# sxyu/volrend

Hardware: AMD Instinct MI355X
Metric: Mrays/s at 800x800, NeRF-synthetic-like SH16 (synthetic C1) (higher is better)
Workload: dtype f32; 1 GPU; C1: synthetic lego-like PlenOctree, depth 9, SH16, 2025715 nodes, 2.23 GB in HBM, 800x800, fx=fy=1111.111, 200-pose orbit, default RenderOptions; fp_mode=strict, launches=38, pcie_inclusive=False, launch_streams=1, parallelism=single GPU

## Files before the change

include/volrend_hip.h:

```cpp
#ifndef VOLREND_HIP_H_
#define VOLREND_HIP_H_

#include <stddef.h>
#include <stdint.h>

#ifdef __cplusplus
extern "C" {
#endif

#define VR_ABI_VERSION 3

enum {
    VR_OK = 0,
    VR_ERR_INVALID_ARGUMENT = 1,
    VR_ERR_HIP = 2,
    VR_ERR_NO_DEVICE = 3,
    VR_ERR_BAD_TREE = 4,
    VR_ERR_UNSUPPORTED = 5,
    VR_ERR_OUT_OF_MEMORY = 6
};

enum { VR_FORMAT_RGBA = 0, VR_FORMAT_SH = 1, VR_FORMAT_SG = 2, VR_FORMAT_ASG = 3 };

enum { VR_FP_STRICT = 0, VR_FP_FMA = 1 };

#define VR_MAX_BASIS 25

typedef struct VrTreeOpaque* vr_tree_t;

typedef struct VrTreeDesc {
    const int32_t* child;
    const uint16_t* data;
    const float* extra;
    uint64_t extra_count;
    float offset[3];
    float scale[3];
    int32_t N;
    int64_t capacity;
    int32_t data_dim;
    int32_t format;
    int32_t basis_dim;
    float ndc_width;
    float ndc_height;
    float ndc_focal;
    int32_t memory;
} VrTreeDesc;

typedef struct VrQuantDesc {
    const uint16_t* quant_colors;
    const uint16_t* quant_map;
    const uint16_t* sigma;
    const uint16_t* data_retained;
    int32_t n_quant;
    int32_t n_retained;
} VrQuantDesc;

typedef struct VrTreeInfo {
    int64_t capacity;
    int32_t N, data_dim, format, basis_dim;
    int32_t max_depth;
    int32_t device;
    uint64_t device_bytes;
    uint64_t leaf_stride;
    int32_t query_mode;
    int32_t top_levels;
    int32_t brick_levels;
    int32_t brick_blocked;
} VrTreeInfo;

#define VR_QUERY_LOOKUP 0
#define VR_QUERY_DESCENT 1
int vr_query_mode_for(int N, int max_depth, int64_t capacity);

typedef struct VrCamera {
    float transform[12];
    int32_t width, height;
    float fx, fy;
} VrCamera;

typedef struct VrRenderOptions {
    float step_size;
    float sigma_thresh;
    float stop_thresh;
    float background_brightness;
    float render_bbox[6];
    int32_t basis_minmax[2];
    float rot_dirs[3];
    int32_t show_grid;
    int32_t grid_max_depth;
    int32_t render_depth;
    int32_t enable_probe;
    float probe[3];
    int32_t probe_disp_size;
} VrRenderOptions;

enum { VR_LAYOUT_FRAME = 0, VR_LAYOUT_COMPACT = 1 };

typedef struct VrFrame {
    void* rgba;
    int64_t pitch;
    const float* depth;
    float* accum;
    int32_t offscreen;
    int32_t layout;
    int32_t tile_w, tile_h;
    int32_t rank, world;
    int32_t fp_mode;
    int32_t reserved;
    uint64_t* counters;
} VrFrame;

typedef struct VrCounters {
    uint64_t rays, rays_hit_box, samples, child_reads, hit_samples, alg_bytes, early_stops;
} VrCounters;

int vr_abi_version(void);
const char* vr_last_error(void);
int vr_device_count(int* count);
int vr_set_device(int device);
int vr_device_name(int device, char* name, size_t name_len);

void vr_default_tree_desc(VrTreeDesc* desc);
int vr_tree_upload(const VrTreeDesc* desc, vr_tree_t* out);
int vr_tree_upload_quantized(const VrTreeDesc* desc, const VrQuantDesc* quant, vr_tree_t* out);
int vr_decode_quantized(const VrTreeDesc* desc, const VrQuantDesc* quant, uint16_t* data_out);
int vr_tree_clone(vr_tree_t src, int device, vr_tree_t* out);
int vr_tree_free(vr_tree_t tree);
int vr_tree_info(vr_tree_t tree, VrTreeInfo* info);
enum { VR_DATA_F16 = 0, VR_DATA_F32 = 1 };
int vr_tree_update_data(vr_tree_t tree, const void* data_dev, int dtype, void* stream);
int vr_tree_read_data(vr_tree_t tree, void* data_dev, int dtype, void* stream);
enum { VR_STEP_SGD = 0, VR_STEP_ADAM = 1 };
typedef struct VrStep {
    float*    master;
    float*    grad;
    uint32_t* touched;
    float*    m;
    float*    v;
    int32_t   kind;
    float     lr, lr_sigma;
    float     beta1, beta2, eps;
    int32_t   step;
} VrStep;
int vr_tree_step(vr_tree_t tree, const VrStep* s, void* stream);

void vr_default_options(VrRenderOptions* opt);
void vr_default_frame(VrFrame* frame);
int64_t vr_compact_bytes(int width, int height, int tile_w, int tile_h, int world);
int vr_render(vr_tree_t tree, const VrCamera* cam, const VrRenderOptions* opt,
              const VrFrame* frame, void* stream);
#define VR_MAX_BATCH 512
int vr_render_batch(vr_tree_t tree, int n_frames, const VrCamera* cams,
                    const VrRenderOptions* opt, const VrFrame* frames, void* stream);
enum { VR_DEPTH_TREE = 0, VR_DEPTH_WORLD = 1 };
typedef struct VrAov {
    float*  depth;
    float*  transmittance;
    int64_t pitch;
} VrAov;
int vr_render_aov(vr_tree_t tree, int n_frames, const VrCamera* cams, const VrRenderOptions* opt,
                  const VrFrame* frames, const VrAov* aovs, int depth_units, void* stream);
typedef struct VrLeafWeights {
    float*    max_weight;
    uint32_t* hits;
} VrLeafWeights;
int vr_accumulate_weights(vr_tree_t tree, int n_frames, const VrCamera* cams,
                          const VrRenderOptions* opt, int fp_mode, const VrLeafWeights* out, void* stream);
int vr_render_backward(vr_tree_t tree, int n_frames, const VrCamera* cams, const VrRenderOptions* opt,
                       int fp_mode, const float* grad_accum, float* grad_data, void* stream);
typedef struct VrRays {
    const float* origins;
    const float* dirs;
} VrRays;
typedef struct VrRayOut {
    void*  rgba;
    float* accum;
} VrRayOut;
int vr_render_rays(vr_tree_t tree, int64_t n, const VrRays* rays, const VrRenderOptions* opt, int fp_mode,
                   const VrRayOut* out, void* stream);
int vr_accumulate_weights_rays(vr_tree_t tree, int64_t n, const VrRays* rays, const VrRenderOptions* opt,
                               int fp_mode, const VrLeafWeights* out, void* stream);
int vr_render_backward_rays(vr_tree_t tree, int64_t n, const VrRays* rays, const VrRenderOptions* opt,
                            int fp_mode, const float* grad_accum, float* grad_data, void* stream);
int vr_render_backward_touched(vr_tree_t tree, int n_frames, const VrCamera* cams, const VrRenderOptions* opt,
                               int fp_mode, const float* grad_accum, float* grad_data, uint32_t* touched,
                               void* stream);
int vr_render_backward_rays_touched(vr_tree_t tree, int64_t n, const VrRays* rays, const VrRenderOptions* opt,
                                    int fp_mode, const float* grad_accum, float* grad_data, uint32_t* touched,
                                    void* stream);
int vr_reserve_rays(vr_tree_t tree, int64_t n, int n_slots);
int vr_reserve(vr_tree_t tree, int width, int height, int n_frames);
int vr_reserve_tiles(vr_tree_t tree, int width, int height, int n_frames, int tile_w, int tile_h,
                     int world, int n_slots);
int vr_tree_status(vr_tree_t tree, uint32_t* status, int reset);
int vr_tree_status_on(vr_tree_t tree, uint32_t* status, int reset, void* stream);
int vr_set_tuning(const char* key, int value);
int vr_tree_set_tuning(vr_tree_t tree, const char* key, int value);
int vr_sched_stats(vr_tree_t tree, uint64_t out[8], int reset);
int vr_touch_enable(vr_tree_t tree, int enable);
int vr_touch_count(vr_tree_t tree, uint64_t out[4], int reset);
int vr_touch_read(vr_tree_t tree, int which, uint32_t* host_words, uint64_t n_words,
                  uint64_t* bitmap_words, uint64_t* granule_bytes);
int vr_assemble_tiles(void* frame_rgba, int64_t pitch, const void* gathered, int width,
                      int height, int tile_w, int tile_h, int world, void* stream);
int vr_assemble_tiles_batch(void* frames_rgba, int64_t frame_stride, int64_t pitch,
                            const void* gathered, int64_t rank_stride, int64_t in_frame_stride,
                            int n_frames, int width, int height, int tile_w, int tile_h, int world,
                            void* stream);
int vr_probe_coeffs(vr_tree_t tree, const VrRenderOptions* opt, float* out_dev, void* stream);

enum { VR_SPACE_WORLD = 0, VR_SPACE_TREE = 1 };

typedef struct VrQueryOut {
    float* sigma;
    int32_t* depth;
    float* local;
    float* coeffs;
    float* rgb;
} VrQueryOut;

int vr_query_points(vr_tree_t tree, int64_t n, const float* xyz_dev, const float* dirs_dev, int space,
                    const VrQueryOut* out, void* stream);
int vr_query_grid(vr_tree_t tree, const float lo[3], const float hi[3], const int32_t res[3],
                  const float dir[3], int space, const VrQueryOut* out, void* stream);

int vr_read_back(void* host_rgba, const void* dev_rgba, int64_t pitch, int width, int height,
                 void* stream);
int vr_stream_sync(void* stream);

#ifdef __cplusplus
}
#endif
#endif
```

volrend_amd/_abi.py:

```python
from __future__ import annotations

import ctypes as C
import os

HERE = os.path.dirname(os.path.abspath(__file__))
LIB_PATH = os.environ.get("VOLREND_HIP_LIB") or os.path.join(HERE, "libvolrend_hip.so")

VR_OK = 0
FORMAT_RGBA, FORMAT_SH, FORMAT_SG, FORMAT_ASG = 0, 1, 2, 3
FORMATS = {"RGBA": FORMAT_RGBA, "SH": FORMAT_SH, "SG": FORMAT_SG, "ASG": FORMAT_ASG}
FP_STRICT, FP_FMA = 0, 1
QUERY_LOOKUP, QUERY_DESCENT = 0, 1
LAYOUT_FRAME, LAYOUT_COMPACT = 0, 1
SPACE_WORLD, SPACE_TREE = 0, 1
SPACES = {"world": SPACE_WORLD, "tree": SPACE_TREE}
DEPTH_TREE, DEPTH_WORLD = 0, 1
DEPTH_UNITS = {"tree": DEPTH_TREE, "world": DEPTH_WORLD}
DATA_F16, DATA_F32 = 0, 1
STEP_SGD, STEP_ADAM = 0, 1
STEP_KINDS = {"sgd": STEP_SGD, "adam": STEP_ADAM}
MAX_BASIS = 25


class VrTreeDesc(C.Structure):
    _fields_ = [("child", C.c_void_p), ("data", C.c_void_p), ("extra", C.c_void_p),
                ("extra_count", C.c_uint64), ("offset", C.c_float * 3), ("scale", C.c_float * 3),
                ("N", C.c_int32), ("capacity", C.c_int64), ("data_dim", C.c_int32),
                ("format", C.c_int32), ("basis_dim", C.c_int32), ("ndc_width", C.c_float),
                ("ndc_height", C.c_float), ("ndc_focal", C.c_float), ("memory", C.c_int32)]


class VrQuantDesc(C.Structure):
    _fields_ = [("quant_colors", C.c_void_p), ("quant_map", C.c_void_p), ("sigma", C.c_void_p),
                ("data_retained", C.c_void_p), ("n_quant", C.c_int32), ("n_retained", C.c_int32)]


class VrTreeInfo(C.Structure):
    _fields_ = [("capacity", C.c_int64), ("N", C.c_int32), ("data_dim", C.c_int32),
                ("format", C.c_int32), ("basis_dim", C.c_int32), ("max_depth", C.c_int32),
                ("device", C.c_int32), ("device_bytes", C.c_uint64), ("leaf_stride", C.c_uint64),
                ("query_mode", C.c_int32), ("top_levels", C.c_int32), ("brick_levels", C.c_int32),
                ("brick_blocked", C.c_int32)]


class VrCamera(C.Structure):
    _fields_ = [("transform", C.c_float * 12), ("width", C.c_int32), ("height", C.c_int32),
                ("fx", C.c_float), ("fy", C.c_float)]


class VrRenderOptions(C.Structure):
    _fields_ = [("step_size", C.c_float), ("sigma_thresh", C.c_float), ("stop_thresh", C.c_float),
                ("background_brightness", C.c_float), ("render_bbox", C.c_float * 6),
                ("basis_minmax", C.c_int32 * 2), ("rot_dirs", C.c_float * 3),
                ("show_grid", C.c_int32), ("grid_max_depth", C.c_int32),
                ("render_depth", C.c_int32), ("enable_probe", C.c_int32),
                ("probe", C.c_float * 3), ("probe_disp_size", C.c_int32)]


class VrFrame(C.Structure):
    _fields_ = [("rgba", C.c_void_p), ("pitch", C.c_int64), ("depth", C.c_void_p),
                ("accum", C.c_void_p), ("offscreen", C.c_int32), ("layout", C.c_int32),
                ("tile_w", C.c_int32), ("tile_h", C.c_int32), ("rank", C.c_int32),
                ("world", C.c_int32), ("fp_mode", C.c_int32), ("reserved", C.c_int32),
                ("counters", C.c_void_p)]


class VrAov(C.Structure):
    _fields_ = [("depth", C.c_void_p), ("transmittance", C.c_void_p), ("pitch", C.c_int64)]


class VrLeafWeights(C.Structure):
    _fields_ = [("max_weight", C.c_void_p), ("hits", C.c_void_p)]


class VrRays(C.Structure):
    _fields_ = [("origins", C.c_void_p), ("dirs", C.c_void_p)]


class VrRayOut(C.Structure):
    _fields_ = [("rgba", C.c_void_p), ("accum", C.c_void_p)]


class VrStep(C.Structure):
    _fields_ = [("master", C.c_void_p), ("grad", C.c_void_p), ("touched", C.c_void_p), ("m", C.c_void_p),
                ("v", C.c_void_p), ("kind", C.c_int32), ("lr", C.c_float), ("lr_sigma", C.c_float),
                ("beta1", C.c_float), ("beta2", C.c_float), ("eps", C.c_float), ("step", C.c_int32)]


class VrQueryOut(C.Structure):
    _fields_ = [("sigma", C.c_void_p), ("depth", C.c_void_p), ("local", C.c_void_p),
                ("coeffs", C.c_void_p), ("rgb", C.c_void_p)]


ABI_VERSION = 3
MAX_BATCH = 512

COUNTER_FIELDS = ("rays", "rays_hit_box", "samples", "child_reads", "hit_samples", "alg_bytes",
                  "early_stops")


PROTOTYPES = {
    "vr_abi_version": (C.c_int, []),
    "vr_last_error": (C.c_char_p, []),
    "vr_device_count": (C.c_int, [C.POINTER(C.c_int)]),
    "vr_set_device": (C.c_int, [C.c_int]),
    "vr_device_name": (C.c_int, [C.c_int, C.c_char_p, C.c_size_t]),
    "vr_default_tree_desc": (None, [C.POINTER(VrTreeDesc)]),
    "vr_tree_upload": (C.c_int, [C.POINTER(VrTreeDesc), C.POINTER(C.c_void_p)]),
    "vr_tree_upload_quantized": (C.c_int, [C.POINTER(VrTreeDesc), C.POINTER(VrQuantDesc),
                                           C.POINTER(C.c_void_p)]),
    "vr_decode_quantized": (C.c_int, [C.POINTER(VrTreeDesc), C.POINTER(VrQuantDesc), C.c_void_p]),
    "vr_tree_clone": (C.c_int, [C.c_void_p, C.c_int, C.POINTER(C.c_void_p)]),
    "vr_tree_free": (C.c_int, [C.c_void_p]),
    "vr_tree_info": (C.c_int, [C.c_void_p, C.POINTER(VrTreeInfo)]),
    "vr_tree_update_data": (C.c_int, [C.c_void_p, C.c_void_p, C.c_int, C.c_void_p]),
    "vr_tree_read_data": (C.c_int, [C.c_void_p, C.c_void_p, C.c_int, C.c_void_p]),
    "vr_query_mode_for": (C.c_int, [C.c_int, C.c_int, C.c_int64]),
    "vr_default_options": (None, [C.POINTER(VrRenderOptions)]),
    "vr_default_frame": (None, [C.POINTER(VrFrame)]),
    "vr_compact_bytes": (C.c_int64, [C.c_int, C.c_int, C.c_int, C.c_int, C.c_int]),
    "vr_render": (C.c_int, [C.c_void_p, C.POINTER(VrCamera), C.POINTER(VrRenderOptions),
                            C.POINTER(VrFrame), C.c_void_p]),
    "vr_render_batch": (C.c_int, [C.c_void_p, C.c_int, C.POINTER(VrCamera),
                                  C.POINTER(VrRenderOptions), C.POINTER(VrFrame), C.c_void_p]),
    "vr_render_aov": (C.c_int, [C.c_void_p, C.c_int, C.POINTER(VrCamera), C.POINTER(VrRenderOptions),
                                C.POINTER(VrFrame), C.POINTER(VrAov), C.c_int, C.c_void_p]),
    "vr_accumulate_weights": (C.c_int, [C.c_void_p, C.c_int, C.POINTER(VrCamera), C.POINTER(VrRenderOptions),
                                        C.c_int, C.POINTER(VrLeafWeights), C.c_void_p]),
    "vr_render_backward": (C.c_int, [C.c_void_p, C.c_int, C.POINTER(VrCamera), C.POINTER(VrRenderOptions),
                                     C.c_int, C.c_void_p, C.c_void_p, C.c_void_p]),
    "vr_render_backward_touched": (C.c_int, [C.c_void_p, C.c_int, C.POINTER(VrCamera), C.POINTER(VrRenderOptions),
                                             C.c_int, C.c_void_p, C.c_void_p, C.c_void_p, C.c_void_p]),
    "vr_render_backward_rays_touched": (C.c_int, [C.c_void_p, C.c_int64, C.POINTER(VrRays), C.POINTER(VrRenderOptions),
                                                  C.c_int, C.c_void_p, C.c_void_p, C.c_void_p, C.c_void_p]),
    "vr_tree_step": (C.c_int, [C.c_void_p, C.POINTER(VrStep), C.c_void_p]),
    "vr_render_rays": (C.c_int, [C.c_void_p, C.c_int64, C.POINTER(VrRays), C.POINTER(VrRenderOptions), C.c_int,
                                 C.POINTER(VrRayOut), C.c_void_p]),
    "vr_accumulate_weights_rays": (C.c_int, [C.c_void_p, C.c_int64, C.POINTER(VrRays), C.POINTER(VrRenderOptions),
                                             C.c_int, C.POINTER(VrLeafWeights), C.c_void_p]),
    "vr_render_backward_rays": (C.c_int, [C.c_void_p, C.c_int64, C.POINTER(VrRays), C.POINTER(VrRenderOptions),
                                          C.c_int, C.c_void_p, C.c_void_p, C.c_void_p]),
    "vr_reserve_rays": (C.c_int, [C.c_void_p, C.c_int64, C.c_int]),
    "vr_reserve": (C.c_int, [C.c_void_p, C.c_int, C.c_int, C.c_int]),
    "vr_reserve_tiles": (C.c_int, [C.c_void_p, C.c_int, C.c_int, C.c_int, C.c_int, C.c_int, C.c_int,
                                   C.c_int]),
    "vr_tree_status": (C.c_int, [C.c_void_p, C.POINTER(C.c_uint32), C.c_int]),
    "vr_tree_status_on": (C.c_int, [C.c_void_p, C.POINTER(C.c_uint32), C.c_int, C.c_void_p]),
    "vr_set_tuning": (C.c_int, [C.c_char_p, C.c_int]),
    "vr_tree_set_tuning": (C.c_int, [C.c_void_p, C.c_char_p, C.c_int]),
    "vr_sched_stats": (C.c_int, [C.c_void_p, C.POINTER(C.c_uint64 * 8), C.c_int]),
    "vr_touch_enable": (C.c_int, [C.c_void_p, C.c_int]),
    "vr_touch_count": (C.c_int, [C.c_void_p, C.POINTER(C.c_uint64 * 4), C.c_int]),
    "vr_touch_read": (C.c_int, [C.c_void_p, C.c_int, C.c_void_p, C.c_uint64, C.POINTER(C.c_uint64),
                                C.POINTER(C.c_uint64)]),
    "vr_assemble_tiles": (C.c_int, [C.c_void_p, C.c_int64, C.c_void_p, C.c_int, C.c_int, C.c_int,
                                    C.c_int, C.c_int, C.c_void_p]),
    "vr_assemble_tiles_batch": (C.c_int, [C.c_void_p, C.c_int64, C.c_int64, C.c_void_p, C.c_int64,
                                          C.c_int64, C.c_int, C.c_int, C.c_int, C.c_int, C.c_int,
                                          C.c_int, C.c_void_p]),
    "vr_probe_coeffs": (C.c_int, [C.c_void_p, C.POINTER(VrRenderOptions), C.c_void_p, C.c_void_p]),
    "vr_query_points": (C.c_int, [C.c_void_p, C.c_int64, C.c_void_p, C.c_void_p, C.c_int,
                                  C.POINTER(VrQueryOut), C.c_void_p]),
    "vr_query_grid": (C.c_int, [C.c_void_p, C.POINTER(C.c_float * 3), C.POINTER(C.c_float * 3),
                                C.POINTER(C.c_int32 * 3), C.POINTER(C.c_float * 3), C.c_int,
                                C.POINTER(VrQueryOut), C.c_void_p]),
    "vr_read_back": (C.c_int, [C.c_void_p, C.c_void_p, C.c_int64, C.c_int, C.c_int, C.c_void_p]),
    "vr_stream_sync": (C.c_int, [C.c_void_p]),
}

_lib = None


class VolrendError(RuntimeError):
    def __init__(self, code: int, msg: str):
        super().__init__(f"volrend_hip error {code}: {msg}")
        self.code = code


def lib():
    global _lib
    if _lib is None:
        if not os.path.exists(LIB_PATH):
            raise RuntimeError(
                f"{LIB_PATH} not found: the HIP library is mandatory (no CPU fallback). "
                "Build it with `python -m volrend_amd.build`.")
        L = C.CDLL(LIB_PATH)
        for name, (res, args) in PROTOTYPES.items():
            fn = getattr(L, name)
            fn.restype = res
            fn.argtypes = args
        if L.vr_abi_version() != ABI_VERSION:
            raise RuntimeError("libvolrend_hip.so ABI version mismatch")
        _lib = L
    return _lib


def check(rc: int) -> None:
    if rc != VR_OK:
        raise VolrendError(rc, (lib().vr_last_error() or b"").decode("utf-8", "replace"))
```

volrend_amd/_tree.py:

```python
from __future__ import annotations

import ctypes as C
import os

import numpy as np

from . import _abi, _ops
from ._args import _stream_ptr


def parse_data_format(s: str):
    idx = next((i for i, ch in enumerate(s) if not ch.isalpha()), -1)
    if idx < 0:
        return "RGBA", -1
    head = s[:idx]
    try:
        dim = int("".join(ch for ch in s[idx:] if ch.isdigit() or ch == "-") or "0")
    except ValueError:
        dim = 0
    return (head if head in ("ASG", "SG", "SH") else "RGBA"), dim


class N3Tree:

    def __init__(self, path: str | None = None, upload: bool = True):
        self.N = 0
        self.data_dim = 0
        self.data_format = ("RGBA", -1)
        self.capacity = 0
        self.scale = np.zeros(3, np.float32)
        self.offset = np.zeros(3, np.float32)
        self.use_ndc = False
        self.ndc_width = self.ndc_height = self.ndc_focal = 0.0
        self.child_ = None
        self.data_ = None
        self.extra_ = None
        self.quant_ = None
        self._handle = C.c_void_p()
        self._loaded = False
        if path is not None:
            self.open(path, upload=upload)

    @classmethod
    def from_arrays(cls, child, data, offset, invradius3, data_format: str, extra=None,
                    ndc=None, upload: bool = True) -> "N3Tree":
        t = cls()
        t._set_arrays(child, data, offset, invradius3, data_format, extra)
        if ndc:
            t.use_ndc = True
            t.ndc_width, t.ndc_height, t.ndc_focal = map(float, ndc)
        if upload:
            t.load_device()
        return t

    @classmethod
    def from_synth(cls, tree, upload: bool = True, ndc=None) -> "N3Tree":
        return cls.from_arrays(tree.child, tree.data, tree.offset, tree.invradius3,
                               tree.data_format, tree.extra, ndc=ndc, upload=upload)

    def _set_arrays(self, child, data, offset, invradius3, data_format, extra, data_dim=None):
        child = np.ascontiguousarray(child, dtype=np.int32)
        if child.ndim != 4 or not (child.shape[1] == child.shape[2] == child.shape[3]):
            raise RuntimeError("child must be int32 [capacity, N, N, N]")
        self.N = int(child.shape[1])
        self.capacity = int(child.shape[0])
        self.child_ = child.reshape(self.capacity, self.N, self.N, self.N)
        self.quant_ = None
        if data is None:
            self.data_ = None
            self.data_dim = int(data_dim)
        else:
            data = np.asarray(data)
            if data.dtype != np.float16:
                raise RuntimeError("data must be stored in half precision")
            self.data_ = np.ascontiguousarray(data)
            self.data_dim = int(self.data_.shape[-1])
            if self.data_.size != self.capacity * self.N ** 3 * self.data_dim:
                raise RuntimeError("data does not have capacity * N^3 * data_dim values")
        self.data_format = parse_data_format(data_format)
        self.scale = np.asarray(invradius3, dtype=np.float32).reshape(3).copy()
        self.offset = np.asarray(offset, dtype=np.float32).reshape(3).copy()
        self.extra_ = None if extra is None else np.ascontiguousarray(extra, dtype=np.float32)

    def open(self, path: str, upload: bool = True, device_decode: bool = True) -> None:
        if not path.endswith(".npz"):
            raise ValueError("tree file must end in .npz")
        if not os.path.exists(path):
            raise FileNotFoundError(f"Can't load because file does not exist: {path}")
        z = np.load(path)
        data_dim = int(z["data_dim"])
        if "data_format" in z.files:
            fmt = str(z["data_format"])
        else:
            fmt = "RGBA" if data_dim == 4 else f"SH{(data_dim - 1) // 3}"
        if "invradius3" in z.files:
            scale = z["invradius3"].astype(np.float32)
        else:
            scale = np.full(3, float(z["invradius"]), dtype=np.float32)
        child = z["child"]
        extra = z["extra_data"] if "extra_data" in z.files else None
        if "quant_colors" in z.files and upload and device_decode:
            self._set_arrays(child, None, z["offset"], scale, fmt, extra, data_dim=data_dim)
            self.quant_ = _quant_arrays(z, child)
        else:
            if "quant_colors" in z.files:
                data = _decode_quantised(z, child, data_dim)
            else:
                data = z["data"]
            self._set_arrays(child, data, z["offset"], scale, fmt, extra)
            if self.data_dim != data_dim:
                raise RuntimeError("data_dim does not match the data array")
        pb = path[:-4] + "_poses_bounds.npy"
        if os.path.exists(pb):
            arr = np.load(pb).reshape(-1)
            self.use_ndc = True
            self.ndc_height, self.ndc_width, self.ndc_focal = float(arr[4]), float(arr[9]), float(
                arr[14])
        if upload:
            self.load_device()

    def load_device(self) -> None:
        L = _abi.lib()
        self.free_device()
        d = _abi.VrTreeDesc()
        L.vr_default_tree_desc(C.byref(d))
        d.child = self.child_.ctypes.data
        if self.data_ is not None:
            d.data = self.data_.ctypes.data
        elif self.quant_ is None:
            raise RuntimeError("tree has no data (clear_cpu_memory was called)")
        if self.extra_ is not None:
            d.extra = self.extra_.ctypes.data
            d.extra_count = self.extra_.size
        for i in range(3):
            d.offset[i] = float(self.offset[i])
            d.scale[i] = float(self.scale[i])
        d.N = self.N
        d.capacity = self.capacity
        d.data_dim = self.data_dim
        d.format = _abi.FORMATS[self.data_format[0]]
        d.basis_dim = self.data_format[1]
        d.ndc_width = self.ndc_width if self.use_ndc else -1.0
        d.ndc_height = self.ndc_height
        d.ndc_focal = self.ndc_focal
        d.memory = 0
        h = C.c_void_p()
        if self.data_ is None:
            _abi.check(L.vr_tree_upload_quantized(C.byref(d), C.byref(self._quant_desc()),
                                                  C.byref(h)))
        else:
            _abi.check(L.vr_tree_upload(C.byref(d), C.byref(h)))
        self._handle = h
        self._loaded = True

    def _quant_desc(self) -> "_abi.VrQuantDesc":
        q = _abi.VrQuantDesc()
        a = self.quant_
        q.n_quant = a["quant_map"].shape[0]
        q.quant_colors = a["quant_colors"].ctypes.data
        q.quant_map = a["quant_map"].ctypes.data
        q.sigma = a["sigma"].ctypes.data
        if a["data_retained"] is not None:
            q.n_retained = a["data_retained"].shape[0]
            q.data_retained = a["data_retained"].ctypes.data
        return q

    def decode_host(self, on_device: bool = False) -> np.ndarray:
        if self.data_ is None and self.quant_ is not None:
            shape = (self.capacity, self.N, self.N, self.N, self.data_dim)
            if on_device:
                d = _abi.VrTreeDesc()
                _abi.lib().vr_default_tree_desc(C.byref(d))
                d.N, d.capacity, d.data_dim, d.memory = self.N, self.capacity, self.data_dim, 0
                out = np.empty(shape, np.float16)
                _abi.check(_abi.lib().vr_decode_quantized(C.byref(d), C.byref(self._quant_desc()),
                                                          out.ctypes.data))
                self.data_ = out
            else:
                a = self.quant_
                self.data_ = _decode_arrays(a["quant_colors"], a["quant_map"], a["sigma"],
                                            a["data_retained"], self.data_dim).reshape(shape)
        return self.data_

    def clone_to(self, device: int) -> "N3Tree":
        t = N3Tree()
        for k in ("N", "data_dim", "data_format", "capacity", "scale", "offset", "use_ndc",
                  "ndc_width", "ndc_height", "ndc_focal", "child_"):
            setattr(t, k, getattr(self, k))
        h = C.c_void_p()
        _abi.check(_abi.lib().vr_tree_clone(self.handle, int(device), C.byref(h)))
        t._handle = h
        t._loaded = True
        return t

    def free_device(self) -> None:
        if self._handle:
            _abi.lib().vr_tree_free(self._handle)
            self._handle = C.c_void_p()
        self._loaded = False

    def is_device_loaded(self) -> bool:
        return self._loaded

    def clear_cpu_memory(self) -> None:
        self.data_ = None
        self.quant_ = None

    def sched_stats(self, reset: bool = True) -> dict:
        out = (C.c_uint64 * 8)()
        _abi.check(_abi.lib().vr_sched_stats(self._handle, C.byref(out), 1 if reset else 0))
        names = ("march_rounds", "march_lanes", "shade_rounds", "shade_lanes", "distinct_leaves",
                 "retire_rounds", "retired", "iterations")
        return dict(zip(names, [int(v) for v in out]))

    def touch_enable(self, enable: bool = True) -> None:
        _abi.check(_abi.lib().vr_touch_enable(self.handle, 1 if enable else 0))

    def touch_count(self, reset: bool = True) -> dict:
        out = (C.c_uint64 * 4)()
        _abi.check(_abi.lib().vr_touch_count(self.handle, C.byref(out), 1 if reset else 0))
        return dict(zip(("leaves", "nodes", "top", "bricks"), [int(v) for v in out]))

    def touch_read(self, which: int):
        words, gran = C.c_uint64(0), C.c_uint64(0)
        _abi.check(_abi.lib().vr_touch_read(self.handle, int(which), None, 0, C.byref(words), C.byref(gran)))
        out = np.zeros(int(words.value), dtype=np.uint32)
        if out.size:
            _abi.check(_abi.lib().vr_touch_read(self.handle, int(which), out.ctypes.data, out.size, None, None))
        return out, int(gran.value)

    def reserve(self, width: int, height: int, n_frames: int, shard: "TileShard | None" = None,
                n_slots: int = 2) -> None:
        if shard is None and n_slots == 2:
            _abi.check(_abi.lib().vr_reserve(self.handle, int(width), int(height), int(n_frames)))
        else:
            tw, th, world = (shard.tile_w, shard.tile_h, shard.world) if shard else (0, 0, 1)
            _abi.check(_abi.lib().vr_reserve_tiles(self.handle, int(width), int(height),
                                                   int(n_frames), tw, th, world, int(n_slots)))

    def set_tuning(self, **kw) -> None:
        for k, v in kw.items():
            _abi.check(_abi.lib().vr_tree_set_tuning(self.handle, k.encode(), int(v)))

    def status(self, reset: bool = False, stream=None) -> int:
        out = C.c_uint32(0)
        if stream is not None:
            _abi.check(_abi.lib().vr_tree_status_on(self.handle, C.byref(out), 1 if reset else 0,
                                                    _stream_ptr(stream)))
        else:
            _abi.check(_abi.lib().vr_tree_status(self.handle, C.byref(out), 1 if reset else 0))
        return int(out.value)

    def reserve_rays(self, n: int, n_slots: int = 2) -> None:
        _abi.check(_abi.lib().vr_reserve_rays(self.handle, int(n), int(n_slots)))

    query, query_grid = _ops.query_points, _ops.query_grid
    accumulate_weights, render_backward = _ops.accumulate_weights, _ops.render_backward
    render_rays, accumulate_weights_rays = _ops.render_rays, _ops.accumulate_weights_rays
    render_backward_rays, touched_words = _ops.render_backward_rays, _ops.touched_words
    step, update_data, read_data = _ops.tree_step, _ops.update_data, _ops.read_data

    def info(self) -> dict:
        i = _abi.VrTreeInfo()
        _abi.check(_abi.lib().vr_tree_info(self._handle, C.byref(i)))
        return {n: int(getattr(i, n)) for n, _ in i._fields_}

    @property
    def handle(self):
        if not self._loaded:
            raise RuntimeError("tree is not on the device (call load_device)")
        return self._handle

    def __del__(self):
        try:
            self.free_device()
        except Exception:
            pass


def _quant_arrays(z, child) -> dict:
    qc = z["quant_colors"]
    if qc.dtype != np.float16:
        raise RuntimeError("codebook must be stored in half precision")
    qm = z["quant_map"]
    n_q = qm.shape[0]
    if qc.shape[0] != n_q:
        raise RuntimeError("codebook and map basis numbers does not match")
    cap, N = qm.shape[1], child.shape[1]
    if cap != child.shape[0] or qc.shape[1:] != (65536, 3):
        raise RuntimeError("quantised arrays do not match the tree")
    n_slots = cap * N * N * N
    retained = z["data_retained"] if "data_retained" in z.files else None
    return dict(
        quant_colors=np.ascontiguousarray(qc),
        quant_map=np.ascontiguousarray(qm.reshape(n_q, n_slots), dtype=np.uint16),
        sigma=np.ascontiguousarray(z["sigma"].reshape(n_slots), dtype=np.float16),
        data_retained=None if retained is None else np.ascontiguousarray(
            retained.reshape(retained.shape[0], n_slots, 3), dtype=np.float16))


def _decode_arrays(qc, qm, sigma, retained, data_dim: int) -> np.ndarray:
    n_q, n_slots = qm.shape
    n_ret = 0 if retained is None else retained.shape[0]
    n_basis = n_q + n_ret
    data = np.zeros((n_slots, data_dim), dtype=np.float16)
    for j in range(n_q):
        cols = qc[j][qm[j].astype(np.int64)]
        for c in range(3):
            data[:, j + n_ret + c * n_basis] = cols[:, c]
    data[:, data_dim - 1] = sigma
    for j in range(n_ret):
        for c in range(3):
            data[:, j + c * n_basis] = retained[j, :, c]
    return data


def _decode_quantised(z, child, data_dim: int) -> np.ndarray:
    a = _quant_arrays(z, child)
    cap, N = child.shape[0], child.shape[1]
    return _decode_arrays(a["quant_colors"], a["quant_map"], a["sigma"], a["data_retained"],
                          data_dim).reshape(cap, N, N, N, data_dim)
```

volrend_amd/csrc/vr_api.cpp:

```cpp
#include <hip/hip_runtime.h>

#include <climits>
#include <cstdarg>
#include <cstdio>
#include <cstdlib>
#include <cstring>
#include <mutex>

#include "vr_host.h"
#include "vr_tree_walk.h"

namespace {

thread_local char g_err[512] = "";

enum KnobRange { kClamp, kClamp64, kFlag, kAutoFlag };
struct Knob { const char *key, *env; int Tuning::*field; KnobRange range; int lo, hi; bool fixed_at_upload; };
const Knob kKnobs[] = {
    {"march_max", "VR_MARCH_MAX", &Tuning::march_max, kClamp, 1, INT_MAX, false},
    {"refill_min", "VR_REFILL_MIN", &Tuning::refill_min, kClamp, 1, 64, false},
    {"drain_flush", "VR_DRAIN_FLUSH", &Tuning::drain_flush, kClamp, 0, 64, false},
    {"waves_per_cu", "VR_WAVES_PER_CU", &Tuning::waves_per_cu, kClamp, 0, 64, false},
    {"frame_group", "VR_FRAME_GROUP", &Tuning::frame_group, kClamp, 0, INT_MAX, false},
    {"super_block", "VR_SUPER_BLOCK", &Tuning::super_block, kClamp, 0, 64, false},
    {"records_nt", "VR_RECORDS_NT", &Tuning::records_nt, kAutoFlag, 0, 0, false},
    {"xcd_queues", "VR_XCD_QUEUES", &Tuning::xcd_queues, kFlag, 0, 0, false},
    {"chunk_max", "VR_CHUNK_MAX", &Tuning::chunk_max, kClamp64, 0, INT_MAX, false},
    {"raygen_waves", "VR_RAYGEN_WAVES", &Tuning::raygen_waves, kClamp, 0, INT_MAX, false},
    {"top_levels", "VR_TOP_LEVELS", &Tuning::top_levels, kClamp, INT_MIN, INT_MAX, true},
    {"brick_levels", "VR_BRICK_LEVELS", &Tuning::brick_levels, kClamp, INT_MIN, INT_MAX, true},
    {"brick_blocked", "VR_BRICK_BLOCKED", &Tuning::brick_blocked, kAutoFlag, 0, 0, true},
    {"max_iter", "VR_MAX_ITER", &Tuning::max_iter, kClamp, 1, INT_MAX, false},
    {"weights_check", "VR_WEIGHTS_CHECK", &Tuning::weights_check, kFlag, 0, 0, false},
};

const Knob* find_knob(const char* key) {
    for (const Knob& k : kKnobs)
        if (!strcmp(key, k.key)) return &k;
    return nullptr;
}

void set_knob(Tuning& tn, const Knob& k, int v) {
    const int clamped = v < k.lo ? k.lo : (v > k.hi ? k.hi : v);
    tn.*k.field = k.range == kFlag       ? v != 0
                  : k.range == kAutoFlag ? (v < 0 ? -1 : v != 0)
                  : k.range == kClamp64  ? (clamped > 0 && clamped < 64 ? 64 : clamped & ~63)
                                         : clamped;
}

std::mutex g_tuning_mutex;
Tuning& default_tuning_locked() {
    static Tuning tn = [] {
        Tuning x;
        for (const Knob& k : kKnobs)
            if (const char* e = getenv(k.env)) set_knob(x, k, atoi(e));
        return x;
    }();
    return tn;
}

uint64_t touch_granule(int which) {
    return which == 0 ? (1ull << vr::kTouchLeafShift) : 128ull;
}
size_t touch_words(uint64_t array_bytes, int which) {
    const uint64_t g = touch_granule(which);
    return (size_t)(((array_bytes + g - 1) / g + 31) / 32);
}

}

int fail(int code, const char* fmt, ...) {
    va_list ap;
    va_start(ap, fmt);
    vsnprintf(g_err, sizeof(g_err), fmt, ap);
    va_end(ap);
    return code;
}

Tuning default_tuning() {
    std::lock_guard<std::mutex> g(g_tuning_mutex);
    return default_tuning_locked();
}

extern "C" {

int vr_abi_version(void) { return VR_ABI_VERSION; }

const char* vr_last_error(void) { return g_err; }

int vr_device_count(int* count) {
    if (!count) return fail(VR_ERR_INVALID_ARGUMENT, "count is NULL");
    int n = 0;
    hipError_t e = hipGetDeviceCount(&n);
    if (e != hipSuccess) {
        *count = 0;
        return fail(VR_ERR_NO_DEVICE, "hipGetDeviceCount: %s", hipGetErrorString(e));
    }
    *count = n;
    return VR_OK;
}

int vr_set_device(int device) {
    if (device < 0) return VR_OK;
    HIP_TRY(hipSetDevice(device));
    return VR_OK;
}

int vr_device_name(int device, char* name, size_t name_len) {
    if (!name || name_len == 0) return fail(VR_ERR_INVALID_ARGUMENT, "name buffer is NULL");
    hipDeviceProp_t prop;
    if (device < 0) HIP_TRY(hipGetDevice(&device));
    HIP_TRY(hipGetDeviceProperties(&prop, device));
    snprintf(name, name_len, "%s", prop.gcnArchName);
    return VR_OK;
}

void vr_default_tree_desc(VrTreeDesc* d) {
    if (!d) return;
    memset(d, 0, sizeof(*d));
    d->N = 2;
    d->format = VR_FORMAT_RGBA;
    d->basis_dim = -1;
    d->ndc_width = -1.f;
}

int vr_tree_info(vr_tree_t t, VrTreeInfo* info) {
    if (!t || !info) return fail(VR_ERR_INVALID_ARGUMENT, "tree/info is NULL");
    info->capacity = t->desc.capacity;
    info->N = t->desc.N;
    info->data_dim = t->desc.data_dim;
    info->format = t->desc.format;
    info->basis_dim = t->desc.basis_dim;
    info->max_depth = t->max_depth;
    info->device = t->device;
    info->device_bytes = t->device_bytes;
    info->leaf_stride = (uint64_t)t->leaf_stride_h * 2u;
    info->query_mode = t->top_levels > 0 ? VR_QUERY_LOOKUP : VR_QUERY_DESCENT;
    info->top_levels = t->top_levels;
    info->brick_levels = t->brick_levels;
    info->brick_blocked = t->brick_blocked;
    return VR_OK;
}

int vr_query_mode_for(int N, int max_depth, int64_t capacity) {
    return lookup_applies(N, max_depth, capacity) ? VR_QUERY_LOOKUP : VR_QUERY_DESCENT;
}

void vr_default_options(VrRenderOptions* o) {
    if (!o) return;
    memset(o, 0, sizeof(*o));
    o->step_size = 1e-4f;
    o->sigma_thresh = 1e-2f;
    o->stop_thresh = 1e-2f;
    o->background_brightness = 1.f;
    o->render_bbox[3] = o->render_bbox[4] = o->render_bbox[5] = 1.f;
    o->basis_minmax[0] = 0;
    o->basis_minmax[1] = VR_MAX_BASIS - 1;
    o->grid_max_depth = 4;
    o->probe[2] = 1.f;
    o->probe_disp_size = 100;
}

void vr_default_frame(VrFrame* f) {
    if (!f) return;
    memset(f, 0, sizeof(*f));
    f->offscreen = 1;
    f->layout = VR_LAYOUT_FRAME;
    f->world = 1;
    f->fp_mode = VR_FP_STRICT;
}

int64_t vr_compact_bytes(int width, int height, int tile_w, int tile_h, int world) {
    vr::KParams g;
    if (tile_geometry(width, height, tile_w, tile_h, 0, world, g) != VR_OK) return -1;
    return (int64_t)g.n_local_tiles * g.tile_w * g.tile_h * 4;
}

int vr_set_tuning(const char* key, int value) {
    if (!key) return fail(VR_ERR_INVALID_ARGUMENT, "key is NULL");
    const Knob* k = find_knob(key);
    if (!k) return fail(VR_ERR_INVALID_ARGUMENT, "unknown tuning key '%s'", key);
    std::lock_guard<std::mutex> g(g_tuning_mutex);
    set_knob(default_tuning_locked(), *k, value);
    return VR_OK;
}

int vr_tree_set_tuning(vr_tree_t t, const char* key, int value) {
    if (!t || !key) return fail(VR_ERR_INVALID_ARGUMENT, "tree/key is NULL");
    const Knob* k = find_knob(key);
    if (!k) return fail(VR_ERR_INVALID_ARGUMENT, "unknown tuning key '%s'", key);
    if (k->fixed_at_upload)
        return fail(VR_ERR_INVALID_ARGUMENT, "'%s' is fixed at upload (vr_set_tuning before it)", key);
    std::lock_guard<std::mutex> g(t->launch_mutex);
    set_knob(t->tn, *k, value);
    return VR_OK;
}

int vr_sched_stats(vr_tree_t t, uint64_t out[vr::kSchedStats], int reset) {
    if (!t || !out) return fail(VR_ERR_INVALID_ARGUMENT, "NULL argument");
    DeviceGuard guard(t->device);
    HIP_TRY(hipMemcpy(out, t->sched_stats.get(), vr::kSchedStats * sizeof(uint64_t), hipMemcpyDeviceToHost));
    if (reset) HIP_TRY(hipMemset(t->sched_stats.get(), 0, vr::kSchedStats * sizeof(uint64_t)));
    return VR_OK;
}

int vr_tree_status(vr_tree_t t, uint32_t* status, int reset) {
    if (!t || !status) return fail(VR_ERR_INVALID_ARGUMENT, "NULL argument");
    DeviceGuard guard(t->device);
    HIP_TRY(hipMemcpy(status, t->status.get(), sizeof(uint32_t), hipMemcpyDeviceToHost));
    if (reset) HIP_TRY(hipMemset(t->status.get(), 0, sizeof(uint32_t)));
    return VR_OK;
}

int vr_tree_status_on(vr_tree_t t, uint32_t* status, int reset, void* stream) {
    if (!t || !status) return fail(VR_ERR_INVALID_ARGUMENT, "NULL argument");
    DeviceGuard guard(t->device);
    hipStream_t hs = static_cast<hipStream_t>(stream);
    thread_local uint32_t* pinned = nullptr;
    if (!pinned) HIP_TRY(hipHostMalloc((void**)&pinned, sizeof(uint32_t), hipHostMallocPortable));
    HIP_TRY(hipMemcpyAsync(pinned, t->status.get(), sizeof(uint32_t), hipMemcpyDeviceToHost, hs));
    if (reset) HIP_TRY(hipMemsetAsync(t->status.get(), 0, sizeof(uint32_t), hs));
    HIP_TRY(hipStreamSynchronize(hs));
    *status = *pinned;
    return VR_OK;
}

int vr_touch_enable(vr_tree_t t, int enable) {
    if (!t) return fail(VR_ERR_INVALID_ARGUMENT, "tree is NULL");
    DeviceGuard guard(t->device);
    std::lock_guard<std::mutex> lock(t->launch_mutex);
    HIP_TRY(hipDeviceSynchronize());
    for (int i = 0; i < 4; ++i) {
        HIP_TRY(t->touch[i].reset());
        const size_t words = touch_words(t->arrays[i].bytes(), i);
        if (enable && words) {
            HIP_TRY(t->touch[i].alloc(words * sizeof(uint32_t)));
            HIP_TRY(hipMemset(t->touch[i].get(), 0, words * sizeof(uint32_t)));
        }
    }
    if (enable && !t->touch_out) HIP_TRY(t->touch_out.alloc(4 * sizeof(unsigned long long)));
    return VR_OK;
}

int vr_touch_count(vr_tree_t t, uint64_t out[4], int reset) {
    if (!t || !out) return fail(VR_ERR_INVALID_ARGUMENT, "NULL argument");
    if (!t->touch_out) return fail(VR_ERR_INVALID_ARGUMENT, "vr_touch_enable(tree, 1) first");
    DeviceGuard guard(t->device);
    std::lock_guard<std::mutex> lock(t->launch_mutex);
    HIP_TRY(hipDeviceSynchronize());
    HIP_TRY(hipMemset(t->touch_out.get(), 0, 4 * sizeof(unsigned long long)));
    for (int i = 0; i < 4; ++i) {
        if (!t->touch[i]) continue;
        const size_t words = touch_words(t->arrays[i].bytes(), i);
        HIP_TRY(vr::launch_popcount(t->touch[i].get<uint32_t>(), words,
                                    t->touch_out.get<unsigned long long>() + i, nullptr));
        if (reset) HIP_TRY(hipMemsetAsync(t->touch[i].get(), 0, words * sizeof(uint32_t), nullptr));
    }
    HIP_TRY(hipMemcpy(out, t->touch_out.get(), 4 * sizeof(uint64_t), hipMemcpyDeviceToHost));
    return VR_OK;
}

int vr_touch_read(vr_tree_t t, int which, uint32_t* host_words, uint64_t n_words,
                  uint64_t* bitmap_words, uint64_t* granule_bytes) {
    if (!t || which < 0 || which > 3) return fail(VR_ERR_INVALID_ARGUMENT, "tree / array index");
    if (!t->touch_out) return fail(VR_ERR_INVALID_ARGUMENT, "vr_touch_enable(tree, 1) first");
    DeviceGuard guard(t->device);
    std::lock_guard<std::mutex> lock(t->launch_mutex);
    const uint64_t words = t->touch[which] ? touch_words(t->arrays[which].bytes(), which) : 0;
    if (bitmap_words) *bitmap_words = words;
    if (granule_bytes) *granule_bytes = touch_granule(which);
    const uint64_t n = n_words < words ? n_words : words;
    if (host_words && n) {
        HIP_TRY(hipDeviceSynchronize());
        HIP_TRY(hipMemcpy(host_words, t->touch[which].get(), n * sizeof(uint32_t), hipMemcpyDeviceToHost));
    }
    return VR_OK;
}

int vr_assemble_tiles(void* frame_rgba, int64_t pitch, const void* gathered, int width, int height,
                      int tile_w, int tile_h, int world, void* stream) {
    if (world < 1) world = 1;
    const int64_t rank_bytes = vr_compact_bytes(width, height, tile_w, tile_h, world);
    if (rank_bytes < 0) return VR_ERR_INVALID_ARGUMENT;
    return vr_assemble_tiles_batch(frame_rgba, 0, pitch, gathered, rank_bytes, 0, 1, width, height,
                                   tile_w, tile_h, world, stream);
}

int vr_assemble_tiles_batch(void* frames_rgba, int64_t frame_stride, int64_t pitch,
                            const void* gathered, int64_t rank_stride, int64_t in_frame_stride,
                            int n_frames, int width, int height, int tile_w, int tile_h, int world,
                            void* stream) {
    if (!frames_rgba || !gathered) return fail(VR_ERR_INVALID_ARGUMENT, "NULL buffer");
    if (n_frames < 1) return fail(VR_ERR_INVALID_ARGUMENT, "n_frames must be positive");
    if (world < 1) world = 1;
    vr::KParams g;
    if (int rc = tile_geometry(width, height, tile_w, tile_h, 0, world, g)) return rc;
    HIP_TRY(vr::launch_assemble(static_cast<uint8_t*>(frames_rgba),
                                pitch ? pitch : (int64_t)width * 4,
                                static_cast<const uint8_t*>(gathered), width, height, g.tile_w, g.tile_h, world,
                                n_frames, frame_stride, rank_stride, in_frame_stride,
                                static_cast<hipStream_t>(stream)));
    return VR_OK;
}

int vr_probe_coeffs(vr_tree_t t, const VrRenderOptions* opt, float* out_dev, void* stream) {
    if (!t || !opt || !out_dev) return fail(VR_ERR_INVALID_ARGUMENT, "NULL argument");
    DeviceGuard guard(t->device);
    vr::KParams k;
    memset(&k, 0, sizeof(k));
    fill_tree_params(k, t);
    HIP_TRY(vr::launch_probe(k, opt->probe, out_dev, static_cast<hipStream_t>(stream)));
    return VR_OK;
}

int vr_read_back(void* host_rgba, const void* dev_rgba, int64_t pitch, int width, int height,
                 void* stream) {
    if (!host_rgba || !dev_rgba) return fail(VR_ERR_INVALID_ARGUMENT, "NULL buffer");
    if (pitch == 0) pitch = (int64_t)width * 4;
    HIP_TRY(hipMemcpy2DAsync(host_rgba, (size_t)width * 4, dev_rgba, (size_t)pitch,
                             (size_t)width * 4, (size_t)height, hipMemcpyDeviceToHost,
                             static_cast<hipStream_t>(stream)));
    return VR_OK;
}

int vr_stream_sync(void* stream) {
    HIP_TRY(hipStreamSynchronize(static_cast<hipStream_t>(stream)));
    return VR_OK;
}

}
```

volrend_amd/csrc/vr_host.h:

```cpp
#pragma once
#include <hip/hip_runtime.h>

#include <mutex>
#include <vector>

#include "vr_internal.h"
#include "vr_launch_plan.h"

#pragma GCC visibility push(hidden)

#include "volrend/internal/hip_owners.hpp"
using volrend::internal::DeviceBuffer;
using volrend::internal::DeviceEvent;
using volrend::internal::DeviceGuard;

int fail(int code, const char* fmt, ...);
inline int hip_code(hipError_t e) { return e == hipErrorOutOfMemory ? VR_ERR_OUT_OF_MEMORY : VR_ERR_HIP; }

#define HIP_TRY(expr)                                                                                 \
    do {                                                                                              \
        hipError_t e_ = (expr);                                                                       \
        if (e_ != hipSuccess)                                                                         \
            return fail(hip_code(e_), "%s failed: %s (%s:%d)", #expr, hipGetErrorString(e_), __FILE__, \
                        __LINE__);                                                                    \
    } while (0)

Tuning default_tuning();

constexpr unsigned kLaunchSlots = 8;

struct LaunchSlot {
    DeviceEvent done;
    bool used = false;
    hipStream_t last_stream = nullptr;
    bool growing = false;
    DeviceBuffer rays;
};

enum TreeArray { kLeaves = 0, kNodes = 1, kTop = 2, kBricks = 3 };

struct TreeShape {
    VrTreeDesc desc{};
    int32_t max_depth = 0;
    int leaf_stride_h = 0;
    int top_levels = 0, brick_levels = 0, n_bricks = 0;
    int brick_blocked = 0;
    uint64_t device_bytes = 0;
};

struct VrTreeOpaque : TreeShape {
    int device = 0;
    DeviceBuffer arrays[4];
    DeviceBuffer extra, status, sched_stats;
    DeviceBuffer touch[4];
    DeviceBuffer touch_out;
    DeviceBuffer probe_buf;
    DeviceBuffer slot_frames;
    DeviceBuffer slot_heads;
    DeviceBuffer slot_aovs;
    std::vector<int32_t> file_node;
    DeviceBuffer file_node_dev;
    std::vector<int32_t> brick_root;
    DeviceBuffer brick_root_dev;
    DeviceBuffer node_of_file_dev;
    LaunchSlot slots[kLaunchSlots];
    unsigned launch_seq = 0;
    std::mutex launch_mutex;
    Tuning tn;
    int n_cus = 256;
};

void fill_tree_params(vr::KParams& k, const VrTreeOpaque* t);

int tile_geometry(int width, int height, int tile_w, int tile_h, int rank, int world, vr::KParams& k);
int launch_geometry(int width, int height, int tile_w, int tile_h, int rank, int world, int n_frames,
                    vr::KParams& k);
int list_geometry(const char* what, int64_t n, vr::KParams& k);

inline size_t ray_buffer_bytes(uint32_t total_rays, int words_per_ray) {
    return vr::ray_slots(total_rays) * (size_t)words_per_ray * sizeof(uint32_t);
}
inline size_t list_pixel_bytes(uint32_t total_rays) { return (size_t)total_rays * 4; }

int acquire_slot(VrTreeOpaque* t, std::unique_lock<std::mutex>& guard, hipStream_t hs, vr::KParams& k,
                 size_t need, unsigned& slot);

class SlotTurn {
    LaunchSlot* slot_ = nullptr;
    hipStream_t stream_ = nullptr;
public:
    int begin(LaunchSlot& ls, hipStream_t hs);
    ~SlotTurn();
};

int ensure_device_table(VrTreeOpaque* t, DeviceBuffer& dev, const std::vector<int32_t>& host, size_t entries,
                        const char* name);
int ensure_file_nodes(VrTreeOpaque* t);

#pragma GCC visibility pop
```

volrend_amd/csrc/vr_internal.h:

```cpp
#pragma once
#include <hip/hip_runtime.h>
#include <stdint.h>

#include "volrend_hip.h"

namespace vr {

constexpr int kMaxBatch = 512;
constexpr int kTableChunk = 48;
constexpr int kTouchLeafShift = 7;

enum { BASIS_RGBA = -1, BASIS_1 = 1, BASIS_4 = 4, BASIS_9 = 9, BASIS_16 = 16, BASIS_25 = 25 };
__host__ __device__ inline int basis_flavour(int format, int basis_dim) {
    if (format == VR_FORMAT_RGBA || basis_dim < 0) return BASIS_RGBA;
    switch (basis_dim) {
        case 25: return BASIS_25;
        case 16: return BASIS_16;
        case 9: return BASIS_9;
        case 4: return BASIS_4;
        default: return BASIS_1;
    }
}
__host__ __device__ inline int basis_words(int flavour) { return flavour == BASIS_RGBA ? 0 : flavour; }
__host__ __device__ inline bool ray_vdir(int format, int flavour) {
    return format == VR_FORMAT_SH && basis_words(flavour) > 3;
}
__host__ __device__ inline int ray_tail_words(int format, int flavour) {
    return ray_vdir(format, flavour) ? 3 : basis_words(flavour);
}

enum {
    kRayCen = 0,
    kRayDir = 3,
    kRayInvDir = 6,
    kRayT = 9,
    kRayTmax = 10,
    kRayDeltaScale = 11,
    kRayXy = 12,
    kRayPixelLo = 13,
    kRayPixelHi = 14,
    kRayFrame = 15,
    kRayWords = 16,
    kRayTail = kRayWords,
};
__host__ __device__ inline uint32_t ray_groups16(uint32_t total_rays) { return ((total_rays >> 6) + 15u) >> 4; }
__host__ __device__ inline size_t ray_slots(uint32_t total_rays) { return (size_t)ray_groups16(total_rays) * 16 * 64; }

constexpr int kMaxQueues = 8;
constexpr int kMaxQueuesShift = 3;
constexpr int kQueueStride = 16;
constexpr int kQueueHead = 0;
constexpr int kQueueCount = 1;
constexpr int kSlotHeaderWords = 16;
constexpr int kSlotWords = 160;
static_assert(kMaxQueues == 1 << kMaxQueuesShift, "queues are picked with shifts and masks");
static_assert(kSlotWords >= kSlotHeaderWords + kMaxQueues * kQueueStride, "a slot holds its header and every queue");

enum {
    kStatMarchRounds = 0,
    kStatMarchLanes,
    kStatShadeRounds,
    kStatShadeLanes,
    kStatDistinctLeaves,
    kStatRetireRounds,
    kStatRetiredRays,
    kStatIterations,
    kSchedStats
};
static_assert(kSchedStats == 8, "vr_sched_stats(out[8]) is public ABI");

struct FrameDesc {
    float xf[12];
    uint8_t* rgba;
    float* accum;
    const float* depth;
    VrCounters* counters;
};

struct FrameTable {
    int32_t first;
    int32_t n;
    FrameDesc f[kTableChunk];
};

struct KParams {
    const uint32_t* nodes;
    const uint16_t* leaves;
    const uint2* top;
    const uint32_t* bricks;
    const float* extra;
    float offset[3];
    float scale[3];
    int32_t N, N3;
    int64_t capacity;
    int32_t data_dim;
    int32_t format;
    int32_t basis_dim;
    int32_t leaf_stride_h;
    int32_t max_depth;
    int32_t top_levels;
    int32_t brick_levels;
    int32_t brick_blocked;
    float ndc_width, ndc_height, ndc_focal;
    int32_t width, height;
    float fx, fy;
    float step_size, sigma_thresh, stop_thresh, background_brightness;
    float bbox[6];
    int32_t basis_min, basis_max;
    int32_t render_depth;
    int32_t enable_probe;
    int32_t probe_disp_size;
    const float* probe_coeffs;
    int32_t rot_enabled;
    float rot_k[3];
    float rot_cos, rot_sin;
    const FrameDesc* frames;
    int32_t n_frames;
    int64_t pitch;
    int32_t offscreen;
    int32_t layout;
    int32_t tile_w, tile_h;
    int32_t tiles_x, tiles_y;
    int32_t rank, world;
    int32_t n_local_tiles;
    int32_t wblocks_per_tile_x;
    int32_t wblocks_per_tile;
    int64_t n_wave_blocks;
    uint32_t total_rays;
    uint32_t* queue_head;
    int32_t n_queues;
    int32_t chunk_max;
    const uint32_t* ray_buf;
    uint32_t* ray_buf_rw;
    int32_t basis_words;
    int32_t ray_tail_words;
    int32_t ray_vdir;
    int32_t refill_min;
    int32_t march_max;
    int32_t drain_flush;
    int32_t max_iter;
    int32_t instrumented;
    int32_t any_accum;
    int32_t records_nt;
    int32_t frame_group;
    int32_t super_block;
    uint32_t* status;
    unsigned long long* sched_stats;
    uint32_t* touch[4];
};

inline bool uses_lookup(const KParams& p) { return p.N == 2 && p.top_levels > 0; }

inline unsigned persistent_grid(int64_t total_blocks, int n_cus, int waves_per_cu) {
    int64_t want = total_blocks / 2;
    if (want < 256) want = 256;
    if (want > total_blocks) want = total_blocks;
    const int64_t cap = (int64_t)n_cus * waves_per_cu;
    return (unsigned)(want < cap ? want : cap);
}

struct AovDesc {
    float* depth;
    float* transmittance;
};
struct AovParams {
    const AovDesc* planes;
    int64_t pitch;
    int32_t depth_world;
};
struct AovTable {
    int32_t first;
    int32_t n;
    AovDesc f[kTableChunk];
};

constexpr int kWeightRayWords = kRayDeltaScale + 1;
static_assert(kWeightRayWords <= kRayWords, "a slot reserved for colour rays holds the weight rays of the same shape");
struct WeightParams {
    uint32_t* max_weight;
    uint32_t* hits;
    const int32_t* file_node;
};

constexpr int kRayListShift = 15;
constexpr int kRayListWidth = 1 << kRayListShift;
struct RayList {
    const float* origins;
    const float* dirs;
    int64_t n;
};
__host__ __device__ inline uint32_t ray_list_slots(int64_t n) { return (uint32_t)(((n + 63) >> 6) << 6); }

hipError_t launch_weights(const KParams& p, const WeightParams& w, int fp_mode, int n_cus, int waves_override,
                          int gen_waves, bool check_first, hipStream_t stream, const RayList* rays = nullptr);

enum {
    kGradRayVdir = kWeightRayWords,
    kGradRayPixel = kGradRayVdir + 3,
    kGradRayWords = kGradRayPixel + 1,
};
static_assert(kGradRayWords <= kRayWords, "a slot reserved for colour rays holds the backward rays of the same shape");
struct GradParams {
    const float* grad_accum;
    float* grad_data;
    const int32_t* file_node;
    uint32_t* touched;
};

hipError_t launch_grad(const KParams& p, const GradParams& g, int fp_mode, int n_cus, int waves_override,
                       int gen_waves, hipStream_t stream, const RayList* rays = nullptr);

struct UpdateArgs {
    uint32_t* nodes;
    uint16_t* leaves;
    const int32_t* file_node;
    void* data;
    int64_t capacity;
    int32_t N3, data_dim;
    int32_t stride_h;
    int32_t f32;
};
hipError_t launch_update_values(const UpdateArgs& a, int n_cus, hipStream_t stream);
hipError_t launch_read_values(const UpdateArgs& a, int n_cus, hipStream_t stream);
hipError_t launch_refresh_lookup(const uint32_t* nodes, const int32_t* brick_root, int n_bricks, uint2* top,
                                 uint32_t* bricks, int top_levels, int brick_levels, hipStream_t stream);

struct StepArgs {
    uint32_t* nodes;
    uint16_t* leaves;
    const int32_t* node_of_file;
    float* master;
    float* grad;
    float* m;
    float* v;
    uint32_t* touched;
    int64_t n_words;
    int64_t n_slots;
    int32_t N3, data_dim;
    int32_t stride_h;
    int32_t adam;
    float lr, lr_sigma;
    float beta1, beta2, omb1, omb2, sbc2, eps;
};
hipError_t launch_step_values(const StepArgs& a, int n_cus, hipStream_t stream);

hipError_t launch_prepare_aov(const AovParams& a, const AovTable& tbl, hipStream_t stream);
hipError_t launch_render_aov(const KParams& p, const AovParams& a, int fp_mode, int n_cus, int waves_override,
                             int gen_waves, hipStream_t stream);
hipError_t launch_prepare(const KParams& p, const FrameTable& tbl, hipStream_t stream);
hipError_t launch_render(const KParams& p, int fp_mode, int n_cus, int waves_override, int gen_waves,
                         hipStream_t stream, const RayList* rays = nullptr);
hipError_t launch_probe(const KParams& p, const float probe[3], float* out_dev,
                        hipStream_t stream);

int leaf_stride_halfs(int data_dim);
hipError_t launch_relayout(const int32_t* child, const uint16_t* data, const int32_t* perm,
                           uint32_t* nodes, uint16_t* leaves, int64_t n_slots, int N3,
                           int data_dim, int stride_h, hipStream_t stream);
hipError_t launch_decode_quant(const uint16_t* colors, const uint16_t* map, const uint16_t* sigma,
                               const uint16_t* retained, uint16_t* data, int64_t n_slots,
                               int n_quant, int n_ret, int data_dim, hipStream_t stream);
hipError_t launch_build_lookup(const uint32_t* nodes, const int32_t* brick_root, int n_bricks,
                               uint2* top, uint32_t* bricks, int top_levels, int brick_levels,
                               int brick_blocked, uint32_t* error_flag, hipStream_t stream);
hipError_t launch_popcount(const uint32_t* words, uint64_t n_words, unsigned long long* out,
                           hipStream_t stream);
hipError_t launch_assemble(uint8_t* frame, int64_t pitch, const uint8_t* gathered, int width,
                           int height, int tile_w, int tile_h, int world, int n_frames,
                           int64_t out_stride, int64_t rank_stride, int64_t in_stride,
                           hipStream_t stream);

}
```

volrend_amd/csrc/vr_launch.cpp:

```cpp
#include <hip/hip_runtime.h>

#include <cmath>
#include <cstring>
#include <mutex>

#include "vr_host.h"

static_assert(kPlanQueues == vr::kMaxQueues, "vr_launch_plan.h restates the queue count of vr_internal.h");

namespace {

float host_norm3(const float* d, int fma) {
    float s;
    if (fma) {
        s = std::fmaf(d[0], d[0], d[1] * d[1]);
        s = std::fmaf(d[2], d[2], s);
    } else {
        s = d[0] * d[0] + d[1] * d[1];
        s = d[2] * d[2] + s;
    }
    return std::sqrt(s);
}

}

void fill_tree_params(vr::KParams& k, const VrTreeOpaque* t) {
    k.nodes = t->arrays[kNodes].get<uint32_t>();
    k.leaves = t->arrays[kLeaves].get<uint16_t>();
    k.top = t->arrays[kTop].get<uint2>();
    k.bricks = t->arrays[kBricks].get<uint32_t>();
    k.top_levels = t->top_levels;
    k.brick_levels = t->brick_levels;
    k.brick_blocked = t->brick_blocked;
    k.extra = t->extra.get<float>();
    for (int i = 0; i < 3; ++i) {
        k.offset[i] = t->desc.offset[i];
        k.scale[i] = t->desc.scale[i];
    }
    k.N = t->desc.N;
    k.N3 = t->desc.N * t->desc.N * t->desc.N;
    k.capacity = t->desc.capacity;
    k.data_dim = t->desc.data_dim;
    k.format = t->desc.format;
    k.basis_dim = t->desc.basis_dim;
    k.leaf_stride_h = t->leaf_stride_h;
    k.max_depth = t->max_depth;
    k.ndc_width = t->desc.ndc_width;
    k.ndc_height = t->desc.ndc_height;
    k.ndc_focal = t->desc.ndc_focal;
    k.status = t->status.get<uint32_t>();
    k.sched_stats = t->sched_stats.get<unsigned long long>();
    for (int i = 0; i < 4; ++i) k.touch[i] = t->touch[i].get<uint32_t>();
}

int tile_geometry(int width, int height, int tile_w, int tile_h, int rank, int world, vr::KParams& k) {
    if (width <= 0 || height <= 0) return fail(VR_ERR_INVALID_ARGUMENT, "empty image");
    if (tile_w == 0 && tile_h == 0) {
        tile_w = (width + 7) & ~7;
        tile_h = (height + 7) & ~7;
    }
    if (tile_w <= 0 || tile_h <= 0 || (tile_w & 7) || (tile_h & 7))
        return fail(VR_ERR_INVALID_ARGUMENT, "tile size %dx%d must be positive multiples of 8",
                    tile_w, tile_h);
    k.tile_w = tile_w;
    k.tile_h = tile_h;
    k.tiles_x = (width + tile_w - 1) / tile_w;
    k.tiles_y = (height + tile_h - 1) / tile_h;
    k.rank = rank;
    k.world = world < 1 ? 1 : world;
    k.n_local_tiles = (int32_t)(((int64_t)k.tiles_x * k.tiles_y - rank + k.world - 1) / k.world);
    k.wblocks_per_tile_x = tile_w / 8;
    k.wblocks_per_tile = (tile_w / 8) * (tile_h / 8);
    k.n_wave_blocks = (int64_t)k.n_local_tiles * k.wblocks_per_tile;
    return VR_OK;
}

int launch_geometry(int width, int height, int tile_w, int tile_h, int rank, int world, int n_frames,
                    vr::KParams& k) {
    if (width < 1 || height < 1 || width > 65535 || height > 65535)
        return fail(VR_ERR_INVALID_ARGUMENT, "image size %dx%d outside [1, 65535]", width, height);
    if (int rc = tile_geometry(width, height, tile_w, tile_h, rank, world, k)) return rc;
    const int64_t total = k.n_wave_blocks * 64 * n_frames;
    if (total >= (1ll << 30))
        return fail(VR_ERR_INVALID_ARGUMENT, "batch of %lld rays exceeds the 2^30-ray queue",
                    (long long)total);
    k.total_rays = (uint32_t)total;
    return VR_OK;
}

int list_geometry(const char* what, int64_t n, vr::KParams& k) {
    if (n < 0 || n >= (1ll << 30))
        return fail(VR_ERR_INVALID_ARGUMENT, "%s: n=%lld outside [0, 2^30)", what, (long long)n);
    k.total_rays = vr::ray_list_slots(n);
    k.n_wave_blocks = k.total_rays >> 6;
    k.n_frames = n > 0 ? 1 : 0;
    k.width = vr::kRayListWidth;
    k.height = (int32_t)((n + vr::kRayListWidth - 1) >> vr::kRayListShift);
    k.fx = k.fy = 1.f;
    k.pitch = (int64_t)k.width * 4;
    k.tile_w = k.width;
    k.tile_h = (k.height + 7) & ~7;
    k.tiles_x = k.tiles_y = k.world = k.n_local_tiles = 1;
    return VR_OK;
}

namespace {

struct Views {
    const VrCamera* cams = nullptr;
    int n_frames = 0;
    vr::RayList list{};
    bool is_list = false;
    const vr::RayList* rays() const { return is_list ? &list : nullptr; }
};

int check_focal(const VrCamera& cam) {
    if (!(cam.fx != 0.f) || !(cam.fy != 0.f)) return fail(VR_ERR_INVALID_ARGUMENT, "focal length must be non-zero");
    return VR_OK;
}
int check_intrinsics(const VrCamera* cams, int i) {
    if (cams[i].width != cams[0].width || cams[i].height != cams[0].height || cams[i].fx != cams[0].fx ||
        cams[i].fy != cams[0].fy)
        return fail(VR_ERR_INVALID_ARGUMENT, "frame %d: intrinsics differ within the batch", i);
    return VR_OK;
}

int check_step_size(const VrRenderOptions* opt) {
    if (!(opt->step_size > 0.f))
        return fail(VR_ERR_INVALID_ARGUMENT, "step_size must be positive (got %g)", (double)opt->step_size);
    return VR_OK;
}

int pose_geometry(const VrCamera& cam, int tile_w, int tile_h, int rank, int world, int n_frames, vr::KParams& k) {
    if (int rc = launch_geometry(cam.width, cam.height, tile_w, tile_h, rank, world, n_frames, k)) return rc;
    k.width = cam.width;
    k.height = cam.height;
    k.fx = cam.fx;
    k.fy = cam.fy;
    k.n_frames = n_frames;
    return VR_OK;
}

int validate_batch(vr_tree_t t, int n_frames, const VrCamera* cams, const VrRenderOptions* opt,
                   const VrFrame* frames, vr::KParams& k) {
    if (!t || !cams || !opt || !frames) return fail(VR_ERR_INVALID_ARGUMENT, "NULL argument");
    if (n_frames < 1 || n_frames > VR_MAX_BATCH)
        return fail(VR_ERR_INVALID_ARGUMENT, "n_frames=%d outside [1,%d]", n_frames, VR_MAX_BATCH);
    const VrFrame* f = &frames[0];
    const VrCamera* cam = &cams[0];
    if (f->fp_mode != VR_FP_STRICT && f->fp_mode != VR_FP_FMA)
        return fail(VR_ERR_INVALID_ARGUMENT, "unknown fp_mode %d", f->fp_mode);
    if (f->layout != VR_LAYOUT_FRAME && f->layout != VR_LAYOUT_COMPACT)
        return fail(VR_ERR_INVALID_ARGUMENT, "unknown layout %d", f->layout);
    const int world = f->world < 1 ? 1 : f->world;
    if (f->rank < 0 || f->rank >= world)
        return fail(VR_ERR_INVALID_ARGUMENT, "rank %d outside world %d", f->rank, world);
    if (int rc = pose_geometry(*cam, f->tile_w, f->tile_h, f->rank, world, n_frames, k))
        return rc;
    k.pitch = f->pitch ? f->pitch : (int64_t)cam->width * 4;
    if (k.pitch < (int64_t)cam->width * 4 || k.pitch * cam->height >= (1ll << 32))
        return fail(VR_ERR_INVALID_ARGUMENT, "pitch %lld unusable for a %dx%d frame",
                    (long long)k.pitch, cam->width, cam->height);
    if (int rc = check_focal(*cam)) return rc;

    bool instrumented = false, any_accum = false;
    for (int i = 0; i < n_frames; ++i) {
        const VrFrame& fi = frames[i];
        if (!fi.rgba) return fail(VR_ERR_INVALID_ARGUMENT, "frame %d: rgba is NULL", i);
        if (int rc = check_intrinsics(cams, i)) return rc;
        if (fi.pitch != f->pitch || fi.offscreen != f->offscreen || fi.layout != f->layout ||
            fi.tile_w != f->tile_w || fi.tile_h != f->tile_h || fi.rank != f->rank ||
            fi.world != f->world || fi.fp_mode != f->fp_mode)
            return fail(VR_ERR_INVALID_ARGUMENT, "frame %d: layout/shard/fp_mode differ within the batch", i);
        instrumented = instrumented || fi.counters != nullptr;
        any_accum = any_accum || fi.accum != nullptr;
    }

    if (int rc = check_step_size(opt)) return rc;
    k.instrumented = instrumented ? 1 : 0;
    k.any_accum = any_accum ? 1 : 0;
    return VR_OK;
}

void fill_march_params(vr::KParams& k, const VrRenderOptions* opt) {
    k.step_size = opt->step_size;
    k.sigma_thresh = opt->sigma_thresh;
    k.stop_thresh = opt->stop_thresh;
    memcpy(k.bbox, opt->render_bbox, sizeof(k.bbox));
}

void fill_caller_params(vr::KParams& k, const VrRenderOptions* opt, const VrFrame* f) {
    fill_march_params(k, opt);
    k.background_brightness = opt->background_brightness;
    k.basis_min = opt->basis_minmax[0];
    k.basis_max = opt->basis_minmax[1];
    k.render_depth = opt->render_depth != 0;
    k.enable_probe = opt->enable_probe != 0;
    k.probe_disp_size = opt->probe_disp_size;

    const float angle = host_norm3(opt->rot_dirs, f->fp_mode == VR_FP_FMA);
    if ((double)angle < 1e-6) {
        k.rot_enabled = 0;
    } else {
        k.rot_enabled = 1;
        for (int i = 0; i < 3; ++i) k.rot_k[i] = opt->rot_dirs[i] / angle;
        k.rot_cos = cosf(angle);
        k.rot_sin = sinf(angle);
    }
    k.offscreen = f->offscreen != 0;
    k.layout = f->layout;
}

void fill_tuning_params(vr::KParams& k, const VrTreeOpaque* t, const Tuning& tn, const LaunchPlan& plan) {
    k.records_nt = plan.records_nt;
    k.march_max = tn.march_max;
    k.refill_min = tn.refill_min;
    k.drain_flush = tn.drain_flush;
    k.max_iter = tn.max_iter;
    k.frame_group = plan.frame_group;
    k.super_block = plan.super_block;
    k.n_queues = plan.n_queues;
    k.chunk_max = plan.chunk_max;
    const int flavour = vr::basis_flavour(t->desc.format, t->desc.basis_dim);
    k.basis_words = vr::basis_words(flavour);
    k.ray_tail_words = vr::ray_tail_words(t->desc.format, flavour);
    k.ray_vdir = vr::ray_vdir(t->desc.format, flavour) ? 1 : 0;
}

int record_words(LaunchKind kind, int ray_tail_words) {
    return kind == LaunchKind::kWeights ? vr::kWeightRayWords
           : kind == LaunchKind::kBackward ? vr::kGradRayWords : vr::kRayWords + ray_tail_words;
}
bool needs_file_order(LaunchKind kind) { return kind == LaunchKind::kWeights || kind == LaunchKind::kBackward; }

struct Turn { const vr::KParams& k; const Tuning& tn; int gen_waves; unsigned slot; hipStream_t hs; void* pixel_words; };

template <typename Enqueue>
int run_launch(VrTreeOpaque* t, LaunchKind kind, const Views& v, bool pixel_words, vr::KParams& k, void* stream,
               Enqueue&& enqueue) {
    DeviceGuard device_guard(t->device);
    hipStream_t hs = static_cast<hipStream_t>(stream);
    std::unique_lock<std::mutex> guard(t->launch_mutex);
    if (needs_file_order(kind))
        if (int rc = ensure_file_nodes(t)) return rc;
    if (k.n_frames == 0) return VR_OK;
    const Tuning tn = t->tn;
    const LaunchPlan plan = plan_launch(kind, v.is_list ? RaySource::kList : RaySource::kFrames, k.n_frames, v.list.n,
                                        tn, t->arrays[kTop].bytes() + t->arrays[kBricks].bytes());
    fill_tuning_params(k, t, tn, plan);
    const size_t records = ray_buffer_bytes(k.total_rays, record_words(kind, k.ray_tail_words));
    unsigned slot;
    if (int rc = acquire_slot(t, guard, hs, k, records + (pixel_words ? list_pixel_bytes(k.total_rays) : 0), slot))
        return rc;
    fill_tree_params(k, t);
    SlotTurn turn;
    if (int rc = turn.begin(t->slots[slot], hs)) return rc;
    void* const pixels = pixel_words ? t->slots[slot].rays.get<char>() + records : nullptr;
    return enqueue(Turn{k, tn, plan.raygen_waves, slot, hs, pixels});
}

int validate_aov(int n_frames, const VrCamera* cams, const VrRenderOptions* opt, const VrFrame* frames,
                 const VrAov* aovs, int depth_units, vr::AovParams& a) {
    if (!aovs) return fail(VR_ERR_INVALID_ARGUMENT, "aovs is NULL");
    if (depth_units != VR_DEPTH_TREE && depth_units != VR_DEPTH_WORLD)
        return fail(VR_ERR_INVALID_ARGUMENT, "unknown depth_units %d", depth_units);
    const int64_t row = (int64_t)cams[0].width * 4;
    const int64_t pitch = aovs[0].pitch ? aovs[0].pitch : row;
    for (int i = 0; i < n_frames; ++i) {
        if (!aovs[i].depth && !aovs[i].transmittance)
            return fail(VR_ERR_INVALID_ARGUMENT, "frame %d: both AOV planes are NULL", i);
        const int64_t pi = aovs[i].pitch ? aovs[i].pitch : row;
        if (pi < row || (pi & 3))
            return fail(VR_ERR_INVALID_ARGUMENT, "frame %d: AOV pitch %lld unusable for rows of %d floats", i,
                        (long long)aovs[i].pitch, cams[0].width);
        if (pi != pitch) return fail(VR_ERR_INVALID_ARGUMENT, "frame %d: AOV pitch differs within the batch", i);
    }
    if (opt->render_depth)
        return fail(VR_ERR_UNSUPPORTED, "vr_render_aov with render_depth: the depth visualisation already is that launch");
    if (opt->enable_probe)
        return fail(VR_ERR_UNSUPPORTED, "vr_render_aov with enable_probe: pixels under the probe disc are not traced");
    for (int i = 0; i < n_frames; ++i)
        if (frames[i].counters)
            return fail(VR_ERR_UNSUPPORTED, "frame %d: vr_render_aov has no instrumented flavour (counters)", i);
    a.pitch = pitch;
    a.depth_world = depth_units == VR_DEPTH_WORLD;
    return VR_OK;
}

int enqueue_tables(const vr::KParams& k, const Views& v, hipStream_t hs, const VrFrame* frames = nullptr,
                   const VrAov* aovs = nullptr, const vr::AovParams& a = vr::AovParams{}) {
    for (int first = 0; first < k.n_frames; first += vr::kTableChunk) {
        vr::FrameTable tbl;
        memset(&tbl, 0, sizeof(tbl));
        tbl.first = first;
        tbl.n = k.n_frames - first < vr::kTableChunk ? k.n_frames - first : vr::kTableChunk;
        for (int i = 0; i < tbl.n; ++i) {
            if (!v.is_list) memcpy(tbl.f[i].xf, v.cams[first + i].transform, sizeof(tbl.f[i].xf));
            if (!frames) continue;
            tbl.f[i].rgba = static_cast<uint8_t*>(frames[first + i].rgba);
            tbl.f[i].accum = frames[first + i].accum;
            tbl.f[i].depth = frames[first + i].depth;
            tbl.f[i].counters = reinterpret_cast<VrCounters*>(frames[first + i].counters);
        }
        HIP_TRY(vr::launch_prepare(k, tbl, hs));
        if (aovs) {
            vr::AovTable at;
            memset(&at, 0, sizeof(at));
            at.first = first;
            at.n = tbl.n;
            for (int i = 0; i < at.n; ++i) {
                at.f[i].depth = aovs[first + i].depth;
                at.f[i].transmittance = aovs[first + i].transmittance;
            }
            HIP_TRY(vr::launch_prepare_aov(a, at, hs));
        }
    }
    return VR_OK;
}

int render_launch(vr_tree_t t, int n_frames, const VrCamera* cams, const VrRenderOptions* opt,
                  const VrFrame* frames, const VrAov* aovs, int depth_units, bool want_aov, void* stream) {
    vr::KParams k;
    memset(&k, 0, sizeof(k));
    vr::AovParams a;
    memset(&a, 0, sizeof(a));
    if (int rc = validate_batch(t, n_frames, cams, opt, frames, k)) return rc;
    if (want_aov)
        if (int rc = validate_aov(n_frames, cams, opt, frames, aovs, depth_units, a)) return rc;
    fill_caller_params(k, opt, &frames[0]);
    const Views v{cams, n_frames};
    return run_launch(t, want_aov ? LaunchKind::kAov : LaunchKind::kColour, v, false, k, stream, [&](const Turn& u) -> int {
        a.planes = t->slot_aovs.get<vr::AovDesc>() + (size_t)u.slot * vr::kMaxBatch;
        if (u.k.enable_probe)
            HIP_TRY(vr::launch_probe(u.k, opt->probe, const_cast<float*>(u.k.probe_coeffs), u.hs));
        if (int rc = enqueue_tables(u.k, v, u.hs, frames, want_aov ? aovs : nullptr, a)) return rc;
        if (want_aov)
            HIP_TRY(vr::launch_render_aov(u.k, a, frames[0].fp_mode, t->n_cus, u.tn.waves_per_cu, u.gen_waves, u.hs));
        else
            HIP_TRY(vr::launch_render(u.k, frames[0].fp_mode, t->n_cus, u.tn.waves_per_cu, u.gen_waves, u.hs));
        return VR_OK;
    });
}

int validate_march(int n_frames, const VrCamera* cams, const VrRenderOptions* opt, int fp_mode, vr::KParams& k) {
    if (fp_mode != VR_FP_STRICT && fp_mode != VR_FP_FMA)
        return fail(VR_ERR_INVALID_ARGUMENT, "unknown fp_mode %d", fp_mode);
    if (n_frames < 0 || n_frames > VR_MAX_BATCH)
        return fail(VR_ERR_INVALID_ARGUMENT, "n_frames=%d outside [0,%d]", n_frames, VR_MAX_BATCH);
    if (int rc = check_step_size(opt)) return rc;
    if (n_frames == 0) return VR_OK;
    if (int rc = pose_geometry(cams[0], 0, 0, 0, 1, n_frames, k)) return rc;
    if (int rc = check_focal(cams[0])) return rc;
    for (int i = 1; i < n_frames; ++i)
        if (int rc = check_intrinsics(cams, i)) return rc;
    return VR_OK;
}

int validate_weights(vr_tree_t t, int n_frames, const VrCamera* cams, const VrRenderOptions* opt, int fp_mode,
                     const VrLeafWeights* out, vr::KParams& k) {
    if (!t || !opt || !out || (n_frames > 0 && !cams)) return fail(VR_ERR_INVALID_ARGUMENT, "NULL argument");
    if (!out->max_weight && !out->hits) return fail(VR_ERR_INVALID_ARGUMENT, "both outputs are NULL");
    return validate_march(n_frames, cams, opt, fp_mode, k);
}

int validate_rays(const char* what, vr_tree_t t, int64_t n, const VrRays* rays, const VrRenderOptions* opt,
                  int fp_mode, const void* out, vr::KParams& k, Views& v) {
    if (!t || !rays || !rays->origins || !rays->dirs || !opt || !out)
        return fail(VR_ERR_INVALID_ARGUMENT, "%s: NULL argument", what);
    if (fp_mode != VR_FP_STRICT && fp_mode != VR_FP_FMA)
        return fail(VR_ERR_INVALID_ARGUMENT, "%s: unknown fp_mode %d", what, fp_mode);
    if (int rc = list_geometry(what, n, k)) return rc;
    if (int rc = check_step_size(opt)) return rc;
    v.list = vr::RayList{rays->origins, rays->dirs, n};
    v.is_list = true;
    return VR_OK;
}

template <typename Launch>
int march_launch(vr_tree_t t, LaunchKind kind, const Views& v, const VrRenderOptions* opt, vr::KParams& k, void* stream,
                 Launch&& launch) {
    fill_march_params(k, opt);
    k.offscreen = 1;
    k.layout = VR_LAYOUT_FRAME;
    k.pitch = (int64_t)k.width * 4;
    return run_launch(t, kind, v, false, k, stream, [&](const Turn& u) -> int {
        if (int rc = enqueue_tables(u.k, v, u.hs)) return rc;
        HIP_TRY(launch(u));
        return VR_OK;
    });
}

int weights_launch(vr_tree_t t, const Views& v, const VrRenderOptions* opt, int fp_mode, const VrLeafWeights* out,
                   vr::KParams& k, void* stream) {
    return march_launch(t, LaunchKind::kWeights, v, opt, k, stream, [&](const Turn& u) {
        vr::WeightParams w;
        w.max_weight = reinterpret_cast<uint32_t*>(out->max_weight);
        w.hits = out->hits;
        w.file_node = t->file_node_dev.get<int32_t>();
        return vr::launch_weights(u.k, w, fp_mode, t->n_cus, u.tn.waves_per_cu, u.gen_waves, u.tn.weights_check != 0,
                                  u.hs, v.rays());
    });
}


int check_backward_options(const char* what, const VrRenderOptions* opt) {
    if (opt->render_depth)
        return fail(VR_ERR_UNSUPPORTED, "%s with render_depth: the depth visualisation has no derivative here", what);
    if (opt->enable_probe)
        return fail(VR_ERR_UNSUPPORTED, "%s with enable_probe: pixels under the probe disc are not traced", what);
    if (!(opt->rot_dirs[0] == 0.f) || !(opt->rot_dirs[1] == 0.f) || !(opt->rot_dirs[2] == 0.f))
        return fail(VR_ERR_UNSUPPORTED, "%s with rot_dirs: the view direction is not rotated", what);
    return VR_OK;
}

int validate_backward(const char* what, vr_tree_t t, int n_frames, const VrCamera* cams, const VrRenderOptions* opt,
                      int fp_mode, const float* grad_accum, const float* grad_data, vr::KParams& k) {
    if (!t || !opt || !grad_accum || !grad_data || (n_frames > 0 && !cams))
        return fail(VR_ERR_INVALID_ARGUMENT, "NULL argument");
    if (int rc = validate_march(n_frames, cams, opt, fp_mode, k)) return rc;
    return check_backward_options(what, opt);
}

int check_backward_tree(const VrTreeOpaque* t, const VrRenderOptions* opt, const char* what) {
    const int format = t->desc.format, basis_dim = t->desc.basis_dim;
    if (format == VR_FORMAT_SG || format == VR_FORMAT_ASG)
        return fail(VR_ERR_UNSUPPORTED, "%s: SG / ASG trees are not supported", what);
    if (vr::basis_flavour(format, basis_dim) != vr::BASIS_RGBA &&
        (opt->basis_minmax[0] > 0 || opt->basis_minmax[1] < basis_dim - 1))
        return fail(VR_ERR_UNSUPPORTED, "%s: basis_minmax [%d, %d] leaves out basis functions of the tree (%d)", what,
                    opt->basis_minmax[0], opt->basis_minmax[1], basis_dim);
    return VR_OK;
}

int backward_launch(const char* what, vr_tree_t t, const Views& v, const VrRenderOptions* opt, int fp_mode,
                    const float* grad_accum, float* grad_data, uint32_t* touched, vr::KParams& k, void* stream) {
    if (int rc = check_backward_tree(t, opt, what)) return rc;
    return march_launch(t, LaunchKind::kBackward, v, opt, k, stream, [&](const Turn& u) {
        vr::GradParams g;
        g.grad_accum = grad_accum;
        g.grad_data = grad_data;
        g.file_node = t->file_node_dev.get<int32_t>();
        g.touched = touched;
        return vr::launch_grad(u.k, g, fp_mode, t->n_cus, u.tn.waves_per_cu, u.gen_waves, u.hs, v.rays());
    });
}

int backward_rays(const char* what, vr_tree_t t, int64_t n, const VrRays* rays, const VrRenderOptions* opt,
                  int fp_mode, const float* grad_accum, float* grad_data, uint32_t* touched, void* stream) {
    vr::KParams k;
    memset(&k, 0, sizeof(k));
    Views v;
    if (!grad_accum) return fail(VR_ERR_INVALID_ARGUMENT, "%s: NULL argument", what);
    if (int rc = validate_rays(what, t, n, rays, opt, fp_mode, grad_data, k, v)) return rc;
    if (int rc = check_backward_options(what, opt)) return rc;
    return backward_launch(what, t, v, opt, fp_mode, grad_accum, grad_data, touched, k, stream);
}

}

extern "C" {

int vr_render_backward(vr_tree_t t, int n_frames, const VrCamera* cams, const VrRenderOptions* opt, int fp_mode,
                       const float* grad_accum, float* grad_data, void* stream) {
    vr::KParams k;
    memset(&k, 0, sizeof(k));
    if (int rc = validate_backward("vr_render_backward", t, n_frames, cams, opt, fp_mode, grad_accum, grad_data, k)) return rc;
    return backward_launch("vr_render_backward", t, Views{cams, n_frames}, opt, fp_mode, grad_accum, grad_data, nullptr,
                           k, stream);
}

int vr_render_backward_touched(vr_tree_t t, int n_frames, const VrCamera* cams, const VrRenderOptions* opt, int fp_mode,
                               const float* grad_accum, float* grad_data, uint32_t* touched, void* stream) {
    vr::KParams k;
    memset(&k, 0, sizeof(k));
    if (!touched) return fail(VR_ERR_INVALID_ARGUMENT, "vr_render_backward_touched: NULL argument");
    if (int rc = validate_backward("vr_render_backward_touched", t, n_frames, cams, opt, fp_mode, grad_accum, grad_data, k))
        return rc;
    return backward_launch("vr_render_backward_touched", t, Views{cams, n_frames}, opt, fp_mode, grad_accum, grad_data,
                           touched, k, stream);
}

int vr_render_backward_rays(vr_tree_t t, int64_t n, const VrRays* rays, const VrRenderOptions* opt, int fp_mode,
                            const float* grad_accum, float* grad_data, void* stream) {
    return backward_rays("vr_render_backward_rays", t, n, rays, opt, fp_mode, grad_accum, grad_data, nullptr, stream);
}

int vr_render_backward_rays_touched(vr_tree_t t, int64_t n, const VrRays* rays, const VrRenderOptions* opt, int fp_mode,
                                    const float* grad_accum, float* grad_data, uint32_t* touched, void* stream) {
    if (!touched) return fail(VR_ERR_INVALID_ARGUMENT, "vr_render_backward_rays_touched: NULL argument");
    return backward_rays("vr_render_backward_rays_touched", t, n, rays, opt, fp_mode, grad_accum, grad_data, touched,
                         stream);
}

int vr_accumulate_weights(vr_tree_t t, int n_frames, const VrCamera* cams, const VrRenderOptions* opt,
                          int fp_mode, const VrLeafWeights* out, void* stream) {
    vr::KParams k;
    memset(&k, 0, sizeof(k));
    if (int rc = validate_weights(t, n_frames, cams, opt, fp_mode, out, k)) return rc;
    return weights_launch(t, Views{cams, n_frames}, opt, fp_mode, out, k, stream);
}

int vr_accumulate_weights_rays(vr_tree_t t, int64_t n, const VrRays* rays, const VrRenderOptions* opt, int fp_mode,
                               const VrLeafWeights* out, void* stream) {
    vr::KParams k;
    memset(&k, 0, sizeof(k));
    Views v;
    if (int rc = validate_rays("vr_accumulate_weights_rays", t, n, rays, opt, fp_mode, out, k, v)) return rc;
    if (!out->max_weight && !out->hits)
        return fail(VR_ERR_INVALID_ARGUMENT, "vr_accumulate_weights_rays: both outputs are NULL");
    return weights_launch(t, v, opt, fp_mode, out, k, stream);
}

int vr_render_rays(vr_tree_t t, int64_t n, const VrRays* rays, const VrRenderOptions* opt, int fp_mode,
                   const VrRayOut* out, void* stream) {
    vr::KParams k;
    memset(&k, 0, sizeof(k));
    Views v;
    if (int rc = validate_rays("vr_render_rays", t, n, rays, opt, fp_mode, out, k, v)) return rc;
    if (!out->rgba && !out->accum) return fail(VR_ERR_INVALID_ARGUMENT, "vr_render_rays: both outputs are NULL");
    if (opt->render_depth)
        return fail(VR_ERR_UNSUPPORTED, "vr_render_rays with render_depth: the depth visualisation is not what a ray list is for");
    if (opt->enable_probe)
        return fail(VR_ERR_UNSUPPORTED, "vr_render_rays with enable_probe: the probe disc is a set of pixel positions");
    if (n == 0) return VR_OK;
    VrFrame f;
    memset(&f, 0, sizeof(f));
    f.offscreen = 1;
    f.layout = VR_LAYOUT_FRAME;
    f.fp_mode = fp_mode;
    f.accum = out->accum;
    fill_caller_params(k, opt, &f);
    k.any_accum = out->accum ? 1 : 0;
    return run_launch(t, LaunchKind::kColour, v, !out->rgba, k, stream, [&](const Turn& u) -> int {
        f.rgba = out->rgba ? out->rgba : u.pixel_words;
        if (int rc = enqueue_tables(u.k, v, u.hs, &f)) return rc;
        HIP_TRY(vr::launch_render(u.k, fp_mode, t->n_cus, u.tn.waves_per_cu, u.gen_waves, u.hs, v.rays()));
        return VR_OK;
    });
}

int vr_render_batch(vr_tree_t t, int n_frames, const VrCamera* cams, const VrRenderOptions* opt,
                    const VrFrame* frames, void* stream) {
    return render_launch(t, n_frames, cams, opt, frames, nullptr, 0, false, stream);
}

int vr_render_aov(vr_tree_t t, int n_frames, const VrCamera* cams, const VrRenderOptions* opt,
                  const VrFrame* frames, const VrAov* aovs, int depth_units, void* stream) {
    return render_launch(t, n_frames, cams, opt, frames, aovs, depth_units, true, stream);
}

int vr_render(vr_tree_t t, const VrCamera* cam, const VrRenderOptions* opt, const VrFrame* f,
              void* stream) {
    return vr_render_batch(t, 1, cam, opt, f, stream);
}

}
```

volrend_amd/csrc/vr_launch_plan.h:

```cpp
#pragma once
#include <cstdint>

#pragma GCC visibility push(hidden)

struct Tuning {
    int march_max = 12;
    int refill_min = 20;
    int drain_flush = 16;
    int waves_per_cu = 0;
    int frame_group = 0;
    int super_block = 0;
    int records_nt = -1;
    int xcd_queues = 1;
    int chunk_max = 0;
    int raygen_waves = 0;
    int top_levels = 0;
    int brick_levels = 3;
    int brick_blocked = -1;
    int max_iter = 1 << 22;
    int weights_check = 1;
};

enum class LaunchKind { kColour, kAov, kWeights, kBackward };
enum class RaySource { kFrames, kList };

constexpr int kPlanQueues = 8;

struct LaunchPlan {
    int chunk_max, super_block, records_nt, frame_group, n_queues;
    int raygen_waves;
};

LaunchPlan plan_launch(LaunchKind kind, RaySource source, int n_frames, int64_t list_rays, const Tuning& tn,
                       uint64_t lookup_bytes);

#pragma GCC visibility pop
```

volrend_amd/csrc/vr_render.hip:

```cpp
#ifndef VR_KERNEL_PASS_AOV
#include "vr_device_math.h"
#include "vr_internal.h"
#include "vr_dev_layout.h"
#include "vr_dev_shade.h"
#include "vr_dev_query.h"
#include "vr_dev_rays.h"

namespace vr {

namespace {

constexpr int kSh16Waves = 5;
constexpr int kSh25Waves = 4;
constexpr int kSh9Waves = 7;
constexpr int kSh16Rows = 64;

constexpr int kRing = 128;

template <int BASIS>
struct Stage {
    static constexpr bool kEnabled = BASIS > 1;
    static constexpr int kVec = kEnabled ? RecTraits<BASIS>::kDwords / 4 : 1;
    static constexpr int kRow = kVec * 16;
    static constexpr int kPerInstr = kWave / kVec;
    static constexpr int kPass = !kEnabled ? kWave
                                 : (kRow * kWave <= 5504 ? kWave
                                    : (BASIS == BASIS_16 ? kSh16Rows : kWave / 2));
    static constexpr int kPasses = (BASIS == BASIS_25) ? 2 : 1;
    static constexpr int kShade = kPass * kPasses;
    static constexpr int kInstr = (kPass + kPerInstr - 1) / kPerInstr;
    static constexpr int kBytes = (kEnabled && kPass * kRow > 768) ? kPass * kRow : 768;
};
typedef __attribute__((address_space(1))) const void* vr_gptr_t;
typedef __attribute__((address_space(3))) void* vr_lptr_t;
constexpr int kOwnerQ = 4;

template <int BASIS, bool NT, int RING = kRing>
__device__ __forceinline__ void issue_records(const KParams& p, char* stage, const uint32_t* it_leaf,
                                              uint32_t ring_head, int lane, int n, int pass) {
    using ST = Stage<BASIS>;
#pragma unroll
    for (int k = 0; k < ST::kInstr; ++k) {
        const int rin = k * ST::kPerInstr + lane / ST::kVec;
        const int item = pass * ST::kPass + rin;
        if (lane < ST::kPerInstr * ST::kVec && rin < ST::kPass && item < n) {
            const uint32_t leaf = it_leaf[(ring_head + (uint32_t)item) & (RING - 1)];
            const char* src = reinterpret_cast<const char*>(p.leaves) +
                              (uint64_t)leaf * (uint32_t)(p.leaf_stride_h * 2) + (lane % ST::kVec) * 16;
            __builtin_amdgcn_global_load_lds(
                (vr_gptr_t)src,
                (vr_lptr_t)((__attribute__((address_space(3))) char*)stage + k * ST::kPerInstr * ST::kRow),
                16, 0, NT ? 2  : 0);
        }
    }
}

template <int BASIS, int MODE>
constexpr int min_waves_per_eu() {
    if (MODE != MODE_FAST) return BASIS == BASIS_25 ? 3 : 4;
    return BASIS == BASIS_25 ? kSh25Waves : BASIS == BASIS_16 ? kSh16Waves : BASIS == BASIS_9 ? kSh9Waves : 8;
}
template <int BASIS, int MODE>
constexpr bool aov_depth_in_lds() {
    return MODE == MODE_FAST && (BASIS == BASIS_9 || BASIS == BASIS_16 || BASIS == BASIS_25);
}
template <int BASIS, int MODE, bool AOV = false>
constexpr int waves_per_cu() {
    const int lds = ((kRing * 9 + kWave * 4 + (AOV && aov_depth_in_lds<BASIS, MODE>() ? kWave * 4 : 0) +
                      Stage<BASIS>::kBytes + 511) / 512) * 512;
    const int by_lds = 163840 / lds, by_reg = 4 * min_waves_per_eu<BASIS, MODE>();
    return by_lds < by_reg ? by_lds : by_reg;
}

__device__ __forceinline__ void store_aov(const AovParams& a, int frame, uint32_t xy, float d, float tr) {
    const AovDesc pl = a.planes[frame];
    const int64_t off = (int64_t)(xy >> 16) * a.pitch + (int64_t)(xy & 0xFFFFu) * 4;
    typedef __attribute__((address_space(1))) float vr_gfloat_t;
    if (pl.depth) *(vr_gfloat_t*)(reinterpret_cast<char*>(pl.depth) + off) = d;
    if (pl.transmittance) *(vr_gfloat_t*)(reinterpret_cast<char*>(pl.transmittance) + off) = tr;
}

template <int FMA, bool FULL>
__device__ __forceinline__ void store_colour_ray(const KParams& p, uint32_t slot, const Ray& nr, uint32_t xy,
                                                 uint8_t* px, int frame, const float* vdir) {
    uint32_t* rb = ray_slot(p.ray_buf_rw, kRayWords + p.ray_tail_words, slot);
#pragma unroll
    for (int i = 0; i < 3; ++i) {
        ray_word(rb, kRayCen + i) = f2u(nr.cen[i]);
        ray_word(rb, kRayDir + i) = f2u(nr.dir[i]);
        ray_word(rb, kRayInvDir + i) = f2u(nr.invdir[i]);
    }
    ray_word(rb, kRayT) = f2u(nr.t);
    ray_word(rb, kRayTmax) = f2u(nr.tmax);
    ray_word(rb, kRayDeltaScale) = f2u(nr.delta_scale);
    ray_word(rb, kRayXy) = xy;
    ray_word(rb, kRayPixelLo) = (uint32_t)reinterpret_cast<uint64_t>(px);
    ray_word(rb, kRayPixelHi) = (uint32_t)(reinterpret_cast<uint64_t>(px) >> 32);
    ray_word(rb, kRayFrame) = (uint32_t)frame;
    if (p.ray_vdir) {
#pragma unroll
        for (int i = 0; i < 3; ++i) ray_word(rb, kRayTail + i) = f2u(vdir[i]);
    } else if (p.basis_words > 0) {
        float b[VR_MAX_BASIS];
#pragma unroll
        for (int i = 0; i < VR_MAX_BASIS; ++i) b[i] = 0.f;
        precalc_basis<FMA, FULL>(p, vdir, b);
#pragma unroll
        for (int i = 0; i < VR_MAX_BASIS; ++i)
            if (i < p.basis_words)
                ray_word(rb, kRayTail + i) = f2u((i < p.basis_min || i > p.basis_max) ? 0.f : b[i]);
    }
}

#define VR_RENDER_KERNEL render_kernel
#define VR_RAYGEN_KERNEL raygen_kernel
#define VR_KERNEL_ARGS const KParams p
#define VR_KERNEL_AOV false
#define VR_KERNEL_AOV_LOCAL const AovParams aov{};
#endif

template <int FMA, int BASIS, int MODE, bool BLK = false>
__global__ __launch_bounds__(kWave, (min_waves_per_eu<BASIS, MODE>())) void VR_RENDER_KERNEL(VR_KERNEL_ARGS) {
    constexpr bool AOV = VR_KERNEL_AOV;
    VR_KERNEL_AOV_LOCAL
    using P = Policy<FMA>;
    constexpr bool N2 = MODE != MODE_GENERIC;
    constexpr bool LOBES = MODE != MODE_FAST;
    constexpr bool COUNT = MODE != MODE_FAST;
    constexpr int NB = BASIS > 1 ? BASIS : 1;
    constexpr bool HAS_BASIS = BASIS != BASIS_RGBA;
    using ST = Stage<BASIS>;
    __shared__ uint32_t it_leaf[kRing];
    __shared__ float it_w[kRing];
    __shared__ uint8_t it_own[kRing];
    __shared__ __attribute__((aligned(16))) char stage[ST::kBytes];
    float* const res = reinterpret_cast<float*>(stage);
    float mybasis[NB];
#pragma unroll
    for (int i = 0; i < NB; ++i) mybasis[i] = 0.f;

    const int lane = threadIdx.x & (kWave - 1);
    Ray ray;
    ray.active = false;
    ray.alive = ray.entered = ray.stopped = false;
    __shared__ uint32_t ray_ids[kWave];
    ray.t = 0.f;
    ray.tmax = -1.f;
    ray.light = 1.f;
    ray.delta_scale = 1.f;
#pragma unroll
    for (int i = 0; i < 3; ++i) {
        ray.cen[i] = 0.f;
        ray.dir[i] = 0.f;
        ray.invdir[i] = 1.f;
    }
    ray.out[0] = ray.out[1] = ray.out[2] = ray.out[3] = 0.f;
    RayCounters rc;
    Cursor cur;
    uint32_t qpos = 0;
    uint32_t qsh = 32;
    uint32_t rounds = 0, progress_round = 0;
    bool exhausted = false;
    uint32_t chunk_next = 0, chunk_end = 0;
    uint32_t ring_head = 0, ring_tail = 0;
    const int wpr = kRayWords + p.ray_tail_words;
    uint32_t st_march_r = 0, st_march_l = 0, st_shade_r = 0, st_shade_l = 0, st_distinct = 0,
             st_fin_r = 0, st_fin_l = 0, st_iter = 0;
    constexpr bool D_LDS = AOV && aov_depth_in_lds<BASIS, MODE>();
    float d_reg = 0.f;
    float* d_lds = nullptr;
    if constexpr (D_LDS) {
        __shared__ float d_words[kWave];
        d_lds = d_words;
    }
    auto depth_get = [&]() -> float {
        if constexpr (D_LDS) return d_lds[lane_id_now()];
        else return d_reg;
    };
    auto depth_set = [&](float v) {
        if constexpr (D_LDS) d_lds[lane_id_now()] = v;
        else d_reg = v;
    };

    auto shade_chunk = [&](int n) {
        __syncthreads();
        if (COUNT) {
            st_shade_r++;
            st_shade_l += (uint32_t)n;
            const uint32_t myleaf =
                lane < n ? it_leaf[(ring_head + (uint32_t)lane) & (kRing - 1)] : 0xFFFFFFFFu;
            bool first = lane < n;
            for (int o = 0; o < kWave; ++o) {
                const uint32_t other = (uint32_t)__shfl((int)myleaf, o);
                if (o < lane && other == myleaf) first = false;
            }
            st_distinct += (uint32_t)__builtin_popcountll(__builtin_amdgcn_ballot_w64(first));
            if (lane < n)
                touch(p, TOUCH_LEAVES, (uint64_t)myleaf * (uint32_t)(p.leaf_stride_h * 2),
                      (uint32_t)(2 * (p.data_dim - 1)));
        }
        const bool have = lane < n;
        const uint32_t jmine = (ring_head + (uint32_t)lane) & (kRing - 1);
        const float weight = have ? it_w[jmine] : 0.f;
        const int own4 = (HAS_BASIS && have) ? (int)it_own[jmine] << 2 : lane << 2;
        auto basis_of = [&](int i) -> float {
            return u2f((uint32_t)__builtin_amdgcn_ds_bpermute(own4, (int)f2u(mybasis[i])));
        };
        float bfull[ST::kPasses > 1 ? NB : 1];
        if constexpr (ST::kPasses > 1) {
#pragma unroll
            for (int i = 0; i < NB; ++i) bfull[i] = basis_of(i);
        }
        auto basis_get = [&](int i) -> float {
            if constexpr (ST::kPasses > 1) return bfull[i];
            else return basis_of(i);
        };
        float r0 = 0.f, r1 = 0.f, r2 = 0.f;
        if constexpr (ST::kEnabled) {
#pragma unroll
            for (int pass = 0; pass < ST::kPasses; ++pass) {
                if (pass * ST::kPass < n) {
                    if (p.records_nt)
                        issue_records<BASIS, true>(p, stage, it_leaf, ring_head, lane, n, pass);
                    else
                        issue_records<BASIS, false>(p, stage, it_leaf, ring_head, lane, n, pass);
                    __syncthreads();
                    if (ST::kPasses == 1 || lane / ST::kPass == pass) {
                        const char* row = stage + (lane % ST::kPass) * ST::kRow;
                        float acc[3];
                        channel_sums<FMA, BASIS>(row, basis_get, acc);
                        const float2v e01 = vr_expf2((float2v){-acc[0], -acc[1]}) + splat2(1.f);
                        r0 = weight / e01.x;
                        r1 = weight / e01.y;
                        r2 = weight / (1.f + vr_expf(-acc[2]));
                    }
                    if (ST::kPasses > 1) __syncthreads();
                }
            }
        } else {
          const float b0 = HAS_BASIS ? basis_of(0) : 0.f;
          if (have) {
            Record<BASIS> rec;
            load_record<BASIS>(p, it_leaf[jmine], rec);
            if (HAS_BASIS) {
                r0 = weight / (1.f + vr_expf(-(b0 * rec.at(0))));
                r1 = weight / (1.f + vr_expf(-(b0 * rec.at(1))));
                r2 = weight / (1.f + vr_expf(-(b0 * rec.at(2))));
            } else {
                r0 = rec.at(0);
                r1 = rec.at(1);
                r2 = rec.at(2);
            }
          }
        }
        __syncthreads();
        if (have) {
            res[0 * kWave + lane] = r0;
            res[1 * kWave + lane] = r1;
            res[2 * kWave + lane] = r2;
        }
        __syncthreads();
        const uint32_t head8 = ring_head & 0xFFu;
#pragma unroll
        for (int d = 0; d < kOwnerQ; ++d) {
            const uint32_t pos = __builtin_amdgcn_ubfe(qpos, qsh, 8u);
            const uint32_t idx = (pos - head8) & 0xFFu;
            if (qsh < 32u && idx < (uint32_t)n) {
                if (HAS_BASIS) {
                    ray.out[0] += res[0 * kWave + idx];
                    ray.out[1] += res[1 * kWave + idx];
                    ray.out[2] += res[2 * kWave + idx];
                } else {
                    const float w = it_w[pos & (kRing - 1)];
                    ray.out[0] = P::madd(res[0 * kWave + idx], w, ray.out[0]);
                    ray.out[1] = P::madd(res[1 * kWave + idx], w, ray.out[1]);
                    ray.out[2] = P::madd(res[2 * kWave + idx], w, ray.out[2]);
                }
                qsh += 8u;
            }
        }
        ring_head += (uint32_t)n;
    };

    for (;;) {
        const bool done = ray.active && !(ray.t < ray.tmax) && qsh == 32u;
        const unsigned long long m_done = __builtin_amdgcn_ballot_w64(done);
        const unsigned long long m_free = __builtin_amdgcn_ballot_w64(!ray.active);
        const unsigned long long m_busy =
            __builtin_amdgcn_ballot_w64(ray.active && (ray.t < ray.tmax || qsh < 32u));
        const int n_avail = __builtin_popcountll(m_done | m_free);
        if (COUNT) st_iter++;
        if (n_avail > 0 && (m_busy == 0ull || (!exhausted && n_avail >= p.refill_min))) {
            if (COUNT && m_done != 0ull) {
                st_fin_r++;
                st_fin_l += (uint32_t)__builtin_popcountll(m_done);
            }
            uint32_t px_lo = 0, px_hi = 0, fin_xy = 0, fin_frame = 0;
            float fin_d = 0.f;
            ray.stopped = ray.tmax < 0.f;
            if (done) {
                const uint32_t* rs = ray_slot(p.ray_buf, wpr, ray_ids[lane_id_now()]);
                px_lo = ray_word(rs, kRayPixelLo);
                px_hi = ray_word(rs, kRayPixelHi);
                if (COUNT || p.any_accum || AOV) {
                    fin_xy = ray_word(rs, kRayXy);
                    fin_frame = ray_word(rs, kRayFrame);
                }
                if constexpr (AOV) {
                    fin_d = depth_get();
                    if (aov.depth_world) fin_d = fin_d * ray.delta_scale;
                }
            }
            const bool vacant = done || !ray.active;
            bool take = false;
            if (m_done != 0ull) progress_round = (uint32_t)__builtin_amdgcn_readfirstlane((int)rounds);
            if (!exhausted && chunk_next >= chunk_end) {
                uint32_t lo, hi;
                grab_chunk(p, lane, lo, hi);
                lo = __builtin_amdgcn_readfirstlane(lo);
                hi = __builtin_amdgcn_readfirstlane(hi);
                if (hi == lo) {
                    exhausted = true;
                } else {
                    chunk_next = lo;
                    chunk_end = hi;
                }
            }
            if (!exhausted) {
                const unsigned long long idle = m_done | m_free;
                const uint32_t r = chunk_next + lane_rank(idle);
                const uint32_t c_end = chunk_end;
                const uint32_t left = chunk_end - chunk_next;
                chunk_next += (uint32_t)n_avail < left ? (uint32_t)n_avail : left;
                if (vacant && r < c_end) {
                    take = true;
                    const uint32_t* rs = ray_slot(p.ray_buf, wpr, r);
#pragma unroll
                    for (int i = 0; i < 3; ++i) {
                        ray.cen[i] = u2f(ray_word(rs, kRayCen + i));
                        ray.dir[i] = u2f(ray_word(rs, kRayDir + i));
                        ray.invdir[i] = u2f(ray_word(rs, kRayInvDir + i));
                    }
                    ray.t = u2f(ray_word(rs, kRayT));
                    ray.tmax = u2f(ray_word(rs, kRayTmax));
                    ray.delta_scale = u2f(ray_word(rs, kRayDeltaScale));
                    ray_ids[lane_id_now()] = r;
                    if (HAS_BASIS) {
                        if (BASIS > 1 && p.ray_vdir) {
                            float vd[3];
#pragma unroll
                            for (int i = 0; i < 3; ++i) vd[i] = u2f(ray_word(rs, kRayTail + i));
                            precalc_basis<FMA, false, (BASIS > 1 ? BASIS : 1)>(p, vd, mybasis);
#pragma unroll
                            for (int i = 0; i < NB; ++i)
                                if (i < p.basis_min || i > p.basis_max) mybasis[i] = 0.f;
                        } else {
#pragma unroll
                            for (int i = 0; i < NB; ++i)
                                mybasis[i] = u2f(ray_word(rs, kRayTail + i));
                        }
                    }
                }
            }
            if (done)
                finish_ray<FMA, COUNT>(
                    p, ray, rc,
                    reinterpret_cast<uint8_t*>(((uint64_t)px_hi << 32) | (uint64_t)px_lo), fin_xy,
                    (int)fin_frame);
            if constexpr (AOV) {
                if (done) store_aov(aov, (int)fin_frame, fin_xy, fin_d, ray.light);
                if (vacant) depth_set(0.f);
            }
            if (vacant) {
                ray.active = ray.entered = take;
                if (!take) {
                    ray.t = 0.f;
                    ray.tmax = -1.f;
                }
                ray.out[0] = ray.out[1] = ray.out[2] = ray.out[3] = 0.f;
                ray.light = 1.f;
                rc = RayCounters();
                cur = Cursor();
                qsh = 32u;
                qpos = 0;
            }
        }
        if (!wave_any(ray.active)) {
            if (exhausted) break;
            continue;
        }

        if (rounds - progress_round >= (uint32_t)p.max_iter) {
            if (ray.t < ray.tmax) {
                ray.t = ray.tmax;
                if (p.status) atomicOr(p.status, 1u);
            }
            progress_round = rounds;
        }
        int m = 0;
        for (; m < p.march_max; ++m) {
            const unsigned long long m_go = __builtin_amdgcn_ballot_w64(ray.t < ray.tmax) &
                                            __builtin_amdgcn_ballot_w64(qsh != 0u);
            if (m_go == 0ull) break;
            const bool go = ray.t < ray.tmax && qsh != 0u;
            if (COUNT) {
                st_march_r++;
                st_march_l += (uint32_t)__builtin_popcountll(__builtin_amdgcn_ballot_w64(go));
            }
            bool push = false;
            uint32_t leaf = 0;
            float weight = 0.f;
            if (go) {
                float pos[3];
                pos[0] = P::madd(ray.t, ray.dir[0], ray.cen[0]);
                pos[1] = P::madd(ray.t, ray.dir[1], ray.cen[1]);
                pos[2] = P::madd(ray.t, ray.dir[2], ray.cen[2]);
                float cube_sz = 0.f;
                int levels;
                uint32_t word;
                if (N2) {
                    leaf = query_n2<COUNT, (MODE == MODE_FAST ? (BLK ? 1 : 0) : -1)>(p, pos, &levels, &word, cur);
                } else {
                    leaf = (uint32_t)query_generic<FMA, COUNT>(p, pos, &cube_sz, &levels, &word);
                }
                if (COUNT) {
                    rc.samples++;
                    rc.child_reads += (uint32_t)levels;
                }
                const float dda = dda_unit<FMA>(pos, ray.invdir);
                const float t_subcube =
                    N2 ? __builtin_amdgcn_ldexpf(dda, -levels) : dda / cube_sz;
                const float delta_t = t_subcube + p.step_size;
                const float sigma = h2f((uint16_t)(word & 0xFFFFu));
                bool stop = false;
                if (sigma > p.sigma_thresh) {
                    if (COUNT) rc.hits++;
                    const float att = vr_expf_nonan(-delta_t * ray.delta_scale * sigma);
                    weight = ray.light * (1.f - att);
                    if constexpr (AOV) depth_set(P::madd(weight, ray.t, depth_get()));
                    if (COUNT && p.render_depth)
                        ray.out[0] = P::madd(weight, ray.t, ray.out[0]);
                    else
                        push = true;
                    ray.light *= att;
                    stop = ray.light < p.stop_thresh;
                }
                if (stop) {
                    ray.tmax = -1.f;
                    if (COUNT) rc.early++;
                } else {
                    ray.t += delta_t;
                }
            }
            const unsigned long long m_push = __builtin_amdgcn_ballot_w64(push);
            if (m_push != 0ull) {
                if (push) {
                    const uint32_t seq = ring_tail + lane_rank(m_push);
                    const uint32_t j = seq & (kRing - 1);
                    it_leaf[j] = leaf;
                    it_w[j] = weight;
                    it_own[j] = (uint8_t)lane;
                    qpos = __builtin_amdgcn_alignbit(seq, qpos, 8u);
                    qsh -= 8u;
                }
                ring_tail += (uint32_t)__builtin_popcountll(m_push);
                while (ring_tail - ring_head >= (uint32_t)ST::kShade) shade_chunk(ST::kShade);
            }
            if (exhausted) {
                const unsigned long long m_alive = __builtin_amdgcn_ballot_w64(ray.t < ray.tmax);
                if (__builtin_popcountll(m_alive) <= p.drain_flush &&
                    (m_alive & __builtin_amdgcn_ballot_w64(qsh == 0u)) != 0ull && ring_tail != ring_head) {
                    const uint32_t waiting = ring_tail - ring_head;
                    shade_chunk(waiting < (uint32_t)ST::kShade ? (int)waiting : ST::kShade);
                }
            }
        }
        rounds = (uint32_t)__builtin_amdgcn_readfirstlane((int)(rounds + (uint32_t)m));
        while (ring_tail != ring_head && !wave_any(ray.t < ray.tmax && qsh > 0u)) {
            const uint32_t waiting = ring_tail - ring_head;
            shade_chunk(waiting < (uint32_t)ST::kShade ? (int)waiting : ST::kShade);
        }
    }
    if (COUNT && p.sched_stats && lane == 0) {
        atomicAdd(&p.sched_stats[kStatMarchRounds], (unsigned long long)st_march_r);
        atomicAdd(&p.sched_stats[kStatMarchLanes], (unsigned long long)st_march_l);
        atomicAdd(&p.sched_stats[kStatShadeRounds], (unsigned long long)st_shade_r);
        atomicAdd(&p.sched_stats[kStatShadeLanes], (unsigned long long)st_shade_l);
        atomicAdd(&p.sched_stats[kStatDistinctLeaves], (unsigned long long)st_distinct);
        atomicAdd(&p.sched_stats[kStatRetireRounds], (unsigned long long)st_fin_r);
        atomicAdd(&p.sched_stats[kStatRetiredRays], (unsigned long long)st_fin_l);
        atomicAdd(&p.sched_stats[kStatIterations], (unsigned long long)st_iter);
    }
}



template <int FMA, bool FULL, int GW>
__global__ __launch_bounds__(kWave* GW) void VR_RAYGEN_KERNEL(VR_KERNEL_ARGS) {
    constexpr bool AOV = VR_KERNEL_AOV;
    VR_KERNEL_AOV_LOCAL
    const int lane = threadIdx.x & (kWave - 1);
    const int wave = threadIdx.x >> 6;
    const uint32_t id =
        (uint32_t)(((int64_t)blockIdx.x * GW + wave) * kWave + lane);
    bool valid = false;
    Ray nr;
    uint8_t* px = nullptr;
    uint32_t xy = 0;
    int frame = 0;
    float vdir[3] = {0.f, 0.f, 1.f};
    if (id < p.total_rays) {
        const PixelRef r = locate(p, id);
        if (r.in_image) {
            frame = r.frame;
            xy = (uint32_t)r.x | ((uint32_t)r.y << 16);
            px = pixel_ptr(p, p.frames[r.frame], r);
            setup_ray<FMA>(p, r, nr, vdir);
            if (nr.alive) {
                valid = true;
            } else {
                RayCounters z;
                finish_ray<FMA, FULL>(p, nr, z, px, xy, frame);
                if constexpr (AOV) store_aov(aov, frame, xy, 0.f, 1.f);
            }
        }
    }
    const unsigned long long m_valid = __builtin_amdgcn_ballot_w64(valid);
    const uint32_t my_base = reserve_ray_slots<GW>(p, m_valid, lane, wave);
    if (!valid) return;
    const uint32_t slot = my_base + lane_rank(m_valid);
    uint32_t* rb = ray_slot(p.ray_buf_rw, kRayWords + p.ray_tail_words, slot);
#pragma unroll
    for (int i = 0; i < 3; ++i) {
        ray_word(rb, kRayCen + i) = f2u(nr.cen[i]);
        ray_word(rb, kRayDir + i) = f2u(nr.dir[i]);
        ray_word(rb, kRayInvDir + i) = f2u(nr.invdir[i]);
    }
    ray_word(rb, kRayT) = f2u(nr.t);
    ray_word(rb, kRayTmax) = f2u(nr.tmax);
    ray_word(rb, kRayDeltaScale) = f2u(nr.delta_scale);
    ray_word(rb, kRayXy) = xy;
    ray_word(rb, kRayPixelLo) = (uint32_t)reinterpret_cast<uint64_t>(px);
    ray_word(rb, kRayPixelHi) = (uint32_t)(reinterpret_cast<uint64_t>(px) >> 32);
    ray_word(rb, kRayFrame) = (uint32_t)frame;
    if (p.ray_vdir) {
#pragma unroll
        for (int i = 0; i < 3; ++i) ray_word(rb, kRayTail + i) = f2u(vdir[i]);
    } else if (p.basis_words > 0) {
        float b[VR_MAX_BASIS];
#pragma unroll
        for (int i = 0; i < VR_MAX_BASIS; ++i) b[i] = 0.f;
        precalc_basis<FMA, FULL>(p, vdir, b);
#pragma unroll
        for (int i = 0; i < VR_MAX_BASIS; ++i)
            if (i < p.basis_words)
                ray_word(rb, kRayTail + i) = f2u((i < p.basis_min || i > p.basis_max) ? 0.f : b[i]);
    }
}

#ifndef VR_KERNEL_PASS_AOV
#undef VR_RENDER_KERNEL
#undef VR_RAYGEN_KERNEL
#undef VR_KERNEL_ARGS
#undef VR_KERNEL_AOV
#undef VR_KERNEL_AOV_LOCAL
#define VR_KERNEL_PASS_AOV
#define VR_RENDER_KERNEL render_aov_kernel
#define VR_RAYGEN_KERNEL raygen_aov_kernel
#define VR_KERNEL_ARGS const KParams p, const AovParams aov
#define VR_KERNEL_AOV true
#define VR_KERNEL_AOV_LOCAL
#include "vr_render.hip"
#undef VR_KERNEL_PASS_AOV
#undef VR_RENDER_KERNEL
#undef VR_RAYGEN_KERNEL
#undef VR_KERNEL_ARGS
#undef VR_KERNEL_AOV
#undef VR_KERNEL_AOV_LOCAL

template <int FMA, bool FULL, int GW>
__global__ __launch_bounds__(kWave* GW) void raygen_rays_kernel(const KParams p, const RayList rl) {
    const int lane = threadIdx.x & (kWave - 1);
    const int wave = threadIdx.x >> 6;
    uint32_t id;
    Ray nr;
    float vdir[3] = {0.f, 0.f, 1.f};
    const bool has = list_ray<FMA, GW>(p, rl, lane, wave, id, nr, vdir);
    bool valid = false;
    uint8_t* px = nullptr;
    uint32_t xy = 0;
    if (has) {
        xy = (id & (uint32_t)(kRayListWidth - 1)) | ((id >> kRayListShift) << 16);
        px = p.frames[0].rgba + (int64_t)id * 4;
        if (nr.alive) {
            valid = true;
        } else {
            RayCounters z;
            finish_ray<FMA, false>(p, nr, z, px, xy, 0);
        }
    }
    const unsigned long long m_valid = __builtin_amdgcn_ballot_w64(valid);
    const uint32_t my_base = reserve_ray_slots<GW>(p, m_valid, lane, wave);
    if (!valid) return;
    store_colour_ray<FMA, FULL>(p, my_base + lane_rank(m_valid), nr, xy, px, 0, vdir);
}

__global__ void prepare_launch_kernel(FrameTable tbl, FrameDesc* frames, uint32_t* queue_head) {
    const int i = threadIdx.x;
    if (i < tbl.n) frames[tbl.first + i] = tbl.f[i];
    if (tbl.first == 0 && i < kMaxQueues) {
        queue_head[i * kQueueStride + kQueueHead] = 0u;
        queue_head[i * kQueueStride + kQueueCount] = 0u;
    }
}

__global__ void prepare_aov_kernel(AovTable tbl, AovDesc* planes) {
    const int i = threadIdx.x;
    if (i < tbl.n) planes[tbl.first + i] = tbl.f[i];
}

template <int FMA>
__global__ void probe_overlay_kernel(const KParams p) {
    using P = Policy<FMA>;
    const int side = p.probe_disp_size + 5;
    const int idx = blockIdx.x * blockDim.x + threadIdx.x;
    if (idx >= side * side) return;
    const int y = idx / side;
    const int x = p.width - side + (idx - y * side);
    if (x < 0 || x >= p.width || y >= p.height) return;
    const int tx = x / p.tile_w, ty = y / p.tile_h;
    const int tile = ty * p.tiles_x + tx;
    if (tile % p.world != p.rank) return;
    float cen[3], dir[3], out[4] = {0.f, 0.f, 0.f, 0.f};
    const int xx = x - (p.width - p.probe_disp_size) + 5;
    const int yy = y - 5;
    cen[0] = -((float)xx / (0.5f * (float)p.probe_disp_size) - 1.f);
    cen[1] = ((float)yy / (0.5f * (float)p.probe_disp_size) - 1.f);
    const float c = P::madd(cen[0], cen[0], cen[1] * cen[1]);
    if (!(c <= 1.f)) return;
    if (p.basis_dim >= 0) {
        float basis_fn[VR_MAX_BASIS];
#pragma unroll
        for (int i = 0; i < VR_MAX_BASIS; ++i) basis_fn[i] = 0.f;
        cen[2] = -__builtin_sqrtf(1 - c);
        float xf[9];
        for (int i = 0; i < 9; ++i) xf[i] = p.frames[blockIdx.y].xf[i];
        mv3<FMA>(xf, cen, dir);
        precalc_basis<FMA, true>(p, dir, basis_fn);
        int hi = p.basis_max;
        if (hi > p.basis_dim - 1) hi = p.basis_dim - 1;
        const int lo = p.basis_min < 0 ? 0 : p.basis_min;
        for (int tt = 0; tt < 3; ++tt) {
            const int off = tt * p.basis_dim;
            float tmp = 0.f;
            for (int i = lo; i <= hi; ++i) tmp = P::madd(basis_fn[i], p.probe_coeffs[off + i], tmp);
            out[tt] = 1.f / (1.f + vr_expf(-tmp));
        }
    } else {
        for (int i = 0; i < 3; ++i) out[i] = p.probe_coeffs[i];
    }
    out[3] = 1.f;
    const int64_t pix = (int64_t)y * p.width + x;
    const FrameDesc& fd = p.frames[blockIdx.y];
    if (fd.accum) reinterpret_cast<float4*>(fd.accum)[pix] = make_float4(out[0], out[1], out[2], out[3]);
    uint8_t* const px = pixel_address(p, fd, tile / p.world, x - tx * p.tile_w, y - ty * p.tile_h, x, y);
    *reinterpret_cast<uint32_t*>(px) =
        quant8(out[0]) | (quant8(out[1]) << 8) | (quant8(out[2]) << 16) | 0xFF000000u;
}

__global__ void probe_kernel(const KParams p, float probe0, float probe1, float probe2,
                             float* out) {
    float cen[3] = {p.offset[0] + p.scale[0] * probe0, p.offset[1] + p.scale[1] * probe1,
                    p.offset[2] + p.scale[2] * probe2};
    float cube_sz;
    int levels;
    uint32_t word;
    const int64_t leaf = query_generic<0>(p, cen, &cube_sz, &levels, &word);
    const uint16_t* v = p.leaves + leaf * p.leaf_stride_h;
    for (int i = threadIdx.x; i < p.data_dim - 1; i += blockDim.x) out[i] = h2f(v[i]);
}

bool needs_full(const KParams& p) {
    return p.format == VR_FORMAT_SG || p.format == VR_FORMAT_ASG || p.instrumented || p.render_depth;
}

template <int FMA, int MODE, bool AOV>
hipError_t launch_basis(const KParams& p, const AovParams& a, int64_t total_blocks, int n_cus, int waves_override,
                        hipStream_t s) {
    const dim3 block(kWave);
#define VR_LAUNCH(B)                                                                         \
    do {                                                                                     \
        const dim3 grid(persistent_grid(total_blocks, n_cus,                                 \
                                        waves_override > 0 ? waves_override : waves_per_cu<B, MODE, AOV>())); \
        constexpr bool kBlk = MODE == MODE_FAST;                                             \
        if constexpr (AOV) {                                                                 \
            if (kBlk && p.brick_blocked)                                                     \
                hipLaunchKernelGGL((render_aov_kernel<FMA, B, MODE, kBlk>), grid, block, 0, s, p, a); \
            else                                                                             \
                hipLaunchKernelGGL((render_aov_kernel<FMA, B, MODE, false>), grid, block, 0, s, p, a); \
        } else if (kBlk && p.brick_blocked)                                                  \
            hipLaunchKernelGGL((render_kernel<FMA, B, MODE, kBlk>), grid, block, 0, s, p);   \
        else                                                                                 \
            hipLaunchKernelGGL((render_kernel<FMA, B, MODE, false>), grid, block, 0, s, p);  \
    } while (0)
    switch (basis_flavour(p.format, p.basis_dim)) {
        case BASIS_RGBA: VR_LAUNCH(BASIS_RGBA); break;
        case BASIS_25: VR_LAUNCH(BASIS_25); break;
        case BASIS_16: VR_LAUNCH(BASIS_16); break;
        case BASIS_9: VR_LAUNCH(BASIS_9); break;
        case BASIS_4: VR_LAUNCH(BASIS_4); break;
        default: VR_LAUNCH(BASIS_1); break;
    }
#undef VR_LAUNCH
    return hipGetLastError();
}

template <int FMA, bool AOV>
hipError_t launch_fp(const KParams& p, const AovParams& a, int64_t total_blocks, int n_cus, int waves_override,
                     hipStream_t s) {
    if (!uses_lookup(p)) return launch_basis<FMA, MODE_GENERIC, AOV>(p, a, total_blocks, n_cus, waves_override, s);
    if (needs_full(p)) return launch_basis<FMA, MODE_FULL, AOV>(p, a, total_blocks, n_cus, waves_override, s);
    return launch_basis<FMA, MODE_FAST, AOV>(p, a, total_blocks, n_cus, waves_override, s);
}

template <bool AOV>
hipError_t launch_march(const KParams& p, const AovParams& a, int fp_mode, int n_cus, int waves_override,
                        int gen_waves, hipStream_t stream, const RayList* rays = nullptr) {
    const int64_t total_blocks = p.n_wave_blocks * p.n_frames;
    {
        const bool full = needs_full(p);
#define VR_GEN(FMA_, FULL_, GW_)                                                                    \
    do {                                                                                            \
        const dim3 grid_((unsigned)((total_blocks + GW_ - 1) / GW_)), block_(kWave * GW_);          \
        if constexpr (AOV) hipLaunchKernelGGL((raygen_aov_kernel<FMA_, FULL_, GW_>), grid_, block_, 0, stream, p, a); \
        else if (rays) {                                                                            \
            if constexpr (GW_ >= 4) hipLaunchKernelGGL((raygen_rays_kernel<FMA_, FULL_, GW_>), grid_, block_, 0, stream, p, *rays); \
        }                                                                                           \
        else hipLaunchKernelGGL((raygen_kernel<FMA_, FULL_, GW_>), grid_, block_, 0, stream, p);    \
    } while (0)
#define VR_GEN_GW(FMA_, FULL_)                                                                      \
    do {                                                                                            \
        if (gen_waves >= 16) VR_GEN(FMA_, FULL_, 16);                                               \
        else if (gen_waves >= 4 || rays) VR_GEN(FMA_, FULL_, 4);             \
        else VR_GEN(FMA_, FULL_, 1);                                                                \
    } while (0)
        if (fp_mode == VR_FP_FMA) {
            if (full) VR_GEN_GW(1, true); else VR_GEN_GW(1, false);
        } else {
            if (full) VR_GEN_GW(0, true); else VR_GEN_GW(0, false);
        }
#undef VR_GEN_GW
#undef VR_GEN
    }
    return fp_mode == VR_FP_FMA ? launch_fp<1, AOV>(p, a, total_blocks, n_cus, waves_override, stream)
                                : launch_fp<0, AOV>(p, a, total_blocks, n_cus, waves_override, stream);
}

}

hipError_t launch_prepare(const KParams& p, const FrameTable& tbl, hipStream_t stream) {
    hipLaunchKernelGGL(prepare_launch_kernel, dim3(1), dim3(64), 0, stream, tbl,
                       const_cast<FrameDesc*>(p.frames), p.queue_head);
    return hipGetLastError();
}

hipError_t launch_render(const KParams& p, int fp_mode, int n_cus, int waves_override, int gen_waves,
                         hipStream_t stream, const RayList* rays) {
    if (p.n_wave_blocks <= 0 || p.n_frames <= 0) return hipSuccess;
    const hipError_t e = launch_march<false>(p, AovParams{}, fp_mode, n_cus, waves_override, gen_waves, stream, rays);
    if (e != hipSuccess || !p.enable_probe || p.probe_disp_size <= 0) return e;
    const int side = p.probe_disp_size + 5;
    const dim3 pgrid((unsigned)((side * side + 255) / 256), (unsigned)p.n_frames);
    if (fp_mode == VR_FP_FMA)
        hipLaunchKernelGGL(probe_overlay_kernel<1>, pgrid, dim3(256), 0, stream, p);
    else
        hipLaunchKernelGGL(probe_overlay_kernel<0>, pgrid, dim3(256), 0, stream, p);
    return hipGetLastError();
}

hipError_t launch_prepare_aov(const AovParams& a, const AovTable& tbl, hipStream_t stream) {
    hipLaunchKernelGGL(prepare_aov_kernel, dim3(1), dim3(64), 0, stream, tbl, const_cast<AovDesc*>(a.planes));
    return hipGetLastError();
}

hipError_t launch_render_aov(const KParams& p, const AovParams& a, int fp_mode, int n_cus, int waves_override,
                             int gen_waves, hipStream_t stream) {
    if (p.n_wave_blocks <= 0 || p.n_frames <= 0) return hipSuccess;
    return launch_march<true>(p, a, fp_mode, n_cus, waves_override, gen_waves, stream);
}

hipError_t launch_probe(const KParams& p, const float probe[3], float* out_dev,
                        hipStream_t stream) {
    hipLaunchKernelGGL(probe_kernel, dim3(1), dim3(64), 0, stream, p, probe[0], probe[1],
                       probe[2], out_dev);
    return hipGetLastError();
}

}
#endif
```

volrend_amd/csrc/vr_slots.cpp:

```cpp
#include <hip/hip_runtime.h>

#include <mutex>

#include "vr_host.h"

namespace {

hipError_t replace_ray_buffer(LaunchSlot& ls, size_t bytes) {
    if (ls.rays) {
        if (ls.used) (void)hipEventSynchronize(ls.done.get());
        (void)ls.rays.reset();
        (void)hipGetLastError();
    }
    return ls.rays.alloc(bytes);
}

int reserve_slots(VrTreeOpaque* t, int n_slots, size_t need) {
    DeviceGuard device_guard(t->device);
    std::lock_guard<std::mutex> guard(t->launch_mutex);
    for (int i = 0; i < n_slots; ++i) {
        LaunchSlot& ls = t->slots[i];
        if (ls.growing || ls.rays.bytes() >= need) continue;
        const hipError_t e = replace_ray_buffer(ls, need);
        if (e != hipSuccess) return fail(hip_code(e), "ray buffer of %zu bytes: %s", need, hipGetErrorString(e));
    }
    return VR_OK;
}

size_t colour_record_bytes(const VrTreeOpaque* t, uint32_t total_rays) {
    const int flavour = vr::basis_flavour(t->desc.format, t->desc.basis_dim);
    return ray_buffer_bytes(total_rays, vr::kRayWords + vr::ray_tail_words(t->desc.format, flavour));
}

}

int acquire_slot(VrTreeOpaque* t, std::unique_lock<std::mutex>& guard, hipStream_t hs, vr::KParams& k,
                 size_t need, unsigned& slot) {
    slot = kLaunchSlots;
    for (int want_fit = 1; want_fit >= 0 && slot == kLaunchSlots; --want_fit) {
        for (int pass = 0; pass < 2 && slot == kLaunchSlots; ++pass)
            for (unsigned i = 0; i < kLaunchSlots; ++i) {
                const LaunchSlot& c = t->slots[i];
                if (c.growing || (want_fit && c.rays.bytes() < need)) continue;
                const bool ok = pass == 0 ? (c.used && c.last_stream == hs)
                                          : (!c.used || hipEventQuery(c.done.get()) == hipSuccess);
                if (ok) {
                    slot = i;
                    break;
                }
            }
    }
    (void)hipGetLastError();
    if (slot == kLaunchSlots) {
        for (unsigned a = 0; a < kLaunchSlots && slot == kLaunchSlots; ++a)
            if (!t->slots[(t->launch_seq + a) % kLaunchSlots].growing) slot = (t->launch_seq + a) % kLaunchSlots;
        if (slot == kLaunchSlots)
            return fail(VR_ERR_HIP, "all %u launch slots are being resized by other threads", kLaunchSlots);
    }
    t->launch_seq++;
    LaunchSlot& ls = t->slots[slot];
    k.frames = t->slot_frames.get<vr::FrameDesc>() + (size_t)slot * vr::kMaxBatch;
    k.queue_head = t->slot_heads.get<uint32_t>() + vr::kSlotWords * slot + vr::kSlotHeaderWords;
    k.probe_coeffs = t->probe_buf.get<float>() + (size_t)slot * (size_t)t->desc.data_dim;
    if (ls.rays.bytes() < need) {
        ls.growing = true;
        guard.unlock();
        const hipError_t ge = replace_ray_buffer(ls, need);
        guard.lock();
        ls.growing = false;
        if (ge != hipSuccess)
            return fail(hip_code(ge), "ray buffer of %zu bytes: %s", need, hipGetErrorString(ge));
    }
    k.ray_buf_rw = ls.rays.get<uint32_t>();
    k.ray_buf = k.ray_buf_rw;
    return VR_OK;
}

int SlotTurn::begin(LaunchSlot& ls, hipStream_t hs) {
    if (ls.used) HIP_TRY(hipStreamWaitEvent(hs, ls.done.get(), 0));
    slot_ = &ls;
    stream_ = hs;
    return VR_OK;
}

SlotTurn::~SlotTurn() {
    if (!slot_) return;
    if (hipEventRecord(slot_->done.get(), stream_) == hipSuccess) {
        slot_->used = true;
        slot_->last_stream = stream_;
    } else {
        (void)hipGetLastError();
    }
}

extern "C" {

int vr_reserve_rays(vr_tree_t t, int64_t n, int n_slots) {
    if (!t) return fail(VR_ERR_INVALID_ARGUMENT, "vr_reserve_rays: tree is NULL");
    if (n_slots < 1 || n_slots > (int)kLaunchSlots)
        return fail(VR_ERR_INVALID_ARGUMENT, "vr_reserve_rays: n_slots=%d outside [1,%u]", n_slots, kLaunchSlots);
    vr::KParams geo;
    if (int rc = list_geometry("vr_reserve_rays", n, geo)) return rc;
    return reserve_slots(t, n_slots, colour_record_bytes(t, geo.total_rays) + list_pixel_bytes(geo.total_rays));
}

int vr_reserve_tiles(vr_tree_t t, int width, int height, int n_frames, int tile_w, int tile_h,
                     int world, int n_slots) {
    if (!t) return fail(VR_ERR_INVALID_ARGUMENT, "tree is NULL");
    if (n_frames < 1 || n_frames > VR_MAX_BATCH)
        return fail(VR_ERR_INVALID_ARGUMENT, "vr_reserve(%d x %d, %d frames) out of range", width,
                    height, n_frames);
    if (n_slots < 1 || n_slots > (int)kLaunchSlots)
        return fail(VR_ERR_INVALID_ARGUMENT, "n_slots=%d outside [1,%u]", n_slots, kLaunchSlots);
    vr::KParams geo;
    if (int rc = launch_geometry(width, height, tile_w, tile_h, 0, world, n_frames, geo)) return rc;
    return reserve_slots(t, n_slots, colour_record_bytes(t, geo.total_rays));
}

int vr_reserve(vr_tree_t t, int width, int height, int n_frames) {
    return vr_reserve_tiles(t, width, height, n_frames, 0, 0, 1, 2);
}

}
```

volrend_amd/csrc/vr_tree_kernels.hip:

```cpp
#include "vr_internal.h"
#include "vr_dev_layout.h"

namespace vr {

namespace {

__global__ void assemble_kernel(uint8_t* frame, int64_t pitch, const uint8_t* gathered, int width,
                                int height, int tile_w, int tile_h, int tiles_x, int world,
                                int64_t out_stride, int64_t rank_stride, int64_t in_stride) {
    const int x = blockIdx.x * blockDim.x + threadIdx.x;
    const int y = blockIdx.y * blockDim.y + threadIdx.y;
    if (x >= width || y >= height) return;
    frame += (int64_t)blockIdx.z * out_stride;
    gathered += (int64_t)blockIdx.z * in_stride;
    const int tx = x / tile_w, ty = y / tile_h;
    const int tile = ty * tiles_x + tx;
    const int rank = tile % world;
    const int64_t k = tile / world;
    const int lx = x - tx * tile_w, ly = y - ty * tile_h;
    const int64_t src = (k * tile_w * tile_h + (int64_t)ly * tile_w + lx);
    *reinterpret_cast<uint32_t*>(frame + (int64_t)y * pitch + (int64_t)x * 4) =
        reinterpret_cast<const uint32_t*>(gathered + (int64_t)rank * rank_stride)[src];
}

__global__ void relayout_nodes_kernel(const int32_t* child, const uint16_t* data,
                                      const int32_t* perm, uint32_t* nodes, int64_t n_slots,
                                      int N3, int data_dim) {
    const int64_t i = (int64_t)blockIdx.x * blockDim.x + threadIdx.x;
    if (i >= n_slots) return;
    const int64_t n = i / N3;
    const int s = (int)(i - n * N3);
    const int32_t skip = child[i];
    const int64_t target = n + skip;
    uint32_t w;
    if (skip == 0 || target <= 0 || target >= n_slots / N3) {
        w = kLeafBit | (uint32_t)data[i * data_dim + (data_dim - 1)];
    } else {
        w = (uint32_t)perm[target];
    }
    nodes[(int64_t)perm[n] * N3 + s] = w;
}

__global__ void relayout_leaves_kernel(const uint16_t* data, const int32_t* perm, uint16_t* leaves,
                                       int64_t n_slots, int N3, int data_dim, int stride_h) {
    const int chunks = stride_h / 8;
    const int64_t gid = (int64_t)blockIdx.x * blockDim.x + threadIdx.x;
    const int64_t slot = gid / chunks;
    if (slot >= n_slots) return;
    const int c = (int)(gid - slot * chunks);
    const uint16_t* src = data + slot * data_dim;
    uint16_t h[8];
#pragma unroll
    for (int j = 0; j < 8; ++j) {
        const int e = c * 8 + j;
        h[j] = e < data_dim - 1 ? src[e] : (uint16_t)0;
    }
    uint4 q;
    q.x = h[0] | ((uint32_t)h[1] << 16);
    q.y = h[2] | ((uint32_t)h[3] << 16);
    q.z = h[4] | ((uint32_t)h[5] << 16);
    q.w = h[6] | ((uint32_t)h[7] << 16);
    const int64_t n = slot / N3;
    const int64_t dst = (int64_t)perm[n] * N3 + (slot - n * N3);
    reinterpret_cast<uint4*>(leaves + dst * stride_h)[c] = q;
}

__global__ void decode_quant_kernel(const uint16_t* __restrict__ colors,
                                    const uint16_t* __restrict__ map,
                                    const uint16_t* __restrict__ sigma,
                                    const uint16_t* __restrict__ retained,
                                    uint16_t* __restrict__ data, int64_t n_slots, int n_quant,
                                    int n_ret, int data_dim) {
    const int n_basis = n_quant + n_ret;
    const int64_t total = n_slots * n_basis;
    for (int64_t w = (int64_t)blockIdx.x * blockDim.x + threadIdx.x; w < total;
         w += (int64_t)gridDim.x * blockDim.x) {
        const int64_t slot = w / n_basis;
        const int j = (int)(w - slot * n_basis);
        const uint16_t* c;
        if (j < n_ret) {
            c = retained + ((int64_t)j * n_slots + slot) * 3;
        } else {
            const int q = j - n_ret;
            c = colors + ((int64_t)q * 65536 + map[(int64_t)q * n_slots + slot]) * 3;
        }
        uint16_t* o = data + slot * data_dim + j;
        o[0] = c[0];
        o[n_basis] = c[1];
        o[2 * n_basis] = c[2];
        if (j == 0) data[slot * data_dim + data_dim - 1] = sigma[slot];
    }
}

__global__ void popcount_kernel(const uint32_t* words, uint64_t n_words, unsigned long long* out) {
    unsigned long long acc = 0;
    for (uint64_t i = (uint64_t)blockIdx.x * blockDim.x + threadIdx.x; i < n_words;
         i += (uint64_t)gridDim.x * blockDim.x)
        acc += (unsigned long long)__builtin_popcount(words[i]);
    for (int o = 32; o > 0; o >>= 1) acc += __shfl_down(acc, o);
    if ((threadIdx.x & 63) == 0 && acc) atomicAdd(out, acc);
}

__global__ void build_top_kernel(const uint32_t* nodes, const int32_t* brick_root, int n_bricks,
                                 uint2* top, int G0, uint32_t* error_flag) {
    const uint32_t cell = blockIdx.x * blockDim.x + threadIdx.x;
    if (cell >= (1u << (3 * G0))) return;
    const uint32_t mask = (1u << G0) - 1u;
    const uint32_t cx = (cell >> (2 * G0)) & mask, cy = (cell >> G0) & mask, cz = cell & mask;
    uint32_t node = 0;
    for (int l = 0; l < G0; ++l) {
        const int sh = G0 - 1 - l;
        const uint32_t slot = (((cx >> sh) & 1u) << 2) | (((cy >> sh) & 1u) << 1) | ((cz >> sh) & 1u);
        const uint32_t w = nodes[(uint64_t)node * 8u + slot];
        if (w & kLeafBit) {
            top[cell] = make_uint2(kLeafBit | ((uint32_t)(l + 1) << 16) | (w & 0xFFFFu),
                                   node * 8u + slot);
            return;
        }
        node = w;
    }
    int lo = 0, hi = n_bricks - 1, found = -1;
    while (lo <= hi) {
        const int mid = (lo + hi) >> 1;
        const uint32_t r = (uint32_t)brick_root[mid];
        if (r == node) {
            found = mid;
            break;
        }
        if (r < node) lo = mid + 1; else hi = mid - 1;
    }
    if (found < 0) {
        atomicOr(error_flag, 1u);
        found = 0;
    }
    top[cell] = make_uint2((uint32_t)found, node);
}

__global__ void build_bricks_kernel(const uint32_t* nodes, const int32_t* brick_root, int n_bricks,
                                    uint32_t* bricks, int BL, int blocked, uint32_t* error_flag) {
    const uint64_t gid = (uint64_t)blockIdx.x * blockDim.x + threadIdx.x;
    const uint32_t per = 1u << (3 * BL);
    if (gid >= (uint64_t)n_bricks * per) return;
    const uint32_t b = (uint32_t)(gid >> (3 * BL)), e = (uint32_t)gid & (per - 1u);
    const uint32_t mask = (1u << BL) - 1u;
    uint32_t ex = (e >> (2 * BL)) & mask, ey = (e >> BL) & mask, ez = e & mask;
    if (blocked) {
        ex = (((e >> 8) & 1u) << 2) | ((e >> 3) & 3u);
        ey = (((e >> 7) & 1u) << 2) | ((e >> 1) & 3u);
        ez = (((e >> 5) & 3u) << 1) | (e & 1u);
    }
    const uint32_t root = (uint32_t)brick_root[b];
    uint32_t node = root;
    for (int k = 0; k < BL; ++k) {
        const int sh = BL - 1 - k;
        const uint32_t slot = (((ex >> sh) & 1u) << 2) | (((ey >> sh) & 1u) << 1) | ((ez >> sh) & 1u);
        const uint32_t w = nodes[(uint64_t)node * 8u + slot];
        if (w & kLeafBit) {
            const uint32_t delta = node - root;
            if (delta > 1023u) atomicOr(error_flag, 2u);
            bricks[gid] = kLeafBit | ((uint32_t)k << 29) | ((delta & 1023u) << 19) | (slot << 16) |
                          (w & 0xFFFFu);
            return;
        }
        node = w;
    }
    bricks[gid] = node;
}

}

hipError_t launch_assemble(uint8_t* frame, int64_t pitch, const uint8_t* gathered, int width,
                           int height, int tile_w, int tile_h, int world, int n_frames,
                           int64_t out_stride, int64_t rank_stride, int64_t in_stride,
                           hipStream_t stream) {
    const int tiles_x = (width + tile_w - 1) / tile_w;
    const dim3 block(64, 4);
    const dim3 grid((width + 63) / 64, (height + 3) / 4, n_frames);
    hipLaunchKernelGGL(assemble_kernel, grid, block, 0, stream, frame, pitch, gathered, width,
                       height, tile_w, tile_h, tiles_x, world, out_stride, rank_stride, in_stride);
    return hipGetLastError();
}

int leaf_stride_halfs(int data_dim) {
    const int bytes = 2 * (data_dim - 1);
    int stride = 16;
    while (stride < bytes && stride < 128) stride *= 2;
    if (stride < bytes) stride = (bytes + 31) / 32 * 32;
    return stride / 2;
}

hipError_t launch_relayout(const int32_t* child, const uint16_t* data, const int32_t* perm,
                           uint32_t* nodes, uint16_t* leaves, int64_t n_slots, int N3,
                           int data_dim, int stride_h, hipStream_t stream) {
    const int tpb = 256;
    hipLaunchKernelGGL(relayout_nodes_kernel, dim3((unsigned)((n_slots + tpb - 1) / tpb)), dim3(tpb),
                       0, stream, child, data, perm, nodes, n_slots, N3, data_dim);
    const int64_t n_chunks = n_slots * (stride_h / 8);
    hipLaunchKernelGGL(relayout_leaves_kernel, dim3((unsigned)((n_chunks + tpb - 1) / tpb)),
                       dim3(tpb), 0, stream, data, perm, leaves, n_slots, N3, data_dim, stride_h);
    return hipGetLastError();
}

hipError_t launch_build_lookup(const uint32_t* nodes, const int32_t* brick_root, int n_bricks,
                               uint2* top, uint32_t* bricks, int top_levels, int brick_levels,
                               int brick_blocked, uint32_t* error_flag, hipStream_t stream) {
    const uint32_t n_cells = 1u << (3 * top_levels);
    hipLaunchKernelGGL(build_top_kernel, dim3((n_cells + 255) / 256), dim3(256), 0, stream, nodes,
                       brick_root, n_bricks, top, top_levels, error_flag);
    if (n_bricks > 0 && brick_levels > 0) {
        const uint64_t n = (uint64_t)n_bricks << (3 * brick_levels);
        hipLaunchKernelGGL(build_bricks_kernel, dim3((unsigned)((n + 255) / 256)), dim3(256), 0,
                           stream, nodes, brick_root, n_bricks, bricks, brick_levels,
                           (brick_blocked && brick_levels == 3) ? 1 : 0, error_flag);
    }
    return hipGetLastError();
}

hipError_t launch_popcount(const uint32_t* words, uint64_t n_words, unsigned long long* out,
                           hipStream_t stream) {
    if (n_words == 0) return hipSuccess;
    uint64_t blocks = (n_words + 255) / 256;
    if (blocks > 4096) blocks = 4096;
    hipLaunchKernelGGL(popcount_kernel, dim3((unsigned)blocks), dim3(256), 0, stream, words, n_words,
                       out);
    return hipGetLastError();
}

hipError_t launch_decode_quant(const uint16_t* colors, const uint16_t* map, const uint16_t* sigma,
                               const uint16_t* retained, uint16_t* data, int64_t n_slots,
                               int n_quant, int n_ret, int data_dim, hipStream_t stream) {
    hipError_t e = hipMemsetAsync(data, 0, (size_t)n_slots * data_dim * sizeof(uint16_t), stream);
    if (e != hipSuccess) return e;
    const int64_t total = n_slots * (int64_t)(n_quant + n_ret);
    const int tpb = 256;
    int64_t blocks = (total + tpb - 1) / tpb;
    if (blocks > (1 << 20)) blocks = 1 << 20;
    hipLaunchKernelGGL(decode_quant_kernel, dim3((unsigned)blocks), dim3(tpb), 0, stream, colors,
                       map, sigma, retained, data, n_slots, n_quant, n_ret, data_dim);
    return hipGetLastError();
}

}
```

volrend_amd/csrc/vr_upload.cpp:

```cpp
#include <hip/hip_runtime.h>

#include <algorithm>
#include <chrono>
#include <cstdio>
#include <cstdlib>
#include <future>
#include <memory>
#include <mutex>
#include <new>
#include <vector>

#include "vr_h2d.h"
#include "vr_host.h"
#include "vr_tree_walk.h"

namespace {

int check_quant(const VrTreeDesc* d, const VrQuantDesc* q) {
    if (q->n_quant < 0 || q->n_retained < 0 || q->n_quant + q->n_retained < 1)
        return fail(VR_ERR_INVALID_ARGUMENT, "quantised tree needs at least one basis function");
    if (3 * (q->n_quant + q->n_retained) + 1 > d->data_dim)
        return fail(VR_ERR_INVALID_ARGUMENT, "%d quantised + %d retained basis functions do not "
                    "fit data_dim=%d", q->n_quant, q->n_retained, d->data_dim);
    if (!q->sigma) return fail(VR_ERR_INVALID_ARGUMENT, "sigma is NULL");
    if (q->n_quant && (!q->quant_colors || !q->quant_map))
        return fail(VR_ERR_INVALID_ARGUMENT, "quant_colors/quant_map is NULL");
    if (q->n_retained && !q->data_retained)
        return fail(VR_ERR_INVALID_ARGUMENT, "data_retained is NULL");
    return VR_OK;
}

hipError_t decode_quant_on_device(const VrTreeDesc* d, const VrQuantDesc* q, size_t n_slots,
                                  uint16_t* d_data, int device) {
    const void* src[4] = {q->quant_colors, q->quant_map, q->sigma, q->data_retained};
    const size_t sz[4] = {(size_t)q->n_quant * 65536 * 3 * sizeof(uint16_t), (size_t)q->n_quant * n_slots * sizeof(uint16_t),
                          n_slots * sizeof(uint16_t), (size_t)q->n_retained * n_slots * 3 * sizeof(uint16_t)};
    DeviceBuffer tmp[4];
    const void* dev[4] = {nullptr, nullptr, nullptr, nullptr};
    hipError_t e = hipSuccess;
    CopySegment segs[4];
    int n_seg = 0;
    for (int i = 0; i < 4 && e == hipSuccess; ++i) {
        if (!sz[i]) continue;
        if (d->memory == 1) {
            dev[i] = src[i];
            continue;
        }
        e = tmp[i].alloc(sz[i]);
        segs[n_seg++] = CopySegment{tmp[i].get(), src[i], sz[i]};
        dev[i] = tmp[i].get();
    }
    if (e == hipSuccess && n_seg) e = staged_h2d_multi(segs, n_seg, device);
    if (e == hipSuccess)
        e = vr::launch_decode_quant((const uint16_t*)dev[0], (const uint16_t*)dev[1],
                                    (const uint16_t*)dev[2], (const uint16_t*)dev[3], d_data,
                                    (int64_t)n_slots, q->n_quant, q->n_retained, d->data_dim,
                                    nullptr);
    if (e == hipSuccess) e = hipDeviceSynchronize();
    return e;
}

int check_tree_desc(const VrTreeDesc* d, bool need_data) {
    if (!d->child || (need_data && !d->data))
        return fail(VR_ERR_INVALID_ARGUMENT, "child/data is NULL");
    if (d->N < 2 || d->N > 16) return fail(VR_ERR_INVALID_ARGUMENT, "N=%d out of range", d->N);
    if (d->capacity <= 0) return fail(VR_ERR_INVALID_ARGUMENT, "capacity must be positive");
    if (d->format < VR_FORMAT_RGBA || d->format > VR_FORMAT_ASG)
        return fail(VR_ERR_INVALID_ARGUMENT, "unknown data format %d", d->format);
    const int min_dim = d->format == VR_FORMAT_RGBA ? 4 : 3 * d->basis_dim + 1;
    if (d->format != VR_FORMAT_RGBA && (d->basis_dim < 1 || d->basis_dim > VR_MAX_BASIS))
        return fail(VR_ERR_INVALID_ARGUMENT, "basis_dim=%d out of range [1,%d]", d->basis_dim,
                    VR_MAX_BASIS);
    if (d->data_dim < min_dim)
        return fail(VR_ERR_INVALID_ARGUMENT, "data_dim=%d too small for the format (need %d)",
                    d->data_dim, min_dim);
    if (d->format == VR_FORMAT_SG && (!d->extra || d->extra_count < (uint64_t)d->basis_dim * 4))
        return fail(VR_ERR_INVALID_ARGUMENT, "SG needs basis_dim*4 extra floats");
    if (d->format == VR_FORMAT_ASG && (!d->extra || d->extra_count < (uint64_t)d->basis_dim * 11))
        return fail(VR_ERR_INVALID_ARGUMENT, "ASG needs basis_dim*11 extra floats");
    return VR_OK;
}

hipError_t alloc_launch_scratch(VrTreeOpaque* t) {
    hipError_t e = t->status.alloc(sizeof(uint32_t));
    if (e == hipSuccess) e = hipMemset(t->status.get(), 0, sizeof(uint32_t));
    if (e == hipSuccess) e = t->sched_stats.alloc(vr::kSchedStats * sizeof(unsigned long long));
    if (e == hipSuccess) e = hipMemset(t->sched_stats.get(), 0, vr::kSchedStats * sizeof(unsigned long long));
    if (e == hipSuccess) e = t->probe_buf.alloc(sizeof(float) * (size_t)t->desc.data_dim * kLaunchSlots);
    for (unsigned i = 0; i < kLaunchSlots && e == hipSuccess; ++i) e = t->slots[i].done.create();
    if (e == hipSuccess) e = t->slot_frames.alloc(sizeof(vr::FrameDesc) * vr::kMaxBatch * kLaunchSlots);
    if (e == hipSuccess) e = t->slot_heads.alloc(sizeof(uint32_t) * vr::kSlotWords * kLaunchSlots);
    if (e == hipSuccess) e = t->slot_aovs.alloc(sizeof(vr::AovDesc) * vr::kMaxBatch * kLaunchSlots);
    int cus = 0;
    if (e == hipSuccess && hipDeviceGetAttribute(&cus, hipDeviceAttributeMultiprocessorCount, t->device) == hipSuccess &&
        cus > 0)
        t->n_cus = cus;
    return e;
}


struct UploadJob {
    const VrTreeDesc* d;
    const VrQuantDesc* q;
    const int32_t* host_child;
    int N3;
    size_t n_slots, child_sz, data_sz;
    bool from_host;
    bool timing;
    std::chrono::steady_clock::time_point t_start;
    void mark(const char* what) const {
        const std::chrono::duration<double, std::milli> ms = std::chrono::steady_clock::now() - t_start;
        if (timing) fprintf(stderr, "[volrend_hip] upload: %s at %.1f ms\n", what, ms.count());
    }
};

int check_upload_args(const VrTreeDesc* d, const VrQuantDesc* q, vr_tree_t* out) {
    if (!d || !out) return fail(VR_ERR_INVALID_ARGUMENT, "desc/out is NULL");
    *out = nullptr;
    if (int rc = check_tree_desc(d, q == nullptr)) return rc;
    return q ? check_quant(d, q) : VR_OK;
}

int fetch_child_words(UploadJob& j, std::vector<int32_t>& fetched) {
    if (j.from_host) return VR_OK;
    fetched.resize(j.n_slots);
    HIP_TRY(hipMemcpy(fetched.data(), j.d->child, j.child_sz, hipMemcpyDeviceToHost));
    j.host_child = fetched.data();
    return VR_OK;
}

struct Walk {
    int max_depth = -1;
    std::vector<uint8_t> level;
    char why[256] = "";
};
std::shared_future<Walk> start_walk(const UploadJob& j) {
    return std::async(std::launch::async, [&j] {
        Walk w;
        w.max_depth = validate_topology(j.host_child, j.d->capacity, j.N3, w.level, w.why, sizeof(w.why));
        j.mark("topology checked");
        return w;
    }).share();
}

struct Staged {
    hipError_t e = hipSuccess;
    DeviceBuffer child, data;
};
std::future<Staged> start_copies(const UploadJob& j, hipError_t e_dev, int device,
                                 std::shared_future<Walk> walk) {
    return std::async(std::launch::async, [&j, e_dev, device, walk] {
        Staged s;
        hipError_t& e = s.e;
        if ((e = e_dev) != hipSuccess) return s;
        e = hipSetDevice(device);
        if (j.from_host && e == hipSuccess) e = s.child.alloc(j.child_sz);
        if ((j.q || j.from_host) && e == hipSuccess) e = s.data.alloc(j.data_sz);
        if (j.from_host && e == hipSuccess) warm_upload_cache(device);
        j.mark("runtime + buffers ready");
        if (walk.get().max_depth < 0) return s;
        const CopySegment both[2] = {{s.child.get(), j.d->child, j.child_sz},
                                     {s.data.get(), j.d->data, j.data_sz}};
        if (j.q) {
            if (e == hipSuccess && j.from_host) e = staged_h2d_multi(both, 1, device);
            if (e == hipSuccess) e = decode_quant_on_device(j.d, j.q, j.n_slots, s.data.get<uint16_t>(), device);
        } else if (j.from_host && e == hipSuccess) {
            e = staged_h2d_multi(both, 2, device);
        }
        j.mark("copies done");
        return s;
    });
}

std::unique_ptr<VrTreeOpaque> new_tree(const UploadJob& j, int max_depth, int device, const Tuning& tn) {
    std::unique_ptr<VrTreeOpaque> t(new (std::nothrow) VrTreeOpaque());
    if (!t) return t;
    t->desc = *j.d;
    t->desc.child = nullptr;
    t->desc.data = nullptr;
    t->desc.extra = nullptr;
    t->max_depth = max_depth;
    t->device = device;
    t->tn = tn;
    t->leaf_stride_h = vr::leaf_stride_halfs(j.d->data_dim);
    return t;
}

hipError_t relayout(const UploadJob& j, const Staged& s, const std::vector<int32_t>& perm, VrTreeOpaque* t,
                    DeviceBuffer& d_perm) {
    const int32_t* src_child = j.from_host ? s.child.get<int32_t>() : j.d->child;
    const uint16_t* src_data = (j.q || j.from_host) ? s.data.get<uint16_t>() : j.d->data;
    const size_t leaves_sz = j.n_slots * (size_t)t->leaf_stride_h * sizeof(uint16_t);
    DeviceBuffer& nodes = t->arrays[kNodes];
    hipError_t e = nodes.alloc(j.child_sz);
    if (e == hipSuccess) e = t->arrays[kLeaves].alloc(leaves_sz);
    if (e == hipSuccess) e = alloc_launch_scratch(t);
    if (e == hipSuccess) e = d_perm.alloc(perm.size() * sizeof(int32_t));
    if (e == hipSuccess)
        e = hipMemcpy(d_perm.get(), perm.data(), perm.size() * sizeof(int32_t), hipMemcpyHostToDevice);
    if (e == hipSuccess)
        e = vr::launch_relayout(src_child, src_data, d_perm.get<int32_t>(), nodes.get<uint32_t>(),
                                t->arrays[kLeaves].get<uint16_t>(), (int64_t)j.n_slots, j.N3, j.d->data_dim,
                                t->leaf_stride_h, nullptr);
    t->device_bytes = j.child_sz + leaves_sz + sizeof(uint32_t);
    return e;
}

hipError_t build_lookup(const LookupPlan& plan, const std::vector<int32_t>& brick_roots, VrTreeOpaque* t,
                        DeviceBuffer& d_roots, uint32_t& flag) {
    const int G0 = plan.G0, BL = plan.BL;
    const size_t top_sz = ((size_t)1 << (3 * G0)) * sizeof(uint2);
    const int n_bricks = BL > 0 ? (int)brick_roots.size() : 0;
    const size_t brick_sz = ((size_t)n_bricks << (3 * BL)) * sizeof(uint32_t);
    hipError_t e = t->arrays[kTop].alloc(top_sz);
    if (e == hipSuccess && n_bricks) e = t->arrays[kBricks].alloc(brick_sz);
    if (e == hipSuccess && n_bricks) e = d_roots.alloc(n_bricks * sizeof(int32_t));
    if (e == hipSuccess && n_bricks)
        e = hipMemcpy(d_roots.get(), brick_roots.data(), n_bricks * sizeof(int32_t), hipMemcpyHostToDevice);
    const int blocked = (n_bricks && BL == 3)
                            ? (t->tn.brick_blocked >= 0 ? t->tn.brick_blocked
                                                        : (top_sz + brick_sz > (128ull << 20)))
                            : 0;
    if (e == hipSuccess)
        e = vr::launch_build_lookup(t->arrays[kNodes].get<uint32_t>(), d_roots.get<int32_t>(), n_bricks,
                                    t->arrays[kTop].get<uint2>(), t->arrays[kBricks].get<uint32_t>(),
                                    G0, BL, blocked, t->status.get<uint32_t>(), nullptr);
    if (e == hipSuccess) e = hipMemcpy(&flag, t->status.get(), sizeof(flag), hipMemcpyDeviceToHost);
    if (e == hipSuccess && flag == 0) {
        t->top_levels = G0;
        t->brick_levels = n_bricks ? BL : 0;
        t->brick_blocked = blocked;
        t->n_bricks = n_bricks;
        t->brick_root.assign(brick_roots.begin(), brick_roots.begin() + n_bricks);
        t->device_bytes += top_sz + brick_sz;
    }
    return e;
}

hipError_t upload_extra(const UploadJob& j, VrTreeOpaque* t) {
    if (!j.d->extra || !j.d->extra_count) return hipSuccess;
    const size_t esz = (size_t)j.d->extra_count * sizeof(float);
    hipError_t e = t->extra.alloc(esz);
    if (e == hipSuccess)
        e = hipMemcpy(t->extra.get(), j.d->extra, esz,
                      j.from_host ? hipMemcpyHostToDevice : hipMemcpyDeviceToDevice);
    t->device_bytes += esz;
    return e;
}

int upload_steps(const UploadJob& j, vr_tree_t* out) {
    std::shared_future<Walk> walk = start_walk(j);
    int device = 0;
    const hipError_t e_dev = hipGetDevice(&device);
    j.mark("HIP runtime up");
    std::future<void> prefault = std::async(std::launch::async, [&j] {
        if (j.from_host && !j.q) prefault_host_range(j.d->data, j.data_sz);
    });
    std::future<Staged> copies = start_copies(j, e_dev, device, walk);

    const Walk& w = walk.get();
    if (w.max_depth < 0) return fail(VR_ERR_BAD_TREE, "bad tree: %s", w.why);
    if (e_dev != hipSuccess)
        return fail(VR_ERR_HIP, "hipGetDevice failed: %s", hipGetErrorString(e_dev));
    const Tuning tn = default_tuning();
    const LookupPlan plan =
        plan_lookup(j.d->N, w.max_depth, j.d->capacity, tn.top_levels, tn.brick_levels, [&w](int l) {
            return (uint64_t)std::count(w.level.begin(), w.level.end(), (uint8_t)l);
        });
    std::unique_ptr<VrTreeOpaque> t = new_tree(j, w.max_depth, device, tn);
    if (!t) return fail(VR_ERR_OUT_OF_MEMORY, "host allocation failed");
    std::vector<int32_t> brick_roots;
    const std::vector<int32_t> perm =
        node_permutation(j.host_child, j.d->capacity, j.N3, plan.G0, plan.BL, w.level, brick_roots);
    t->file_node = inverse_permutation(perm);
    j.mark("host walks done");

    const Staged staged = copies.get();
    DeviceBuffer d_perm, d_roots;
    hipError_t e = staged.e;
    if (e == hipSuccess) e = relayout(j, staged, perm, t.get(), d_perm);
    uint32_t flag = 0;
    if (e == hipSuccess && plan.G0 > 0) e = build_lookup(plan, brick_roots, t.get(), d_roots, flag);
    if (e == hipSuccess && flag != 0)
        return fail(VR_ERR_BAD_TREE, "lookup structure build failed (flag %u)", flag);
    if (e == hipSuccess) e = hipDeviceSynchronize();
    if (e == hipSuccess) e = upload_extra(j, t.get());
    if (e != hipSuccess) return fail(hip_code(e), "tree upload failed: %s", hipGetErrorString(e));
    j.mark("device-ready");
    *out = t.release();
    return VR_OK;
}

int upload_body(const VrTreeDesc* d, const VrQuantDesc* q, vr_tree_t* out) {
    if (int rc = check_upload_args(d, q, out)) return rc;
    const int N3 = d->N * d->N * d->N;
    const size_t n_slots = (size_t)d->capacity * N3;
    UploadJob j{d, q, d->child, N3, n_slots, n_slots * sizeof(int32_t),
                n_slots * (size_t)d->data_dim * sizeof(uint16_t), d->memory != 1,
                getenv("VR_UPLOAD_TIMING") != nullptr, std::chrono::steady_clock::now()};
    std::vector<int32_t> fetched;
    if (int rc = fetch_child_words(j, fetched)) return rc;
    return upload_steps(j, out);
}

int upload_impl(const VrTreeDesc* d, const VrQuantDesc* q, vr_tree_t* out) {
    try {
        return upload_body(d, q, out);
    } catch (const std::bad_alloc&) {
        if (out) *out = nullptr;
        return fail(VR_ERR_OUT_OF_MEMORY, "tree upload: host allocation failed");
    } catch (const std::exception& e) {
        if (out) *out = nullptr;
        return fail(VR_ERR_OUT_OF_MEMORY, "tree upload: %s", e.what());
    }
}

}

extern "C" {

int vr_tree_upload(const VrTreeDesc* d, vr_tree_t* out) { return upload_impl(d, nullptr, out); }

int vr_tree_upload_quantized(const VrTreeDesc* d, const VrQuantDesc* q, vr_tree_t* out) {
    if (!q) return fail(VR_ERR_INVALID_ARGUMENT, "quant desc is NULL");
    return upload_impl(d, q, out);
}

int vr_decode_quantized(const VrTreeDesc* d, const VrQuantDesc* q, uint16_t* data_out) {
    if (!d || !q || !data_out) return fail(VR_ERR_INVALID_ARGUMENT, "NULL argument");
    if (d->N < 2 || d->N > 16 || d->capacity <= 0 || d->data_dim < 1)
        return fail(VR_ERR_INVALID_ARGUMENT, "bad N / capacity / data_dim");
    if (int rc = check_quant(d, q)) return rc;
    const size_t n_slots = (size_t)d->capacity * d->N * d->N * d->N;
    const size_t data_sz = n_slots * (size_t)d->data_dim * sizeof(uint16_t);
    DeviceBuffer staging;
    hipError_t e = hipSuccess;
    if (d->memory != 1) e = staging.alloc(data_sz);
    uint16_t* d_data = d->memory != 1 ? staging.get<uint16_t>() : data_out;
    int device = 0;
    if (e == hipSuccess) e = hipGetDevice(&device);
    if (e == hipSuccess) e = decode_quant_on_device(d, q, n_slots, d_data, device);
    if (e == hipSuccess && d->memory != 1)
        e = hipMemcpy(data_out, d_data, data_sz, hipMemcpyDeviceToHost);
    if (e != hipSuccess) return fail(hip_code(e), "quantised decode failed: %s", hipGetErrorString(e));
    return VR_OK;
}

int vr_tree_clone(vr_tree_t src, int device, vr_tree_t* out) {
    if (!src || !out) return fail(VR_ERR_INVALID_ARGUMENT, "tree/out is NULL");
    *out = nullptr;
    int n_dev = 0;
    HIP_TRY(hipGetDeviceCount(&n_dev));
    if (device < 0 || device >= n_dev)
        return fail(VR_ERR_INVALID_ARGUMENT, "device %d outside [0,%d)", device, n_dev);
    std::lock_guard<std::mutex> src_lock(src->launch_mutex);
    {
        DeviceGuard g(src->device);
        HIP_TRY(hipDeviceSynchronize());
    }
    DeviceGuard guard(device);
    std::unique_ptr<VrTreeOpaque> t(new (std::nothrow) VrTreeOpaque());
    if (!t) return fail(VR_ERR_OUT_OF_MEMORY, "host allocation failed");
    static_cast<TreeShape&>(*t) = *src;
    t->device = device;
    t->tn = src->tn;
    t->file_node = src->file_node;
    t->brick_root = src->brick_root;
    t->device_bytes -= src->file_node_dev.bytes() + src->brick_root_dev.bytes() + src->node_of_file_dev.bytes();
    bool p2p = true;
    if (src->device != device) {
        int can = 0;
        if (hipDeviceCanAccessPeer(&can, device, src->device) != hipSuccess) can = 0;
        p2p = can != 0;
        if (p2p) {
            const hipError_t pe = hipDeviceEnablePeerAccess(src->device, 0);
            if (pe != hipSuccess && pe != hipErrorPeerAccessAlreadyEnabled) p2p = false;
        }
        (void)hipGetLastError();
    }
    auto copy = [&](DeviceBuffer& to, const DeviceBuffer& from) {
        if (!from) return hipSuccess;
        const hipError_t e = to.alloc(from.bytes());
        return e != hipSuccess ? e : hipMemcpyPeer(to.get(), device, from.get(), src->device, from.bytes());
    };
    hipError_t e = hipSuccess;
    for (int i = 0; i < 4 && e == hipSuccess; ++i) e = copy(t->arrays[i], src->arrays[i]);
    if (e == hipSuccess) e = copy(t->extra, src->extra);
    if (e == hipSuccess) e = alloc_launch_scratch(t.get());
    if (e == hipSuccess) e = hipDeviceSynchronize();
    if (e != hipSuccess)
        return fail(hip_code(e), "tree clone from device %d to device %d failed: %s%s", src->device, device,
                    hipGetErrorString(e),
                    p2p ? "" : " (the devices have NO peer access: check `rocm-smi --showtopo`, "
                               "IOMMU / ACS settings and HSA_ENABLE_IPC_MODE_LEGACY=0)");
    if (!p2p)
        fprintf(stderr, "[volrend_hip] note: devices %d and %d have no peer access; the clone was "
                        "staged through host memory\n", src->device, device);
    *out = t.release();
    return VR_OK;
}

int vr_tree_free(vr_tree_t t) {
    delete t;
    return VR_OK;
}

}
```

volrend_amd/csrc/vr_values.cpp:

```cpp
#include <hip/hip_runtime.h>

#include <cmath>
#include <mutex>

#include "vr_host.h"

int ensure_device_table(VrTreeOpaque* t, DeviceBuffer& dev, const std::vector<int32_t>& host, size_t entries,
                        const char* name) {
    if (dev) return VR_OK;
    const size_t bytes = host.size() * sizeof(int32_t);
    if (bytes != entries * sizeof(int32_t)) return fail(VR_ERR_HIP, "the tree carries no %s table", name);
    hipError_t e = dev.alloc(bytes);
    if (e == hipSuccess) e = hipMemcpy(dev.get(), host.data(), bytes, hipMemcpyHostToDevice);
    if (e != hipSuccess) {
        (void)dev.reset();
        return fail(hip_code(e), "%s table of %zu bytes: %s", name, bytes, hipGetErrorString(e));
    }
    t->device_bytes += bytes;
    return VR_OK;
}

int ensure_file_nodes(VrTreeOpaque* t) {
    return ensure_device_table(t, t->file_node_dev, t->file_node, (size_t)t->desc.capacity, "file-order");
}

namespace {

int ensure_value_tables(VrTreeOpaque* t) {
    if (int rc = ensure_file_nodes(t)) return rc;
    if (t->top_levels > 0 && t->n_bricks > 0)
        if (int rc = ensure_device_table(t, t->brick_root_dev, t->brick_root, (size_t)t->n_bricks, "brick-root")) return rc;
    return VR_OK;
}

int tree_data_pass(vr_tree_t t, void* data_dev, int dtype, void* stream, bool update) {
    if (!t || !data_dev) return fail(VR_ERR_INVALID_ARGUMENT, "NULL argument");
    if (dtype != VR_DATA_F16 && dtype != VR_DATA_F32) return fail(VR_ERR_INVALID_ARGUMENT, "unknown dtype %d", dtype);
    DeviceGuard device_guard(t->device);
    hipStream_t hs = static_cast<hipStream_t>(stream);
    std::lock_guard<std::mutex> guard(t->launch_mutex);
    if (int rc = ensure_value_tables(t)) return rc;
    vr::UpdateArgs a;
    a.nodes = t->arrays[kNodes].get<uint32_t>();
    a.leaves = t->arrays[kLeaves].get<uint16_t>();
    a.file_node = t->file_node_dev.get<int32_t>();
    a.data = data_dev;
    a.capacity = t->desc.capacity;
    a.N3 = t->desc.N * t->desc.N * t->desc.N;
    a.data_dim = t->desc.data_dim;
    a.stride_h = t->leaf_stride_h;
    a.f32 = dtype == VR_DATA_F32;
    if (!update) {
        HIP_TRY(vr::launch_read_values(a, t->n_cus, hs));
        return VR_OK;
    }
    HIP_TRY(vr::launch_update_values(a, t->n_cus, hs));
    if (t->top_levels > 0)
        HIP_TRY(vr::launch_refresh_lookup(a.nodes, t->brick_root_dev.get<int32_t>(), t->n_bricks,
                                          t->arrays[kTop].get<uint2>(), t->arrays[kBricks].get<uint32_t>(),
                                          t->top_levels, t->brick_levels, hs));
    return VR_OK;
}

int validate_step(vr_tree_t t, const VrStep* s) {
    if (!t || !s || !s->master || !s->grad || !s->touched) return fail(VR_ERR_INVALID_ARGUMENT, "NULL argument");
    if (s->kind != VR_STEP_SGD && s->kind != VR_STEP_ADAM) return fail(VR_ERR_INVALID_ARGUMENT, "unknown kind %d", s->kind);
    if (!std::isfinite(s->lr) || !std::isfinite(s->lr_sigma))
        return fail(VR_ERR_INVALID_ARGUMENT, "lr / lr_sigma must be finite (got %g, %g)", (double)s->lr, (double)s->lr_sigma);
    if (!std::isfinite(s->eps)) return fail(VR_ERR_INVALID_ARGUMENT, "eps must be finite (got %g)", (double)s->eps);
    if (s->kind == VR_STEP_ADAM) {
        if (!s->m || !s->v) return fail(VR_ERR_INVALID_ARGUMENT, "VR_STEP_ADAM: NULL moments (m / v)");
        if (s->step < 1) return fail(VR_ERR_INVALID_ARGUMENT, "VR_STEP_ADAM: step=%d must be at least 1", s->step);
        if (!(s->beta1 >= 0.f && s->beta1 < 1.f) || !(s->beta2 >= 0.f && s->beta2 < 1.f))
            return fail(VR_ERR_INVALID_ARGUMENT, "VR_STEP_ADAM: beta1=%g, beta2=%g outside [0, 1)", (double)s->beta1,
                        (double)s->beta2);
    }
    return VR_OK;
}

}

extern "C" {

int vr_tree_step(vr_tree_t t, const VrStep* s, void* stream) {
    if (int rc = validate_step(t, s)) return rc;
    DeviceGuard device_guard(t->device);
    hipStream_t hs = static_cast<hipStream_t>(stream);
    std::lock_guard<std::mutex> guard(t->launch_mutex);
    if (int rc = ensure_value_tables(t)) return rc;
    if (!t->node_of_file_dev) {
        const size_t cap = (size_t)t->desc.capacity;
        if (t->file_node.size() != cap) return fail(VR_ERR_HIP, "the tree carries no file-order table");
        std::vector<int32_t> inverse(cap);
        for (size_t m = 0; m < cap; ++m) inverse[(size_t)t->file_node[m]] = (int32_t)m;
        if (int rc = ensure_device_table(t, t->node_of_file_dev, inverse, cap, "device-order")) return rc;
    }
    vr::StepArgs a;
    a.nodes = t->arrays[kNodes].get<uint32_t>();
    a.leaves = t->arrays[kLeaves].get<uint16_t>();
    a.node_of_file = t->node_of_file_dev.get<int32_t>();
    a.master = s->master;
    a.grad = s->grad;
    a.m = s->m;
    a.v = s->v;
    a.touched = s->touched;
    a.N3 = t->desc.N * t->desc.N * t->desc.N;
    a.n_slots = t->desc.capacity * a.N3;
    a.n_words = (a.n_slots + 31) / 32;
    a.data_dim = t->desc.data_dim;
    a.stride_h = t->leaf_stride_h;
    a.adam = s->kind == VR_STEP_ADAM;
    a.lr = s->lr;
    a.lr_sigma = s->lr_sigma;
    a.beta1 = a.beta2 = a.omb1 = a.omb2 = a.eps = 0.f;
    a.sbc2 = 1.f;
    if (a.adam) {
        const double b1 = (double)s->beta1, b2 = (double)s->beta2;
        const double bc1 = 1.0 - std::pow(b1, (double)s->step);
        a.beta1 = s->beta1;
        a.beta2 = s->beta2;
        a.omb1 = (float)(1.0 - b1);
        a.omb2 = (float)(1.0 - b2);
        a.sbc2 = (float)std::sqrt(1.0 - std::pow(b2, (double)s->step));
        a.lr = (float)((double)s->lr / bc1);
        a.lr_sigma = (float)((double)s->lr_sigma / bc1);
        a.eps = s->eps;
    }
    if (a.n_words > 0 && a.data_dim > 0) HIP_TRY(vr::launch_step_values(a, t->n_cus, hs));
    if (t->top_levels > 0)
        HIP_TRY(vr::launch_refresh_lookup(a.nodes, t->brick_root_dev.get<int32_t>(), t->n_bricks,
                                          t->arrays[kTop].get<uint2>(), t->arrays[kBricks].get<uint32_t>(),
                                          t->top_levels, t->brick_levels, hs));
    return VR_OK;
}

int vr_tree_update_data(vr_tree_t t, const void* data_dev, int dtype, void* stream) {
    return tree_data_pass(t, const_cast<void*>(data_dev), dtype, stream, true);
}

int vr_tree_read_data(vr_tree_t t, void* data_dev, int dtype, void* stream) {
    return tree_data_pass(t, data_dev, dtype, stream, false);
}

}
```

Measured before the change: 2767 Mrays/s.

## Cull empty 8x8 pixel blocks using a coarse occupancy grid before ray generation

Builds a coarse occupancy bitmap and surface-cell list from the octree at upload time. Per frame, a new kernel projects occupied cells into a per-8x8-block screen mask, and raygen then skips setup for rays in blocks the mask marks empty. Rays that would only cross empty space are meant to avoid traversal entirely. The cost is an extra mask kernel per launch, extra scratch memory and occupancy rebuilds after data updates. Correctness depends on the projection being conservative.

```diff
diff --git a/include/volrend_hip.h b/include/volrend_hip.h
--- a/include/volrend_hip.h
+++ b/include/volrend_hip.h
@@ -197,6 +197,7 @@
 int vr_set_tuning(const char* key, int value);
 int vr_tree_set_tuning(vr_tree_t tree, const char* key, int value);
 int vr_sched_stats(vr_tree_t tree, uint64_t out[8], int reset);
+int vr_tree_cull_stats(vr_tree_t tree, uint64_t out[2], int reset);
 int vr_touch_enable(vr_tree_t tree, int enable);
 int vr_touch_count(vr_tree_t tree, uint64_t out[4], int reset);
 int vr_touch_read(vr_tree_t tree, int which, uint32_t* host_words, uint64_t n_words,
diff --git a/volrend_amd/_abi.py b/volrend_amd/_abi.py
--- a/volrend_amd/_abi.py
+++ b/volrend_amd/_abi.py
@@ -149,6 +149,7 @@
     "vr_set_tuning": (C.c_int, [C.c_char_p, C.c_int]),
     "vr_tree_set_tuning": (C.c_int, [C.c_void_p, C.c_char_p, C.c_int]),
     "vr_sched_stats": (C.c_int, [C.c_void_p, C.POINTER(C.c_uint64 * 8), C.c_int]),
+    "vr_tree_cull_stats": (C.c_int, [C.c_void_p, C.POINTER(C.c_uint64 * 2), C.c_int]),
     "vr_touch_enable": (C.c_int, [C.c_void_p, C.c_int]),
     "vr_touch_count": (C.c_int, [C.c_void_p, C.POINTER(C.c_uint64 * 4), C.c_int]),
     "vr_touch_read": (C.c_int, [C.c_void_p, C.c_int, C.c_void_p, C.c_uint64, C.POINTER(C.c_uint64),
diff --git a/volrend_amd/_tree.py b/volrend_amd/_tree.py
--- a/volrend_amd/_tree.py
+++ b/volrend_amd/_tree.py
@@ -213,6 +213,11 @@
                  "retire_rounds", "retired", "iterations")
         return dict(zip(names, [int(v) for v in out]))
 
+    def cull_stats(self, reset: bool = True) -> dict:
+        out = (C.c_uint64 * 2)()
+        _abi.check(_abi.lib().vr_tree_cull_stats(self.handle, C.byref(out), 1 if reset else 0))
+        return {"blocks": int(out[0]), "culled": int(out[1])}
+
     def touch_enable(self, enable: bool = True) -> None:
         _abi.check(_abi.lib().vr_touch_enable(self.handle, 1 if enable else 0))
 
diff --git a/volrend_amd/csrc/vr_api.cpp b/volrend_amd/csrc/vr_api.cpp
--- a/volrend_amd/csrc/vr_api.cpp
+++ b/volrend_amd/csrc/vr_api.cpp
@@ -32,6 +32,7 @@
     {"brick_blocked", "VR_BRICK_BLOCKED", &Tuning::brick_blocked, kAutoFlag, 0, 0, true},
     {"max_iter", "VR_MAX_ITER", &Tuning::max_iter, kClamp, 1, INT_MAX, false},
     {"weights_check", "VR_WEIGHTS_CHECK", &Tuning::weights_check, kFlag, 0, 0, false},
+    {"block_cull", "VR_BLOCK_CULL", &Tuning::block_cull, kFlag, 0, 0, false},
 };
 
 const Knob* find_knob(const char* key) {
@@ -204,6 +205,20 @@
     return VR_OK;
 }
 
+int vr_tree_cull_stats(vr_tree_t t, uint64_t out[2], int reset) {
+    if (!t || !out) return fail(VR_ERR_INVALID_ARGUMENT, "NULL argument");
+    DeviceGuard guard(t->device);
+    uint64_t lines[vr::kCullStatLines * vr::kCullStatStride];
+    HIP_TRY(hipMemcpy(lines, t->cull_stats.get(), sizeof(lines), hipMemcpyDeviceToHost));
+    if (reset) HIP_TRY(hipMemset(t->cull_stats.get(), 0, sizeof(lines)));
+    out[0] = out[1] = 0;
+    for (int i = 0; i < vr::kCullStatLines; ++i) {
+        out[0] += lines[i * vr::kCullStatStride];
+        out[1] += lines[i * vr::kCullStatStride + 1];
+    }
+    return VR_OK;
+}
+
 int vr_tree_status(vr_tree_t t, uint32_t* status, int reset) {
     if (!t || !status) return fail(VR_ERR_INVALID_ARGUMENT, "NULL argument");
     DeviceGuard guard(t->device);
diff --git a/volrend_amd/csrc/vr_host.h b/volrend_amd/csrc/vr_host.h
--- a/volrend_amd/csrc/vr_host.h
+++ b/volrend_amd/csrc/vr_host.h
@@ -45,6 +45,7 @@
     int leaf_stride_h = 0;
     int top_levels = 0, brick_levels = 0, n_bricks = 0;
     int brick_blocked = 0;
+    int occ_levels = -1;
     uint64_t device_bytes = 0;
 };
 
@@ -52,6 +53,8 @@
     int device = 0;
     DeviceBuffer arrays[4];
     DeviceBuffer extra, status, sched_stats;
+    DeviceBuffer occ;
+    DeviceBuffer cull_stats;
     DeviceBuffer touch[4];
     DeviceBuffer touch_out;
     DeviceBuffer probe_buf;
@@ -81,6 +84,14 @@
     return vr::ray_slots(total_rays) * (size_t)words_per_ray * sizeof(uint32_t);
 }
 inline size_t list_pixel_bytes(uint32_t total_rays) { return (size_t)total_rays * 4; }
+inline uint32_t block_mask_words(const vr::KParams& k) {
+    const uint64_t blocks = (uint64_t)k.tiles_x * (uint64_t)(k.tile_w / 8) * (uint64_t)k.tiles_y * (uint64_t)(k.tile_h / 8);
+    return (uint32_t)(((blocks + 127) / 128) * 4);
+}
+inline size_t block_mask_bytes(const vr::KParams& k, int n_frames) {
+    return (size_t)block_mask_words(k) * sizeof(uint32_t) * (size_t)n_frames;
+}
+hipError_t refresh_occupancy(const VrTreeOpaque* t, hipStream_t hs);
 
 int acquire_slot(VrTreeOpaque* t, std::unique_lock<std::mutex>& guard, hipStream_t hs, vr::KParams& k,
                  size_t need, unsigned& slot);
diff --git a/volrend_amd/csrc/vr_internal.h b/volrend_amd/csrc/vr_internal.h
--- a/volrend_amd/csrc/vr_internal.h
+++ b/volrend_amd/csrc/vr_internal.h
@@ -150,6 +150,9 @@
 };
 
 inline bool uses_lookup(const KParams& p) { return p.N == 2 && p.top_levels > 0; }
+inline bool needs_full(const KParams& p) {
+    return p.format == VR_FORMAT_SG || p.format == VR_FORMAT_ASG || p.instrumented || p.render_depth;
+}
 
 inline unsigned persistent_grid(int64_t total_blocks, int n_cus, int waves_per_cu) {
     int64_t want = total_blocks / 2;
@@ -173,6 +176,29 @@
     int32_t n;
     AovDesc f[kTableChunk];
 };
+
+constexpr int kOccMaxLevels = 7;
+constexpr int kOccHeaderWords = 4;
+constexpr int kCullStatLines = 16;
+constexpr int kCullStatStride = 8;
+constexpr int kMaskMaxWords = 4096;
+__host__ __device__ inline size_t occ_bitmap_words(int g) { return g >= 2 ? ((size_t)1 << (3 * g)) / 32 : 1; }
+__host__ __device__ inline size_t occ_words(int g) { return kOccHeaderWords + occ_bitmap_words(g) + ((size_t)1 << (3 * g)); }
+struct CullParams {
+    const uint32_t* mask;
+    uint32_t words_per_frame;
+    uint32_t nbx;
+    unsigned long long* stats;
+};
+struct MaskParams {
+    uint32_t* mask;
+    uint32_t words_per_frame, nbx, nby;
+    const uint32_t* occ;
+    int32_t levels;
+    int32_t groups_per_frame;
+};
+hipError_t launch_block_mask(const KParams& p, const MaskParams& m, hipStream_t stream);
+hipError_t launch_build_occupancy(const uint32_t* nodes, int levels, uint32_t* occ, hipStream_t stream);
 
 constexpr int kWeightRayWords = kRayDeltaScale + 1;
 static_assert(kWeightRayWords <= kRayWords, "a slot reserved for colour rays holds the weight rays of the same shape");
@@ -245,11 +271,12 @@
 hipError_t launch_step_values(const StepArgs& a, int n_cus, hipStream_t stream);
 
 hipError_t launch_prepare_aov(const AovParams& a, const AovTable& tbl, hipStream_t stream);
-hipError_t launch_render_aov(const KParams& p, const AovParams& a, int fp_mode, int n_cus, int waves_override,
-                             int gen_waves, hipStream_t stream);
-hipError_t launch_prepare(const KParams& p, const FrameTable& tbl, hipStream_t stream);
-hipError_t launch_render(const KParams& p, int fp_mode, int n_cus, int waves_override, int gen_waves,
-                         hipStream_t stream, const RayList* rays = nullptr);
+hipError_t launch_render_aov(const KParams& p, const AovParams& a, const CullParams& cull, int fp_mode, int n_cus,
+                             int waves_override, int gen_waves, hipStream_t stream);
+hipError_t launch_prepare(const KParams& p, const FrameTable& tbl, hipStream_t stream, uint32_t* mask = nullptr,
+                          uint32_t words_per_frame = 0);
+hipError_t launch_render(const KParams& p, const CullParams& cull, int fp_mode, int n_cus, int waves_override,
+                         int gen_waves, hipStream_t stream, const RayList* rays = nullptr);
 hipError_t launch_probe(const KParams& p, const float probe[3], float* out_dev,
                         hipStream_t stream);
 
diff --git a/volrend_amd/csrc/vr_launch.cpp b/volrend_amd/csrc/vr_launch.cpp
--- a/volrend_amd/csrc/vr_launch.cpp
+++ b/volrend_amd/csrc/vr_launch.cpp
@@ -233,10 +233,10 @@
 }
 bool needs_file_order(LaunchKind kind) { return kind == LaunchKind::kWeights || kind == LaunchKind::kBackward; }
 
-struct Turn { const vr::KParams& k; const Tuning& tn; int gen_waves; unsigned slot; hipStream_t hs; void* pixel_words; };
+struct Turn { const vr::KParams& k; const Tuning& tn; int gen_waves; unsigned slot; hipStream_t hs; void* extra; };
 
 template <typename Enqueue>
-int run_launch(VrTreeOpaque* t, LaunchKind kind, const Views& v, bool pixel_words, vr::KParams& k, void* stream,
+int run_launch(VrTreeOpaque* t, LaunchKind kind, const Views& v, size_t extra_bytes, vr::KParams& k, void* stream,
                Enqueue&& enqueue) {
     DeviceGuard device_guard(t->device);
     hipStream_t hs = static_cast<hipStream_t>(stream);
@@ -250,13 +250,12 @@
     fill_tuning_params(k, t, tn, plan);
     const size_t records = ray_buffer_bytes(k.total_rays, record_words(kind, k.ray_tail_words));
     unsigned slot;
-    if (int rc = acquire_slot(t, guard, hs, k, records + (pixel_words ? list_pixel_bytes(k.total_rays) : 0), slot))
-        return rc;
+    if (int rc = acquire_slot(t, guard, hs, k, records + extra_bytes, slot)) return rc;
     fill_tree_params(k, t);
     SlotTurn turn;
     if (int rc = turn.begin(t->slots[slot], hs)) return rc;
-    void* const pixels = pixel_words ? t->slots[slot].rays.get<char>() + records : nullptr;
-    return enqueue(Turn{k, tn, plan.raygen_waves, slot, hs, pixels});
+    void* const extra = extra_bytes ? t->slots[slot].rays.get<char>() + records : nullptr;
+    return enqueue(Turn{k, tn, plan.raygen_waves, slot, hs, extra});
 }
 
 int validate_aov(int n_frames, const VrCamera* cams, const VrRenderOptions* opt, const VrFrame* frames,
@@ -288,7 +287,8 @@
 }
 
 int enqueue_tables(const vr::KParams& k, const Views& v, hipStream_t hs, const VrFrame* frames = nullptr,
-                   const VrAov* aovs = nullptr, const vr::AovParams& a = vr::AovParams{}) {
+                   const VrAov* aovs = nullptr, const vr::AovParams& a = vr::AovParams{},
+                   const vr::MaskParams& m = vr::MaskParams{}) {
     for (int first = 0; first < k.n_frames; first += vr::kTableChunk) {
         vr::FrameTable tbl;
         memset(&tbl, 0, sizeof(tbl));
@@ -302,7 +302,7 @@
             tbl.f[i].depth = frames[first + i].depth;
             tbl.f[i].counters = reinterpret_cast<VrCounters*>(frames[first + i].counters);
         }
-        HIP_TRY(vr::launch_prepare(k, tbl, hs));
+        HIP_TRY(vr::launch_prepare(k, tbl, hs, m.mask, m.words_per_frame));
         if (aovs) {
             vr::AovTable at;
             memset(&at, 0, sizeof(at));
@@ -318,6 +318,14 @@
     return VR_OK;
 }
 
+bool culls_blocks(const VrTreeOpaque* t, const vr::KParams& k, const Tuning& tn, const VrRenderOptions* opt) {
+    if (!tn.block_cull || !t->occ || !vr::uses_lookup(k) || vr::needs_full(k)) return false;
+    if (opt->sigma_thresh < 0.f || k.ndc_width > 0) return false;
+    for (int i = 0; i < 3; ++i)
+        if (!(opt->render_bbox[i] >= 0.f) || !(opt->render_bbox[i + 3] <= 1.f)) return false;
+    return block_mask_words(k) <= (uint32_t)vr::kMaskMaxWords;
+}
+
 int render_launch(vr_tree_t t, int n_frames, const VrCamera* cams, const VrRenderOptions* opt,
                   const VrFrame* frames, const VrAov* aovs, int depth_units, bool want_aov, void* stream) {
     vr::KParams k;
@@ -329,15 +337,30 @@
         if (int rc = validate_aov(n_frames, cams, opt, frames, aovs, depth_units, a)) return rc;
     fill_caller_params(k, opt, &frames[0]);
     const Views v{cams, n_frames};
-    return run_launch(t, want_aov ? LaunchKind::kAov : LaunchKind::kColour, v, false, k, stream, [&](const Turn& u) -> int {
+    const size_t mask_bytes = t->occ ? block_mask_bytes(k, n_frames) : 0;
+    return run_launch(t, want_aov ? LaunchKind::kAov : LaunchKind::kColour, v, mask_bytes, k, stream, [&](const Turn& u) -> int {
         a.planes = t->slot_aovs.get<vr::AovDesc>() + (size_t)u.slot * vr::kMaxBatch;
         if (u.k.enable_probe)
             HIP_TRY(vr::launch_probe(u.k, opt->probe, const_cast<float*>(u.k.probe_coeffs), u.hs));
-        if (int rc = enqueue_tables(u.k, v, u.hs, frames, want_aov ? aovs : nullptr, a)) return rc;
+        vr::MaskParams m{};
+        vr::CullParams cull{};
+        if (u.extra && culls_blocks(t, u.k, u.tn, opt)) {
+            m.mask = static_cast<uint32_t*>(u.extra);
+            m.words_per_frame = block_mask_words(u.k);
+            m.nbx = (uint32_t)(u.k.tiles_x * (u.k.tile_w / 8));
+            m.nby = (uint32_t)(u.k.tiles_y * (u.k.tile_h / 8));
+            m.occ = t->occ.get<uint32_t>();
+            m.levels = t->occ_levels;
+            const int groups = 2048 / n_frames;
+            m.groups_per_frame = groups < 4 ? 4 : (groups > 128 ? 128 : groups);
+            cull = vr::CullParams{m.mask, m.words_per_frame, m.nbx, t->cull_stats.get<unsigned long long>()};
+        }
+        if (int rc = enqueue_tables(u.k, v, u.hs, frames, want_aov ? aovs : nullptr, a, m)) return rc;
+        if (m.mask) HIP_TRY(vr::launch_block_mask(u.k, m, u.hs));
         if (want_aov)
-            HIP_TRY(vr::launch_render_aov(u.k, a, frames[0].fp_mode, t->n_cus, u.tn.waves_per_cu, u.gen_waves, u.hs));
+            HIP_TRY(vr::launch_render_aov(u.k, a, cull, frames[0].fp_mode, t->n_cus, u.tn.waves_per_cu, u.gen_waves, u.hs));
         else
-            HIP_TRY(vr::launch_render(u.k, frames[0].fp_mode, t->n_cus, u.tn.waves_per_cu, u.gen_waves, u.hs));
+            HIP_TRY(vr::launch_render(u.k, cull, frames[0].fp_mode, t->n_cus, u.tn.waves_per_cu, u.gen_waves, u.hs));
         return VR_OK;
     });
 }
@@ -383,7 +406,7 @@
     k.offscreen = 1;
     k.layout = VR_LAYOUT_FRAME;
     k.pitch = (int64_t)k.width * 4;
-    return run_launch(t, kind, v, false, k, stream, [&](const Turn& u) -> int {
+    return run_launch(t, kind, v, 0, k, stream, [&](const Turn& u) -> int {
         if (int rc = enqueue_tables(u.k, v, u.hs)) return rc;
         HIP_TRY(launch(u));
         return VR_OK;
@@ -531,10 +554,11 @@
     f.accum = out->accum;
     fill_caller_params(k, opt, &f);
     k.any_accum = out->accum ? 1 : 0;
-    return run_launch(t, LaunchKind::kColour, v, !out->rgba, k, stream, [&](const Turn& u) -> int {
-        f.rgba = out->rgba ? out->rgba : u.pixel_words;
+    const size_t pixel_bytes = out->rgba ? 0 : list_pixel_bytes(k.total_rays);
+    return run_launch(t, LaunchKind::kColour, v, pixel_bytes, k, stream, [&](const Turn& u) -> int {
+        f.rgba = out->rgba ? out->rgba : u.extra;
         if (int rc = enqueue_tables(u.k, v, u.hs, &f)) return rc;
-        HIP_TRY(vr::launch_render(u.k, fp_mode, t->n_cus, u.tn.waves_per_cu, u.gen_waves, u.hs, v.rays()));
+        HIP_TRY(vr::launch_render(u.k, vr::CullParams{}, fp_mode, t->n_cus, u.tn.waves_per_cu, u.gen_waves, u.hs, v.rays()));
         return VR_OK;
     });
 }
diff --git a/volrend_amd/csrc/vr_launch_plan.h b/volrend_amd/csrc/vr_launch_plan.h
--- a/volrend_amd/csrc/vr_launch_plan.h
+++ b/volrend_amd/csrc/vr_launch_plan.h
@@ -19,6 +19,7 @@
     int brick_blocked = -1;
     int max_iter = 1 << 22;
     int weights_check = 1;
+    int block_cull = 1;
 };
 
 enum class LaunchKind { kColour, kAov, kWeights, kBackward };
diff --git a/volrend_amd/csrc/vr_render.hip b/volrend_amd/csrc/vr_render.hip
--- a/volrend_amd/csrc/vr_render.hip
+++ b/volrend_amd/csrc/vr_render.hip
@@ -115,6 +115,7 @@
 #define VR_RENDER_KERNEL render_kernel
 #define VR_RAYGEN_KERNEL raygen_kernel
 #define VR_KERNEL_ARGS const KParams p
+#define VR_RAYGEN_ARGS const KParams p, const CullParams cull
 #define VR_KERNEL_AOV false
 #define VR_KERNEL_AOV_LOCAL const AovParams aov{};
 #endif
@@ -496,7 +497,7 @@
 
 
 template <int FMA, bool FULL, int GW>
-__global__ __launch_bounds__(kWave* GW) void VR_RAYGEN_KERNEL(VR_KERNEL_ARGS) {
+__global__ __launch_bounds__(kWave* GW) void VR_RAYGEN_KERNEL(VR_RAYGEN_ARGS) {
     constexpr bool AOV = VR_KERNEL_AOV;
     VR_KERNEL_AOV_LOCAL
     const int lane = threadIdx.x & (kWave - 1);
@@ -504,6 +505,7 @@
     const uint32_t id =
         (uint32_t)(((int64_t)blockIdx.x * GW + wave) * kWave + lane);
     bool valid = false;
+    bool culled = false;
     Ray nr;
     uint8_t* px = nullptr;
     uint32_t xy = 0;
@@ -511,11 +513,19 @@
     float vdir[3] = {0.f, 0.f, 1.f};
     if (id < p.total_rays) {
         const PixelRef r = locate(p, id);
+        if constexpr (!FULL) {
+            if (cull.mask) {
+                const uint32_t b = (uint32_t)(r.y >> 3) * cull.nbx + (uint32_t)(r.x >> 3);
+                const uint32_t w = cull.mask[(size_t)r.frame * cull.words_per_frame + (b >> 5)];
+                culled = __builtin_amdgcn_readfirstlane((int)((w >> (b & 31u)) & 1u)) == 0;
+            }
+        }
         if (r.in_image) {
             frame = r.frame;
             xy = (uint32_t)r.x | ((uint32_t)r.y << 16);
             px = pixel_ptr(p, p.frames[r.frame], r);
-            setup_ray<FMA>(p, r, nr, vdir);
+            if (culled) reset_ray(nr);
+            else setup_ray<FMA>(p, r, nr, vdir);
             if (nr.alive) {
                 valid = true;
             } else {
@@ -526,7 +536,29 @@
         }
     }
     const unsigned long long m_valid = __builtin_amdgcn_ballot_w64(valid);
+    __shared__ uint32_t wave_culled[GW];
+    if constexpr (!FULL && GW > 1) {
+        if (cull.mask && lane == 0) wave_culled[wave] = culled ? 1u : 0u;
+    }
     const uint32_t my_base = reserve_ray_slots<GW>(p, m_valid, lane, wave);
+    if constexpr (!FULL) {
+        if (cull.mask && threadIdx.x < 2u) {
+            const int64_t left = (int64_t)(p.total_rays >> 6) - (int64_t)blockIdx.x * GW;
+            uint32_t n = (uint32_t)(left < 0 ? 0 : (left < GW ? left : GW));
+            if (threadIdx.x == 1u) {
+                if constexpr (GW > 1) {
+                    n = 0;
+#pragma unroll
+                    for (int w = 0; w < GW; ++w) n += wave_culled[w];
+                } else {
+                    n = culled ? 1u : 0u;
+                }
+            }
+            if (n)
+                atomicAdd(cull.stats + (blockIdx.x & (uint32_t)(kCullStatLines - 1)) * kCullStatStride + threadIdx.x,
+                          (unsigned long long)n);
+        }
+    }
     if (!valid) return;
     const uint32_t slot = my_base + lane_rank(m_valid);
     uint32_t* rb = ray_slot(p.ray_buf_rw, kRayWords + p.ray_tail_words, slot);
@@ -562,12 +594,14 @@
 #undef VR_RENDER_KERNEL
 #undef VR_RAYGEN_KERNEL
 #undef VR_KERNEL_ARGS
+#undef VR_RAYGEN_ARGS
 #undef VR_KERNEL_AOV
 #undef VR_KERNEL_AOV_LOCAL
 #define VR_KERNEL_PASS_AOV
 #define VR_RENDER_KERNEL render_aov_kernel
 #define VR_RAYGEN_KERNEL raygen_aov_kernel
 #define VR_KERNEL_ARGS const KParams p, const AovParams aov
+#define VR_RAYGEN_ARGS const KParams p, const AovParams aov, const CullParams cull
 #define VR_KERNEL_AOV true
 #define VR_KERNEL_AOV_LOCAL
 #include "vr_render.hip"
@@ -575,6 +609,7 @@
 #undef VR_RENDER_KERNEL
 #undef VR_RAYGEN_KERNEL
 #undef VR_KERNEL_ARGS
+#undef VR_RAYGEN_ARGS
 #undef VR_KERNEL_AOV
 #undef VR_KERNEL_AOV_LOCAL
 
@@ -605,12 +640,100 @@
     store_colour_ray<FMA, FULL>(p, my_base + lane_rank(m_valid), nr, xy, px, 0, vdir);
 }
 
-__global__ void prepare_launch_kernel(FrameTable tbl, FrameDesc* frames, uint32_t* queue_head) {
+__global__ void prepare_launch_kernel(FrameTable tbl, FrameDesc* frames, uint32_t* queue_head, uint32_t* mask,
+                                      uint32_t words_per_frame) {
     const int i = threadIdx.x;
     if (i < tbl.n) frames[tbl.first + i] = tbl.f[i];
     if (tbl.first == 0 && i < kMaxQueues) {
         queue_head[i * kQueueStride + kQueueHead] = 0u;
         queue_head[i * kQueueStride + kQueueCount] = 0u;
+    }
+    if (mask) {
+        uint4* const q = reinterpret_cast<uint4*>(mask + (size_t)tbl.first * words_per_frame);
+        const uint32_t n = (uint32_t)tbl.n * (words_per_frame >> 2);
+        for (uint32_t j = threadIdx.x; j < n; j += blockDim.x) q[j] = make_uint4(0u, 0u, 0u, 0u);
+    }
+}
+
+__global__ __launch_bounds__(256) void block_mask_kernel(const KParams p, const MaskParams m) {
+    __shared__ uint32_t bits[kMaskMaxWords];
+    __shared__ uint32_t whole;
+    const uint32_t wpf = m.words_per_frame;
+    for (uint32_t i = threadIdx.x; i < wpf; i += blockDim.x) bits[i] = 0u;
+    if (threadIdx.x == 0) whole = 0u;
+    __syncthreads();
+    const int frame = blockIdx.y;
+    const int g = m.levels;
+    const uint32_t count = m.occ[0];
+    const uint32_t* const list = m.occ + kOccHeaderWords + occ_bitmap_words(g);
+    const uint32_t per = (count + (uint32_t)m.groups_per_frame - 1u) / (uint32_t)m.groups_per_frame;
+    const uint32_t lo = blockIdx.x * per;
+    const uint32_t hi = lo + per < count ? lo + per : count;
+    float xf[12];
+#pragma unroll
+    for (int i = 0; i < 12; ++i) xf[i] = p.frames[frame].xf[i];
+    const float cell = u2f((uint32_t)(127 - g) << 23);
+    float inv_scale[3], r2 = 0.f;
+#pragma unroll
+    for (int i = 0; i < 3; ++i) {
+        inv_scale[i] = 1.f / p.scale[i];
+        const float h = 0.5f * cell * inv_scale[i];
+        r2 += h * h;
+    }
+    const float r = __builtin_sqrtf(r2) * 1.0001f;
+    bool ok = r > 0.f && r < 1e30f;
+#pragma unroll
+    for (int a = 0; a < 3; ++a)
+#pragma unroll
+        for (int b = a; b < 3; ++b) {
+            const float d = xf[3 * a] * xf[3 * b] + xf[3 * a + 1] * xf[3 * b + 1] + xf[3 * a + 2] * xf[3 * b + 2];
+            if (!(__builtin_fabsf(d - (a == b ? 1.f : 0.f)) <= 1e-4f)) ok = false;
+        }
+    const float afx = __builtin_fabsf(p.fx), afy = __builtin_fabsf(p.fy);
+    const uint32_t n_mask = (1u << g) - 1u;
+    const float fnbx = (float)m.nbx, fnby = (float)m.nby;
+    if (!ok && lo < hi) whole = 1u;
+    for (uint32_t idx = lo + threadIdx.x; ok && idx < hi; idx += blockDim.x) {
+        const uint32_t c = list[idx];
+        const float tc[3] = {((float)((c >> (2 * g)) & n_mask) + 0.5f) * cell, ((float)((c >> g) & n_mask) + 0.5f) * cell,
+                             ((float)(c & n_mask) + 0.5f) * cell};
+        float d[3];
+#pragma unroll
+        for (int i = 0; i < 3; ++i) d[i] = (tc[i] - p.offset[i]) * inv_scale[i] - xf[9 + i];
+        const float X = xf[0] * d[0] + xf[1] * d[1] + xf[2] * d[2];
+        const float Y = xf[3] * d[0] + xf[4] * d[1] + xf[5] * d[2];
+        const float depth = -(xf[6] * d[0] + xf[7] * d[1] + xf[8] * d[2]);
+        if (!(depth - r > 0.01f * r)) {
+            if (!(depth + r < 0.f)) whole = 1u;
+            continue;
+        }
+        const float inv = 1.f / (depth * (depth - r));
+        const float rx = afx * r * __builtin_sqrtf(depth * depth + X * X) * inv * 1.05f + 1.f;
+        const float ry = afy * r * __builtin_sqrtf(depth * depth + Y * Y) * inv * 1.05f + 1.f;
+        const float px = 0.5f * (float)p.width + p.fx * X / depth;
+        const float py = 0.5f * (float)p.height - p.fy * Y / depth;
+        const float fx0 = __builtin_floorf(__builtin_fmaxf((px - rx) * 0.125f, 0.f));
+        const float fx1 = __builtin_floorf(__builtin_fminf((px + rx) * 0.125f, fnbx - 1.f));
+        const float fy0 = __builtin_floorf(__builtin_fmaxf((py - ry) * 0.125f, 0.f));
+        const float fy1 = __builtin_floorf(__builtin_fminf((py + ry) * 0.125f, fnby - 1.f));
+        if (!(fx0 <= fx1) || !(fy0 <= fy1)) continue;
+        const uint32_t bx0 = (uint32_t)fx0, bx1 = (uint32_t)fx1, by0 = (uint32_t)fy0, by1 = (uint32_t)fy1;
+        for (uint32_t by = by0; by <= by1; ++by) {
+            const uint32_t first = by * m.nbx + bx0, last = by * m.nbx + bx1;
+            for (uint32_t w = first >> 5; w <= (last >> 5); ++w) {
+                const uint32_t from = w == (first >> 5) ? (first & 31u) : 0u;
+                const uint32_t to = w == (last >> 5) ? (last & 31u) : 31u;
+                const uint32_t mask = (0xFFFFFFFFu >> (31u - to)) & (0xFFFFFFFFu << from);
+                if ((bits[w] & mask) != mask) atomicOr(&bits[w], mask);
+            }
+        }
+    }
+    __syncthreads();
+    uint32_t* const out = m.mask + (size_t)frame * wpf;
+    const bool all = whole != 0u;
+    for (uint32_t i = threadIdx.x; i < wpf; i += blockDim.x) {
+        const uint32_t v = all ? 0xFFFFFFFFu : bits[i];
+        if (v != 0u && (out[i] & v) != v) atomicOr(&out[i], v);
     }
 }
 
@@ -678,10 +801,6 @@
     const int64_t leaf = query_generic<0>(p, cen, &cube_sz, &levels, &word);
     const uint16_t* v = p.leaves + leaf * p.leaf_stride_h;
     for (int i = threadIdx.x; i < p.data_dim - 1; i += blockDim.x) out[i] = h2f(v[i]);
-}
-
-bool needs_full(const KParams& p) {
-    return p.format == VR_FORMAT_SG || p.format == VR_FORMAT_ASG || p.instrumented || p.render_depth;
 }
 
 template <int FMA, int MODE, bool AOV>
@@ -724,19 +843,19 @@
 }
 
 template <bool AOV>
-hipError_t launch_march(const KParams& p, const AovParams& a, int fp_mode, int n_cus, int waves_override,
-                        int gen_waves, hipStream_t stream, const RayList* rays = nullptr) {
+hipError_t launch_march(const KParams& p, const AovParams& a, const CullParams& cull, int fp_mode, int n_cus,
+                        int waves_override, int gen_waves, hipStream_t stream, const RayList* rays = nullptr) {
     const int64_t total_blocks = p.n_wave_blocks * p.n_frames;
     {
         const bool full = needs_full(p);
 #define VR_GEN(FMA_, FULL_, GW_)                                                                    \
     do {                                                                                            \
         const dim3 grid_((unsigned)((total_blocks + GW_ - 1) / GW_)), block_(kWave * GW_);          \
-        if constexpr (AOV) hipLaunchKernelGGL((raygen_aov_kernel<FMA_, FULL_, GW_>), grid_, block_, 0, stream, p, a); \
+        if constexpr (AOV) hipLaunchKernelGGL((raygen_aov_kernel<FMA_, FULL_, GW_>), grid_, block_, 0, stream, p, a, cull); \
         else if (rays) {                                                                            \
             if constexpr (GW_ >= 4) hipLaunchKernelGGL((raygen_rays_kernel<FMA_, FULL_, GW_>), grid_, block_, 0, stream, p, *rays); \
         }                                                                                           \
-        else hipLaunchKernelGGL((raygen_kernel<FMA_, FULL_, GW_>), grid_, block_, 0, stream, p);    \
+        else hipLaunchKernelGGL((raygen_kernel<FMA_, FULL_, GW_>), grid_, block_, 0, stream, p, cull); \
     } while (0)
 #define VR_GEN_GW(FMA_, FULL_)                                                                      \
     do {                                                                                            \
@@ -758,16 +877,25 @@
 
 }
 
-hipError_t launch_prepare(const KParams& p, const FrameTable& tbl, hipStream_t stream) {
+hipError_t launch_prepare(const KParams& p, const FrameTable& tbl, hipStream_t stream, uint32_t* mask,
+                          uint32_t words_per_frame) {
     hipLaunchKernelGGL(prepare_launch_kernel, dim3(1), dim3(64), 0, stream, tbl,
-                       const_cast<FrameDesc*>(p.frames), p.queue_head);
+                       const_cast<FrameDesc*>(p.frames), p.queue_head, mask, words_per_frame);
     return hipGetLastError();
 }
 
-hipError_t launch_render(const KParams& p, int fp_mode, int n_cus, int waves_override, int gen_waves,
-                         hipStream_t stream, const RayList* rays) {
+hipError_t launch_block_mask(const KParams& p, const MaskParams& m, hipStream_t stream) {
+    if (p.n_frames <= 0 || m.groups_per_frame <= 0) return hipSuccess;
+    hipLaunchKernelGGL(block_mask_kernel, dim3((unsigned)m.groups_per_frame, (unsigned)p.n_frames), dim3(256), 0, stream,
+                       p, m);
+    return hipGetLastError();
+}
+
+hipError_t launch_render(const KParams& p, const CullParams& cull, int fp_mode, int n_cus, int waves_override,
+                         int gen_waves, hipStream_t stream, const RayList* rays) {
     if (p.n_wave_blocks <= 0 || p.n_frames <= 0) return hipSuccess;
-    const hipError_t e = launch_march<false>(p, AovParams{}, fp_mode, n_cus, waves_override, gen_waves, stream, rays);
+    const hipError_t e =
+        launch_march<false>(p, AovParams{}, cull, fp_mode, n_cus, waves_override, gen_waves, stream, rays);
     if (e != hipSuccess || !p.enable_probe || p.probe_disp_size <= 0) return e;
     const int side = p.probe_disp_size + 5;
     const dim3 pgrid((unsigned)((side * side + 255) / 256), (unsigned)p.n_frames);
@@ -783,10 +911,10 @@
     return hipGetLastError();
 }
 
-hipError_t launch_render_aov(const KParams& p, const AovParams& a, int fp_mode, int n_cus, int waves_override,
-                             int gen_waves, hipStream_t stream) {
+hipError_t launch_render_aov(const KParams& p, const AovParams& a, const CullParams& cull, int fp_mode, int n_cus,
+                             int waves_override, int gen_waves, hipStream_t stream) {
     if (p.n_wave_blocks <= 0 || p.n_frames <= 0) return hipSuccess;
-    return launch_march<true>(p, a, fp_mode, n_cus, waves_override, gen_waves, stream);
+    return launch_march<true>(p, a, cull, fp_mode, n_cus, waves_override, gen_waves, stream);
 }
 
 hipError_t launch_probe(const KParams& p, const float probe[3], float* out_dev,
diff --git a/volrend_amd/csrc/vr_slots.cpp b/volrend_amd/csrc/vr_slots.cpp
--- a/volrend_amd/csrc/vr_slots.cpp
+++ b/volrend_amd/csrc/vr_slots.cpp
@@ -114,7 +114,7 @@
         return fail(VR_ERR_INVALID_ARGUMENT, "n_slots=%d outside [1,%u]", n_slots, kLaunchSlots);
     vr::KParams geo;
     if (int rc = launch_geometry(width, height, tile_w, tile_h, 0, world, n_frames, geo)) return rc;
-    return reserve_slots(t, n_slots, colour_record_bytes(t, geo.total_rays));
+    return reserve_slots(t, n_slots, colour_record_bytes(t, geo.total_rays) + (t->occ ? block_mask_bytes(geo, n_frames) : 0));
 }
 
 int vr_reserve(vr_tree_t t, int width, int height, int n_frames) {
diff --git a/volrend_amd/csrc/vr_tree_kernels.hip b/volrend_amd/csrc/vr_tree_kernels.hip
--- a/volrend_amd/csrc/vr_tree_kernels.hip
+++ b/volrend_amd/csrc/vr_tree_kernels.hip
@@ -167,6 +167,101 @@
     bricks[gid] = node;
 }
 
+__device__ __forceinline__ bool leaf_occupied(uint32_t w) {
+    return (float)__builtin_bit_cast(_Float16, (uint16_t)(w & 0xFFFFu)) > 0.f;
+}
+
+__device__ bool subtree_occupied(const uint32_t* nodes, uint32_t node) {
+    constexpr int kStack = 24;
+    uint32_t st_node[kStack];
+    uint32_t st_next[kStack];
+    int sp = 0;
+    st_node[0] = node;
+    st_next[0] = 0;
+    while (sp >= 0) {
+        if (st_next[sp] == 8u) {
+            --sp;
+            continue;
+        }
+        const uint32_t w = nodes[(uint64_t)st_node[sp] * 8u + st_next[sp]];
+        st_next[sp]++;
+        if (w & kLeafBit) {
+            if (leaf_occupied(w)) return true;
+        } else {
+            if (sp + 1 >= kStack) return true;
+            ++sp;
+            st_node[sp] = w;
+            st_next[sp] = 0;
+        }
+    }
+    return false;
+}
+
+__global__ void occupancy_cells_kernel(const uint32_t* nodes, int g, uint32_t* occ) {
+    const uint32_t cell = blockIdx.x * blockDim.x + threadIdx.x;
+    const uint32_t n_cells = 1u << (3 * g);
+    if (cell == 0) occ[0] = 0u;
+    bool set = false;
+    if (cell < n_cells) {
+        const uint32_t mask = (1u << g) - 1u;
+        const uint32_t cx = (cell >> (2 * g)) & mask, cy = (cell >> g) & mask, cz = cell & mask;
+        uint32_t node = 0;
+        bool leaf = false;
+        for (int l = 0; l < g; ++l) {
+            const int sh = g - 1 - l;
+            const uint32_t slot = (((cx >> sh) & 1u) << 2) | (((cy >> sh) & 1u) << 1) | ((cz >> sh) & 1u);
+            const uint32_t w = nodes[(uint64_t)node * 8u + slot];
+            if (w & kLeafBit) {
+                leaf = true;
+                set = leaf_occupied(w);
+                break;
+            }
+            node = w;
+        }
+        if (!leaf) set = subtree_occupied(nodes, node);
+    }
+    const unsigned long long m = __builtin_amdgcn_ballot_w64(set);
+    if ((threadIdx.x & 31u) == 0u && cell < (n_cells > 32u ? n_cells : 32u))
+        occ[kOccHeaderWords + (cell >> 5)] = (uint32_t)(m >> (threadIdx.x & 32u));
+}
+
+__global__ void occupancy_list_kernel(int g, uint32_t* occ) {
+    const uint32_t cell = blockIdx.x * blockDim.x + threadIdx.x;
+    const uint32_t n_cells = 1u << (3 * g);
+    const uint32_t* bits = occ + kOccHeaderWords;
+    uint32_t* list = occ + kOccHeaderWords + occ_bitmap_words(g);
+    bool keep = false;
+    if (cell < n_cells) {
+        const int n = 1 << g;
+        const int c[3] = {(int)((cell >> (2 * g)) & (uint32_t)(n - 1)), (int)((cell >> g) & (uint32_t)(n - 1)),
+                          (int)(cell & (uint32_t)(n - 1))};
+        auto is_set = [&](int x, int y, int z) -> bool {
+            if (x < 0 || y < 0 || z < 0 || x >= n || y >= n || z >= n) return false;
+            const uint32_t i = ((uint32_t)x << (2 * g)) | ((uint32_t)y << g) | (uint32_t)z;
+            return (bits[i >> 5] >> (i & 31u)) & 1u;
+        };
+        if (is_set(c[0], c[1], c[2]))
+            keep = !(is_set(c[0] - 1, c[1], c[2]) && is_set(c[0] + 1, c[1], c[2]) && is_set(c[0], c[1] - 1, c[2]) &&
+                     is_set(c[0], c[1] + 1, c[2]) && is_set(c[0], c[1], c[2] - 1) && is_set(c[0], c[1], c[2] + 1));
+    }
+    const unsigned long long m = __builtin_amdgcn_ballot_w64(keep);
+    if (m == 0ull) return;
+    const uint32_t lane = threadIdx.x & 63u;
+    uint32_t base = 0;
+    if (lane == (uint32_t)__builtin_ctzll(m)) base = atomicAdd(&occ[0], (uint32_t)__builtin_popcountll(m));
+    base = (uint32_t)__builtin_amdgcn_readlane((int)base, __builtin_ctzll(m));
+    if (keep)
+        list[base + __builtin_amdgcn_mbcnt_hi((uint32_t)(m >> 32), __builtin_amdgcn_mbcnt_lo((uint32_t)m, 0u))] = cell;
+}
+
+}
+
+hipError_t launch_build_occupancy(const uint32_t* nodes, int levels, uint32_t* occ, hipStream_t stream) {
+    const uint32_t n_cells = 1u << (3 * levels);
+    const dim3 grid((n_cells + 255u) / 256u), block(256);
+    hipLaunchKernelGGL(occupancy_cells_kernel, grid, block, 0, stream, nodes, levels, occ);
+    hipLaunchKernelGGL(occupancy_list_kernel, grid, block, 0, stream, levels, occ);
+    return hipGetLastError();
 }
 
 hipError_t launch_assemble(uint8_t* frame, int64_t pitch, const uint8_t* gathered, int width,
diff --git a/volrend_amd/csrc/vr_upload.cpp b/volrend_amd/csrc/vr_upload.cpp
--- a/volrend_amd/csrc/vr_upload.cpp
+++ b/volrend_amd/csrc/vr_upload.cpp
@@ -86,6 +86,9 @@
     if (e == hipSuccess) e = hipMemset(t->status.get(), 0, sizeof(uint32_t));
     if (e == hipSuccess) e = t->sched_stats.alloc(vr::kSchedStats * sizeof(unsigned long long));
     if (e == hipSuccess) e = hipMemset(t->sched_stats.get(), 0, vr::kSchedStats * sizeof(unsigned long long));
+    const size_t cull_sz = (size_t)vr::kCullStatLines * vr::kCullStatStride * sizeof(unsigned long long);
+    if (e == hipSuccess) e = t->cull_stats.alloc(cull_sz);
+    if (e == hipSuccess) e = hipMemset(t->cull_stats.get(), 0, cull_sz);
     if (e == hipSuccess) e = t->probe_buf.alloc(sizeof(float) * (size_t)t->desc.data_dim * kLaunchSlots);
     for (unsigned i = 0; i < kLaunchSlots && e == hipSuccess; ++i) e = t->slots[i].done.create();
     if (e == hipSuccess) e = t->slot_frames.alloc(sizeof(vr::FrameDesc) * vr::kMaxBatch * kLaunchSlots);
@@ -237,6 +240,17 @@
     return e;
 }
 
+hipError_t build_occupancy(VrTreeOpaque* t) {
+    if (t->top_levels <= 0) return hipSuccess;
+    const int deepest = t->max_depth + 1;
+    t->occ_levels = deepest < vr::kOccMaxLevels ? deepest : vr::kOccMaxLevels;
+    const size_t bytes = vr::occ_words(t->occ_levels) * sizeof(uint32_t);
+    hipError_t e = t->occ.alloc(bytes);
+    if (e == hipSuccess) e = refresh_occupancy(t, nullptr);
+    t->device_bytes += bytes;
+    return e;
+}
+
 hipError_t upload_extra(const UploadJob& j, VrTreeOpaque* t) {
     if (!j.d->extra || !j.d->extra_count) return hipSuccess;
     const size_t esz = (size_t)j.d->extra_count * sizeof(float);
@@ -283,6 +297,7 @@
     if (e == hipSuccess && plan.G0 > 0) e = build_lookup(plan, brick_roots, t.get(), d_roots, flag);
     if (e == hipSuccess && flag != 0)
         return fail(VR_ERR_BAD_TREE, "lookup structure build failed (flag %u)", flag);
+    if (e == hipSuccess) e = build_occupancy(t.get());
     if (e == hipSuccess) e = hipDeviceSynchronize();
     if (e == hipSuccess) e = upload_extra(j, t.get());
     if (e != hipSuccess) return fail(hip_code(e), "tree upload failed: %s", hipGetErrorString(e));
@@ -315,6 +330,11 @@
     }
 }
 
+}
+
+hipError_t refresh_occupancy(const VrTreeOpaque* t, hipStream_t hs) {
+    if (!t->occ) return hipSuccess;
+    return vr::launch_build_occupancy(t->arrays[kNodes].get<uint32_t>(), t->occ_levels, t->occ.get<uint32_t>(), hs);
 }
 
 extern "C" {
@@ -386,6 +406,7 @@
     hipError_t e = hipSuccess;
     for (int i = 0; i < 4 && e == hipSuccess; ++i) e = copy(t->arrays[i], src->arrays[i]);
     if (e == hipSuccess) e = copy(t->extra, src->extra);
+    if (e == hipSuccess) e = copy(t->occ, src->occ);
     if (e == hipSuccess) e = alloc_launch_scratch(t.get());
     if (e == hipSuccess) e = hipDeviceSynchronize();
     if (e != hipSuccess)
diff --git a/volrend_amd/csrc/vr_values.cpp b/volrend_amd/csrc/vr_values.cpp
--- a/volrend_amd/csrc/vr_values.cpp
+++ b/volrend_amd/csrc/vr_values.cpp
@@ -59,6 +59,7 @@
         HIP_TRY(vr::launch_refresh_lookup(a.nodes, t->brick_root_dev.get<int32_t>(), t->n_bricks,
                                           t->arrays[kTop].get<uint2>(), t->arrays[kBricks].get<uint32_t>(),
                                           t->top_levels, t->brick_levels, hs));
+    HIP_TRY(refresh_occupancy(t, hs));
     return VR_OK;
 }
 
@@ -131,6 +132,7 @@
         HIP_TRY(vr::launch_refresh_lookup(a.nodes, t->brick_root_dev.get<int32_t>(), t->n_bricks,
                                           t->arrays[kTop].get<uint2>(), t->arrays[kBricks].get<uint32_t>(),
                                           t->top_levels, t->brick_levels, hs));
+    HIP_TRY(refresh_occupancy(t, hs));
     return VR_OK;
 }
 
```

New measurement: 2843 Mrays/s (median of 6 runs). 2.7% higher.
